# pps-lab/rofl-project-code

Hardware: AMD Instinct MI355X
Metric: range-proof elements/sec (create+verify), d=25k 32-bit (higher is better)
Workload: dtype u32x8 (255-bit integer field)

## Files before the change

### include/rofl_zk_debug.h

```cpp
#ifndef ROFL_ZK_DEBUG_H
#define ROFL_ZK_DEBUG_H
#include "rofl_zk.h"
#ifdef __cplusplus
extern "C" {
#endif

typedef struct {
    double total_ms;
    double msm_accumulate_ms;
    uint64_t msm_accumulate_launches;
    uint64_t msm_terms;
    double fold_ms;
    uint64_t fold_launches;
    uint64_t fold_point_reads;
    double host_ms;
    uint64_t msm_additions;
} rofl_timing_t;
int rofl_last_timing(rofl_timing_t *out);
enum { ROFL_TK_MSM_ACCUMULATE_FB = 0, ROFL_TK_MSM_ACCUMULATE_GEN = 1, ROFL_TK_MSM_SCATTER = 2, ROFL_TK_MSM_REDUCE = 3,
       ROFL_TK_MSM_SMALL = 4, ROFL_TK_FOLD_TAB = 5, ROFL_TK_FOLD = 6, ROFL_TK_OTHER = 7,
       ROFL_TK_SIGMA = 8,
       ROFL_TK_VERIFY_SCALARS = 9,
       ROFL_TK_CODEC = 10,
       ROFL_TK_COUNT = 11 };
typedef struct { double ms; uint64_t launches, fe_muls, bytes; } rofl_kernel_time_t;
int rofl_last_kernel_times(rofl_kernel_time_t out[ROFL_TK_COUNT]);
int rofl_set_timing(int enabled);
int rofl_dbg_map_device(int logical, int physical);
int rofl_dbg_bind_device(int device);

int rofl_dbg_msm(const uint8_t *scalars32, const uint8_t *points32, size_t n, uint8_t out32[32]);
int rofl_dbg_verify_labelled(const uint8_t *label, size_t label_len, size_t gens_capacity, const uint8_t *proof, size_t proof_len,
                             const uint8_t *commits32, size_t m, size_t n_bits, const uint8_t verifier_seed[32], int *ok_out);
int rofl_dbg_msm_retries(uint64_t out[4]);
int rofl_dbg_point_decodes(uint64_t *count_out);
int rofl_bench_femul(unsigned iters, double *fe_mul_per_sec_out);
int rofl_dbg_quad_ops(const uint8_t *pairs64, size_t pairs, unsigned doublings, uint8_t *out_serial32, uint8_t *out_quad32);
int rofl_dbg_fd_ops(unsigned op, size_t n, const uint32_t *in, uint32_t *out);
int rofl_dbg_sc_ops(unsigned op, size_t n, const uint32_t *in, uint32_t *out);
int rofl_dbg_quantize(unsigned site, size_t rows, size_t d, size_t dpad, size_t prove_range, unsigned fp_bits, unsigned fp_frac,
                      const float *values, const uint8_t *blindings32, void *out, float *terms_out, uint32_t *status_out);

int rofl_dbg_host_fd_ops_raw(unsigned op, size_t n, const uint32_t *in, uint32_t *out);
int rofl_dbg_host_sc_ops(unsigned op, size_t n, const uint32_t *in, uint32_t *out);
int rofl_dbg_host_pool_stress(unsigned threads, unsigned jobs);
int rofl_dbg_host_fe_mul(const uint8_t a[32], const uint8_t b[32], uint8_t out[32]);
int rofl_dbg_host_fe_ops(const uint8_t a[32], const uint8_t b[32], uint8_t out_add[32], uint8_t out_sub[32], uint8_t out_sq[32], uint8_t out_inv[32]);
int rofl_dbg_host_sc_invert(const uint8_t a[32], uint8_t out_ref[32], uint8_t out_fast[32], double *ns_ref, double *ns_fast);
int rofl_dbg_host_sc_mul(const uint8_t a[32], const uint8_t b[32], uint8_t out[32]);
int rofl_dbg_host_sc_wide(const uint8_t in[64], uint8_t out[32]);
int rofl_dbg_host_sc_wide_mont(const uint8_t in[64], uint8_t out[32]);
int rofl_dbg_host_sc_lazy(const uint8_t *a32, const uint8_t *b32, size_t count, uint8_t out_lazy[32], uint8_t out_ref[32]);
int rofl_dbg_host_from_uniform(const uint8_t in[64], uint8_t out[32]);
int rofl_dbg_host_scalarmult_base(const uint8_t k[32], int use_blinding_base, uint8_t out[32]);
int rofl_dbg_host_fd_codec(const uint8_t in[32], uint8_t out[32]);
int rofl_dbg_host_decode_encode(const uint8_t in[32], uint8_t out[32]);
int rofl_dbg_host_fd_ops(const uint8_t a[32], const uint8_t b[32], uint8_t out_mul[32], uint8_t out_sq[32], uint8_t out_add[32], uint8_t out_sub[32], uint8_t out_inv[32]);
int rofl_dbg_host_fd_scalarmult(const uint8_t k[32], const uint8_t p[32], uint8_t out[32]);
int rofl_dbg_host_merlin(const uint8_t *label, size_t label_len, const uint8_t *msg, size_t msg_len, uint8_t out[64]);
int rofl_dbg_host_nonce(const uint8_t seed[32], uint64_t idx, uint8_t out[32]);
int rofl_dbg_host_blind(const uint8_t seed[32], uint64_t idx, uint8_t out[32]);
int rofl_dbg_host_dh(const uint8_t sk32[32], const uint8_t *own_pk32, const uint8_t peer_pk32[32], uint8_t out32[32], uint8_t *status);
int rofl_dbg_host_shamir_share(size_t n_secrets, const uint8_t *secrets32, const uint8_t *coef_seeds32, size_t threshold, size_t n_shares,
                               const uint32_t *xs, uint8_t *shares_out32);
int rofl_dbg_host_shamir_reconstruct(size_t n_secrets, size_t n_shares, const uint32_t *xs, const uint8_t *shares32, uint8_t *secrets_out32);
int rofl_dbg_host_feldman_commit(size_t n_secrets, const uint8_t *secrets32, const uint8_t *coef_seeds32, size_t threshold,
                                 uint8_t *commitments_out32);
int rofl_dbg_host_feldman_verify(size_t n_secrets, size_t threshold, const uint8_t *commitments32, size_t n_shares, const uint32_t *xs,
                                 const uint8_t *shares32, uint8_t *verdict_out);

int rofl_dbg_host_bench(int what, unsigned iters, double *ns_out);
int rofl_dbg_host_horner8_selftest(unsigned W, unsigned c, int lanes, double *us_simd, double *us_scalar);
int rofl_dbg_host_encode8_selftest(unsigned batches, double *us_simd, double *us_scalar);
int rofl_dbg_host_merlin8_selftest(int lanes, unsigned count, unsigned skew, double *us_simd, double *us_scalar);
int rofl_dbg_host_merlin8_lbl3_selftest(int lanes, unsigned count, unsigned skew, double *us_simd, double *us_scalar);
int rofl_dbg_host_merlin8_lbl3_strided_selftest(int lanes, unsigned count, unsigned skew, unsigned stride, double *us_simd, double *us_scalar);
int rofl_dbg_host_merlin_run_selftest(unsigned count, unsigned skew);
int rofl_dbg_host_keccak_zmm_selftest(unsigned states, unsigned chain, double *ns_zmm, double *ns_scalar);
int rofl_dbg_last_hops(double out[10]);

#ifdef __cplusplus
}
#endif
#endif
```

### rofl_project_code_amd/csrc/fd_dbg.hpp

```cpp
#pragma once
#include "fe26.hpp"

namespace rofl {

#define FD_DBG_IN 80
#define FD_DBG_OUT 80
enum { FD_DBG_UNPACK = 0, FD_DBG_CARRY = 1, FD_DBG_PACK = 2, FD_DBG_ADD = 3, FD_DBG_SUB = 4, FD_DBG_NEG = 5, FD_DBG_MUL = 6, FD_DBG_SQ = 7,
       FD_DBG_MUL_LOOSE = 8, FD_DBG_SQ_LOOSE = 9, FD_DBG_INVERT = 10, FD_DBG_POW22523 = 11, FD_DBG_SQRT_RATIO = 12, FD_DBG_ABS = 13,
       FD_DBG_PRED = 14, FD_DBG_MADD = 15, FD_DBG_MSUB = 16, FD_DBG_GD_ADD = 17, FD_DBG_GD_DOUBLE = 18, FD_DBG_GD_DOUBLE_NOT = 19,
       FD_DBG_TO_NIELS = 20, FD_DBG_TO_NIELS_ZINV = 21, FD_DBG_THREAD_OPS = 22,
       FD_DBG_GQ_DOUBLE = 22, FD_DBG_GQ_ADD = 23, FD_DBG_OPS = 24 };

HD fd fd_dbg_load(const u32 *in, int k) {
    fd r;
#pragma unroll
    for (int i = 0; i < 10; i++) r.v[i] = in[10 * k + i];
    return r;
}
HD void fd_dbg_store(u32 *out, int k, const fd &a) {
#pragma unroll
    for (int i = 0; i < 10; i++) out[10 * k + i] = a.v[i];
}
HD gd gd_dbg_load(const u32 *in, int k) { gd r; r.X = fd_dbg_load(in, k); r.Y = fd_dbg_load(in, k + 1); r.Z = fd_dbg_load(in, k + 2); r.T = fd_dbg_load(in, k + 3); return r; }
HD void gd_dbg_store(u32 *out, int k, const gd &p) { fd_dbg_store(out, k, p.X); fd_dbg_store(out, k + 1, p.Y); fd_dbg_store(out, k + 2, p.Z); fd_dbg_store(out, k + 3, p.T); }
HD void fe_dbg_store(u32 *out, int w, const fe &a) {
#pragma unroll
    for (int i = 0; i < 8; i++) out[w + i] = a.v[i];
}
HD void niels_dbg_store(u32 *out, const niels &q) { fe_dbg_store(out, 0, q.ypx); fe_dbg_store(out, 8, q.ymx); fe_dbg_store(out, 16, q.t2d); }

HDN inline void fd_dbg_apply(u32 op, const u32 *in, u32 *out) {
    switch (op) {
    case FD_DBG_UNPACK: { fe w; for (int i = 0; i < 8; i++) w.v[i] = in[i]; fd_dbg_store(out, 0, fd_unpack(w)); break; }
    case FD_DBG_CARRY: fd_dbg_store(out, 0, fd_carry(fd_dbg_load(in, 0))); break;
    case FD_DBG_PACK: {
        fe w = fd_pack(fd_dbg_load(in, 0));
        uint8_t b[32]; fe_tobytes(b, w);
        fe_dbg_store(out, 0, w);
        for (int i = 0; i < 8; i++) out[8 + i] = (u32)b[4 * i] | ((u32)b[4 * i + 1] << 8) | ((u32)b[4 * i + 2] << 16) | ((u32)b[4 * i + 3] << 24);
        break;
    }
    case FD_DBG_ADD: fd_dbg_store(out, 0, fd_add(fd_dbg_load(in, 0), fd_dbg_load(in, 1))); break;
    case FD_DBG_SUB: fd_dbg_store(out, 0, fd_sub(fd_dbg_load(in, 0), fd_dbg_load(in, 1))); break;
    case FD_DBG_NEG: fd_dbg_store(out, 0, fd_neg(fd_dbg_load(in, 0))); break;
    case FD_DBG_MUL: fd_dbg_store(out, 0, fd_mul(fd_dbg_load(in, 0), fd_dbg_load(in, 1))); break;
    case FD_DBG_SQ: fd_dbg_store(out, 0, fd_sq(fd_dbg_load(in, 0))); break;
    case FD_DBG_MUL_LOOSE: fd_dbg_store(out, 0, fd_mul(fd_sub(fd_dbg_load(in, 0), fd_dbg_load(in, 1)), fd_add(fd_dbg_load(in, 2), fd_dbg_load(in, 3)))); break;
    case FD_DBG_SQ_LOOSE: fd_dbg_store(out, 0, fd_sq(fd_add(fd_dbg_load(in, 0), fd_dbg_load(in, 1)))); break;
    case FD_DBG_INVERT: fd_dbg_store(out, 0, fd_invert(fd_dbg_load(in, 0))); break;
    case FD_DBG_POW22523: fd_dbg_store(out, 0, fd_pow22523(fd_dbg_load(in, 0))); break;
    case FD_DBG_SQRT_RATIO: { fd r; bool sq = fd_sqrt_ratio_i(r, fd_dbg_load(in, 0), fd_dbg_load(in, 1)); fd_dbg_store(out, 0, r); out[10] = sq ? 1u : 0u; break; }
    case FD_DBG_ABS: fd_dbg_store(out, 0, fd_abs(fd_dbg_load(in, 0))); break;
    case FD_DBG_PRED: {
        fd a = fd_dbg_load(in, 0), b = fd_dbg_load(in, 1);
        out[0] = fd_isneg(a) ? 1u : 0u; out[1] = fd_iszero(a) ? 1u : 0u; out[2] = fd_eq(a, b) ? 1u : 0u;
        break;
    }
    case FD_DBG_MADD: case FD_DBG_MSUB: {
        nd q; q.ypx = fd_dbg_load(in, 4); q.ymx = fd_dbg_load(in, 5); q.t2d = fd_dbg_load(in, 6);
        gd_dbg_store(out, 0, gd_madd(gd_dbg_load(in, 0), q, op == FD_DBG_MSUB));
        break;
    }
    case FD_DBG_GD_ADD: gd_dbg_store(out, 0, gd_add(gd_dbg_load(in, 0), gd_dbg_load(in, 4))); break;
    case FD_DBG_GD_DOUBLE: gd_dbg_store(out, 0, gd_double(gd_dbg_load(in, 0))); break;
    case FD_DBG_GD_DOUBLE_NOT: gd_dbg_store(out, 0, gd_double_not(gd_dbg_load(in, 0))); break;
    case FD_DBG_TO_NIELS: niels_dbg_store(out, gd_to_niels(gd_dbg_load(in, 0))); break;
    case FD_DBG_TO_NIELS_ZINV: niels_dbg_store(out, gd_to_niels_zinv(gd_dbg_load(in, 0), fd_dbg_load(in, 4))); break;
    default: break;
    }
}

#define SC_DBG_IN 264
#define SC_DBG_OUT 8
enum { SC_DBG_MONTMUL = 0, SC_DBG_TO_MONT = 1, SC_DBG_FROM_MONT = 2, SC_DBG_MUL_PLAIN = 3, SC_DBG_ADD = 4, SC_DBG_NEG = 5, SC_DBG_SUB = 6,
       SC_DBG_LOAD_REDUCED = 7,
       SC_DBG_FROM_WIDE = 8, SC_DBG_FROM_WIDE_MONT = 9, SC_DBG_MAC = 10, SC_DBG_INVERT_MONT = 11, SC_DBG_OPS = 12 };

HD sc sc_dbg_load(const u32 *in, int k) {
    sc r;
#pragma unroll
    for (int i = 0; i < 8; i++) r.v[i] = in[8 * k + i];
    return r;
}
HDN inline sc sc_dbg_apply(u32 op, const u32 *in) {
    const sc a = sc_dbg_load(in, 0), b = sc_dbg_load(in, 1);
    switch (op) {
    case SC_DBG_MONTMUL: return sc_montmul(a, b);
    case SC_DBG_TO_MONT: return sc_to_mont(a);
    case SC_DBG_FROM_MONT: return sc_from_mont(a);
    case SC_DBG_MUL_PLAIN: return sc_mul_plain(a, b);
    case SC_DBG_ADD: return sc_add(a, b);
    case SC_DBG_NEG: return sc_neg(a);
    case SC_DBG_SUB: return sc_sub(a, b);
    case SC_DBG_LOAD_REDUCED: return sc_geq_l(a.v) ? sc_from_mont(sc_to_mont(a)) : a;
    case SC_DBG_FROM_WIDE: return sc_from_wide(a, b);
    case SC_DBG_FROM_WIDE_MONT: return sc_from_wide_mont(a, b);
    case SC_DBG_MAC: {
        u32 acc[17]; for (int i = 0; i < 17; i++) acc[i] = 0;
        u32 count = in[256] > 16 ? 16 : in[256];
        for (u32 k = 0; k < count; k++) sc_mac_wide(acc, sc_dbg_load(in, 2 * (int)k), sc_dbg_load(in, 2 * (int)k + 1));
        return sc_redc_wide(acc);
    }
    case SC_DBG_INVERT_MONT: return sc_invert_mont(a);
    default: return sc_zero();
    }
}

}
```

### rofl_project_code_amd/csrc/fe26.hpp

```cpp
#pragma once
#include "fe32.hpp"
#if defined(ROFL_FD_CHECK_HOST) && !defined(__HIP_DEVICE_COMPILE__)
#include <assert.h>
#define ROFL_FD_CHECK 1
#endif

namespace rofl {

struct fd { u32 v[10]; };
struct gd { fd X, Y, Z, T; };
struct nd { fd ypx, ymx, t2d; };

#define FD_M26 0x3ffffffu
#define FD_M25 0x1ffffffu

HD fd fd_zero() { fd r = {{0, 0, 0, 0, 0, 0, 0, 0, 0, 0}}; return r; }
HD fd fd_one() { fd r = {{1, 0, 0, 0, 0, 0, 0, 0, 0, 0}}; return r; }

HD fd fd_unpack(const fe &a) {
    const u32 *w = a.v;
    fd r;
    r.v[0] = w[0] & FD_M26;
    r.v[1] = ((w[0] >> 26) | (w[1] << 6)) & FD_M25;
    r.v[2] = ((w[1] >> 19) | (w[2] << 13)) & FD_M26;
// ... 68 lines not shown

HD fd fd_reduce_cols(u64 h0, u64 h1, u64 h2, u64 h3, u64 h4, u64 h5, u64 h6, u64 h7, u64 h8, u64 h9) {
    u64 c;
    c = h0 >> 26; h1 += c; h0 &= FD_M26;
    c = h4 >> 26; h5 += c; h4 &= FD_M26;
    c = h1 >> 25; h2 += c; h1 &= FD_M25;
    c = h5 >> 25; h6 += c; h5 &= FD_M25;
    c = h2 >> 26; h3 += c; h2 &= FD_M26;
    c = h6 >> 26; h7 += c; h6 &= FD_M26;
    c = h3 >> 25; h4 += c; h3 &= FD_M25;
    c = h7 >> 25; h8 += c; h7 &= FD_M25;
    c = h4 >> 26; h5 += c; h4 &= FD_M26;
    c = h8 >> 26; h9 += c; h8 &= FD_M26;
    c = h9 >> 25; h0 += c * 19; h9 &= FD_M25;
    c = h0 >> 26; h1 += c; h0 &= FD_M26;
    fd r = {{(u32)h0, (u32)h1, (u32)h2, (u32)h3, (u32)h4, (u32)h5, (u32)h6, (u32)h7, (u32)h8, (u32)h9}};
    return r;
}

HD fd fd_mul(const fd &f, const fd &g) {
#if defined(ROFL_FD_CHECK)
    for (int i = 0; i < 10; i++) { assert((u64)f.v[i] < (1ULL << 28) + (1ULL << 20)); assert((u64)g.v[i] * 19 < (1ULL << 32)); }
#endif
    u32 f0 = f.v[0], f1 = f.v[1], f2 = f.v[2], f3 = f.v[3], f4 = f.v[4], f5 = f.v[5], f6 = f.v[6], f7 = f.v[7], f8 = f.v[8], f9 = f.v[9];
    u32 g0 = g.v[0], g1 = g.v[1], g2 = g.v[2], g3 = g.v[3], g4 = g.v[4], g5 = g.v[5], g6 = g.v[6], g7 = g.v[7], g8 = g.v[8], g9 = g.v[9];
    u32 g1_19 = 19 * g1, g2_19 = 19 * g2, g3_19 = 19 * g3, g4_19 = 19 * g4, g5_19 = 19 * g5, g6_19 = 19 * g6, g7_19 = 19 * g7, g8_19 = 19 * g8, g9_19 = 19 * g9;
    u32 f1_2 = 2 * f1, f3_2 = 2 * f3, f5_2 = 2 * f5, f7_2 = 2 * f7, f9_2 = 2 * f9;
#define M(a, b) ((u64)(a) * (b))
    u64 h0 = M(f0, g0) + M(f1_2, g9_19) + M(f2, g8_19) + M(f3_2, g7_19) + M(f4, g6_19) + M(f5_2, g5_19) + M(f6, g4_19) + M(f7_2, g3_19) + M(f8, g2_19) + M(f9_2, g1_19);
    u64 h1 = M(f0, g1) + M(f1, g0) + M(f2, g9_19) + M(f3, g8_19) + M(f4, g7_19) + M(f5, g6_19) + M(f6, g5_19) + M(f7, g4_19) + M(f8, g3_19) + M(f9, g2_19);
    u64 h2 = M(f0, g2) + M(f1_2, g1) + M(f2, g0) + M(f3_2, g9_19) + M(f4, g8_19) + M(f5_2, g7_19) + M(f6, g6_19) + M(f7_2, g5_19) + M(f8, g4_19) + M(f9_2, g3_19);
    u64 h3 = M(f0, g3) + M(f1, g2) + M(f2, g1) + M(f3, g0) + M(f4, g9_19) + M(f5, g8_19) + M(f6, g7_19) + M(f7, g6_19) + M(f8, g5_19) + M(f9, g4_19);
    u64 h4 = M(f0, g4) + M(f1_2, g3) + M(f2, g2) + M(f3_2, g1) + M(f4, g0) + M(f5_2, g9_19) + M(f6, g8_19) + M(f7_2, g7_19) + M(f8, g6_19) + M(f9_2, g5_19);
    u64 h5 = M(f0, g5) + M(f1, g4) + M(f2, g3) + M(f3, g2) + M(f4, g1) + M(f5, g0) + M(f6, g9_19) + M(f7, g8_19) + M(f8, g7_19) + M(f9, g6_19);
    u64 h6 = M(f0, g6) + M(f1_2, g5) + M(f2, g4) + M(f3_2, g3) + M(f4, g2) + M(f5_2, g1) + M(f6, g0) + M(f7_2, g9_19) + M(f8, g8_19) + M(f9_2, g7_19);
    u64 h7 = M(f0, g7) + M(f1, g6) + M(f2, g5) + M(f3, g4) + M(f4, g3) + M(f5, g2) + M(f6, g1) + M(f7, g0) + M(f8, g9_19) + M(f9, g8_19);
    u64 h8 = M(f0, g8) + M(f1_2, g7) + M(f2, g6) + M(f3_2, g5) + M(f4, g4) + M(f5_2, g3) + M(f6, g2) + M(f7_2, g1) + M(f8, g0) + M(f9_2, g9_19);
    u64 h9 = M(f0, g9) + M(f1, g8) + M(f2, g7) + M(f3, g6) + M(f4, g5) + M(f5, g4) + M(f6, g3) + M(f7, g2) + M(f8, g1) + M(f9, g0);
    return fd_reduce_cols(h0, h1, h2, h3, h4, h5, h6, h7, h8, h9);
}

HD fd fd_sq(const fd &f) {
#if defined(ROFL_FD_CHECK)
    for (int i = 0; i < 10; i++) assert((u64)f.v[i] * ((i & 1) ? 38 : 19) < (1ULL << 32));
#endif
    u32 f0 = f.v[0], f1 = f.v[1], f2 = f.v[2], f3 = f.v[3], f4 = f.v[4], f5 = f.v[5], f6 = f.v[6], f7 = f.v[7], f8 = f.v[8], f9 = f.v[9];
    u32 f0_2 = 2 * f0, f1_2 = 2 * f1, f2_2 = 2 * f2, f3_2 = 2 * f3, f4_2 = 2 * f4, f5_2 = 2 * f5, f6_2 = 2 * f6, f7_2 = 2 * f7;
    u32 f5_38 = 38 * f5, f6_19 = 19 * f6, f7_38 = 38 * f7, f8_19 = 19 * f8, f9_38 = 38 * f9;
    u64 h0 = M(f0, f0) + M(f1_2, f9_38) + M(f2_2, f8_19) + M(f3_2, f7_38) + M(f4_2, f6_19) + M(f5, f5_38);
    u64 h1 = M(f0_2, f1) + M(f2, f9_38) + M(f3_2, f8_19) + M(f4, f7_38) + M(f5_2, f6_19);
    u64 h2 = M(f0_2, f2) + M(f1_2, f1) + M(f3_2, f9_38) + M(f4_2, f8_19) + M(f5_2, f7_38) + M(f6, f6_19);
    u64 h3 = M(f0_2, f3) + M(f1_2, f2) + M(f4, f9_38) + M(f5_2, f8_19) + M(f6, f7_38);
    u64 h4 = M(f0_2, f4) + M(f1_2, f3_2) + M(f2, f2) + M(f5_2, f9_38) + M(f6_2, f8_19) + M(f7, f7_38);
    u64 h5 = M(f0_2, f5) + M(f1_2, f4) + M(f2_2, f3) + M(f6, f9_38) + M(f7_2, f8_19);
    u64 h6 = M(f0_2, f6) + M(f1_2, f5_2) + M(f2_2, f4) + M(f3_2, f3) + M(f7_2, f9_38) + M(f8, f8_19);
    u64 h7 = M(f0_2, f7) + M(f1_2, f6) + M(f2_2, f5) + M(f3_2, f4) + M(f8, f9_38);
    u64 h8 = M(f0_2, f8) + M(f1_2, f7_2) + M(f2_2, f6) + M(f3_2, f5_2) + M(f4, f4) + M(f9, f9_38);
    u64 h9 = M(f0_2, f9) + M(f1_2, f8) + M(f2_2, f7) + M(f3_2, f6) + M(f4_2, f5);
    return fd_reduce_cols(h0, h1, h2, h3, h4, h5, h6, h7, h8, h9);
}
#undef M

HDN inline fd fd_sqn(fd a, int n) { for (int i = 0; i < n; i++) a = fd_sq(a); return a; }
HDN inline fd fd_invert(const fd &z) {
    fd z2 = fd_sq(z);
    fd z9 = fd_mul(fd_sqn(z2, 2), z);
    fd z11 = fd_mul(z9, z2);
    fd z_5_0 = fd_mul(fd_sq(z11), z9);
    fd z_10_0 = fd_mul(fd_sqn(z_5_0, 5), z_5_0);
    fd z_20_0 = fd_mul(fd_sqn(z_10_0, 10), z_10_0);
    fd z_40_0 = fd_mul(fd_sqn(z_20_0, 20), z_20_0);
    fd z_50_0 = fd_mul(fd_sqn(z_40_0, 10), z_10_0);
    fd z_100_0 = fd_mul(fd_sqn(z_50_0, 50), z_50_0);
    fd z_200_0 = fd_mul(fd_sqn(z_100_0, 100), z_100_0);
    fd z_250_0 = fd_mul(fd_sqn(z_200_0, 50), z_50_0);
    return fd_mul(fd_sqn(z_250_0, 5), z11);
}

HD fd fd_d2() {
    fd r = {{0x2b2f159u, 0x1a6e509u, 0x22add7au, 0x0d4141du, 0x0038052u, 0x0f3d130u, 0x3407977u, 0x19ce331u, 0x1c56dffu, 0x0901b67u}};
    return r;
}

HD gd gd_identity() { gd r; r.X = fd_zero(); r.Y = fd_one(); r.Z = fd_one(); r.T = fd_zero(); return r; }
HD gd gd_unpack(const ge &p) { gd r; r.X = fd_unpack(p.X); r.Y = fd_unpack(p.Y); r.Z = fd_unpack(p.Z); r.T = fd_unpack(p.T); return r; }
HD ge gd_pack(const gd &p) { ge r; r.X = fd_pack(p.X); r.Y = fd_pack(p.Y); r.Z = fd_pack(p.Z); r.T = fd_pack(p.T); return r; }
HD nd nd_unpack(const niels &q) { nd r; r.ypx = fd_unpack(q.ypx); r.ymx = fd_unpack(q.ymx); r.t2d = fd_unpack(q.t2d); return r; }

HD gd gd_madd(const gd &p, const nd &q, bool neg) {
    fd a_f = fd_select(q.ymx, q.ypx, neg), b_f = fd_select(q.ypx, q.ymx, neg);
    fd A = fd_mul(fd_sub(p.Y, p.X), a_f);
    fd B = fd_mul(fd_add(p.Y, p.X), b_f);
    fd C = fd_mul(p.T, q.t2d);
    fd D = fd_add(p.Z, p.Z);
    fd E = fd_sub(B, A), H = fd_add(B, A);
    fd DmC = fd_sub(D, C), DpC = fd_add(D, C);
    gd r;
    fd Fbig = DmC, Gsm = DpC;
    fd XF = fd_select(Fbig, Gsm, neg);
    fd XG = fd_select(Gsm, Fbig, neg);
    r.X = fd_mul(XF, E);
    r.Y = fd_mul(XG, H);
    r.T = fd_mul(E, H);
    r.Z = fd_mul(Fbig, Gsm);
    return r;
}
HD gd gd_add(const gd &p, const gd &q) {
    fd A = fd_mul(fd_sub(p.Y, p.X), fd_sub(q.Y, q.X));
    fd B = fd_mul(fd_add(p.Y, p.X), fd_add(q.Y, q.X));
    fd C = fd_mul(fd_mul(p.T, q.T), fd_d2());
    fd D = fd_mul(p.Z, q.Z); D = fd_add(D, D);
    fd E = fd_sub(B, A), H = fd_add(B, A);
    fd F = fd_sub(D, C), G = fd_add(D, C);
    gd r; r.X = fd_mul(F, E); r.Y = fd_mul(G, H); r.T = fd_mul(E, H); r.Z = fd_mul(F, G);
    return r;
}
HD gd gd_double(const gd &p) {
    fd XX = fd_sq(p.X), YY = fd_sq(p.Y), ZZ = fd_sq(p.Z);
    fd ZZ2 = fd_add(ZZ, ZZ);
    fd S = fd_sq(fd_add(p.X, p.Y));
    fd cY = fd_carry(fd_add(YY, XX));
    fd cZ = fd_carry(fd_sub(YY, XX));
    fd cX = fd_sub(S, cY);
    fd cT = fd_sub(ZZ2, cZ);
    gd r; r.X = fd_mul(cT, cX); r.Y = fd_mul(cY, cZ); r.Z = fd_mul(cT, cZ); r.T = fd_mul(cX, cY);
    return r;
}
HD gd gd_double_not(const gd &p) {
    fd XX = fd_sq(p.X), YY = fd_sq(p.Y), ZZ = fd_sq(p.Z);
    fd ZZ2 = fd_add(ZZ, ZZ);
    fd S = fd_sq(fd_add(p.X, p.Y));
    fd cY = fd_carry(fd_add(YY, XX));
    fd cZ = fd_carry(fd_sub(YY, XX));
    fd cX = fd_sub(S, cY);
    fd cT = fd_sub(ZZ2, cZ);
    gd r; r.X = fd_mul(cT, cX); r.Y = fd_mul(cY, cZ); r.Z = fd_mul(cT, cZ); r.T = p.T;
    return r;
}
HDN inline niels gd_to_niels_zinv(const gd &p, const fd &zi) {
    fd x = fd_mul(p.X, zi), y = fd_mul(p.Y, zi);
    niels r;
    r.ypx = fd_pack(fd_add(y, x)); r.ymx = fd_pack(fd_sub(y, x)); r.t2d = fd_pack(fd_mul(fd_mul(x, y), fd_d2()));
    return r;
}
HDN inline niels gd_to_niels(const gd &p) {
    fd zi = fd_invert(p.Z);
    fd x = fd_mul(p.X, zi), y = fd_mul(p.Y, zi);
    niels r;
    r.ypx = fd_pack(fd_add(y, x)); r.ymx = fd_pack(fd_sub(y, x)); r.t2d = fd_pack(fd_mul(fd_mul(x, y), fd_d2()));
    return r;
}

HD bool fd_iszero(const fd &a) { return fe_iszero(fd_pack(a)); }
HD bool fd_isneg(const fd &a) { return fe_isneg(fd_pack(a)); }
HD bool fd_eq(const fd &a, const fd &b) { return fe_iszero(fe_sub(fd_pack(a), fd_pack(b))); }
HD fd fd_abs(const fd &a) { fd t = fd_carry(a); return fd_select(t, fd_carry(fd_neg(t)), fd_isneg(t)); }
HDN inline fd fd_pow22523(const fd &z) {
    fd z2 = fd_sq(z);
    fd z9 = fd_mul(fd_sqn(z2, 2), z);
    fd z11 = fd_mul(z9, z2);
    fd z_5_0 = fd_mul(fd_sq(z11), z9);
    fd z_10_0 = fd_mul(fd_sqn(z_5_0, 5), z_5_0);
    fd z_20_0 = fd_mul(fd_sqn(z_10_0, 10), z_10_0);
    fd z_40_0 = fd_mul(fd_sqn(z_20_0, 20), z_20_0);
    fd z_50_0 = fd_mul(fd_sqn(z_40_0, 10), z_10_0);
    fd z_100_0 = fd_mul(fd_sqn(z_50_0, 50), z_50_0);
    fd z_200_0 = fd_mul(fd_sqn(z_100_0, 100), z_100_0);
    fd z_250_0 = fd_mul(fd_sqn(z_200_0, 50), z_50_0);
    return fd_mul(fd_sqn(z_250_0, 2), z);
}
HDN inline bool fd_sqrt_ratio_i(fd &out, const fd &u, const fd &v) {
    fd sqrtm1 = fd_unpack(fe_sqrtm1());
    fd v3 = fd_mul(fd_sq(v), v);
    fd v7 = fd_mul(fd_sq(v3), v);
    fd r = fd_mul(fd_mul(u, v3), fd_pow22523(fd_mul(u, v7)));
    fd check = fd_mul(v, fd_sq(r));
    fd neg_u = fd_carry(fd_neg(u));
    bool correct = fd_eq(check, u);
    bool flipped = fd_eq(check, neg_u);
    bool flipped_i = fd_eq(check, fd_mul(neg_u, sqrtm1));
    fd r_prime = fd_mul(r, sqrtm1);
    r = fd_select(r, r_prime, flipped || flipped_i);
    out = fd_abs(r);
    return correct || flipped;
}
HDN inline void gd_ristretto_encode(uint8_t *s, const gd &p) {
    fd sqrtm1 = fd_unpack(fe_sqrtm1());
    fd X = fd_carry(p.X), Y = fd_carry(p.Y), Z = fd_carry(p.Z), T = fd_carry(p.T);
    fd u1 = fd_mul(fd_add(Z, Y), fd_sub(Z, Y));
    fd u2 = fd_mul(X, Y);
    fd invsqrt; fd_sqrt_ratio_i(invsqrt, fd_one(), fd_mul(u1, fd_sq(u2)));
    fd den1 = fd_mul(invsqrt, u1), den2 = fd_mul(invsqrt, u2);
    fd z_inv = fd_mul(fd_mul(den1, den2), T);
    fd ix0 = fd_mul(X, sqrtm1), iy0 = fd_mul(Y, sqrtm1);
    fd ench = fd_mul(den1, fd_unpack(fe_invsqrt_a_minus_d()));
    bool rotate = fd_isneg(fd_mul(T, z_inv));
    fd x = fd_select(X, iy0, rotate), y = fd_select(Y, ix0, rotate);
    fd den_inv = fd_select(den2, ench, rotate);
    if (fd_isneg(fd_mul(x, z_inv))) y = fd_carry(fd_neg(y));
    fd sres = fd_abs(fd_mul(den_inv, fd_sub(Z, y)));
    fe_tobytes(s, fd_pack(sres));
}
HDN inline bool gd_ristretto_decode(gd &p, const uint8_t *sb) {
    fe s8 = fe_frombytes(sb);
    uint8_t chk[32]; fe_tobytes(chk, s8);
    bool canon = true;
    for (int i = 0; i < 32; i++) canon &= (chk[i] == sb[i]);
    if (!canon || (sb[0] & 1)) return false;
    fd s = fd_unpack(s8);
    fd ss = fd_sq(s);
    fd u1 = fd_carry(fd_sub(fd_one(), ss)), u2 = fd_carry(fd_add(fd_one(), ss));
    fd u2s = fd_sq(u2);
    fd v = fd_carry(fd_sub(fd_carry(fd_neg(fd_mul(fd_unpack(fe_d()), fd_sq(u1)))), u2s));
    fd invsqrt; bool ok = fd_sqrt_ratio_i(invsqrt, fd_one(), fd_mul(v, u2s));
    fd dx = fd_mul(invsqrt, u2);
    fd dy = fd_mul(fd_mul(invsqrt, dx), v);
    fd x = fd_abs(fd_mul(fd_add(s, s), dx));
    fd y = fd_mul(u1, dy);
    fd t = fd_mul(x, y);
    if (!ok || fd_isneg(t) || fd_iszero(y)) return false;
    p.X = x; p.Y = y; p.Z = fd_one(); p.T = t;
// ... 5 lines not shown
```

### rofl_project_code_amd/csrc/host_msm.hpp

```cpp
#pragma once

MsmPlan msm_plan(size_t n, size_t np = 1) {
    MsmPlan p;
    static const size_t t13 = knob("ROFL_MSM_T13") ? (size_t)atol(knob("ROFL_MSM_T13")) : ((size_t)1 << 13);
    static const size_t t10_knob = knob("ROFL_MSM_T10") ? (size_t)atol(knob("ROFL_MSM_T10")) : 0;
    const size_t t10 = t10_knob ? t10_knob : (np >= 32 ? (size_t)1 << 11 : (size_t)1 << 9);
    if (n >= (1u << 17)) p.c = 16; else if (n >= t13) p.c = 13; else if (n >= t10) p.c = 10; else if (n >= 64) p.c = 7; else p.c = 4;
    if (const char *e = knob("ROFL_MSM_C")) { int v = atoi(e); if (v == 4 || v == 7 || v == 10 || v == 13 || v == 16) p.c = (u32)v; }
    p.W = (254 + p.c - 1) / p.c;
    p.W = (253 - p.c + p.c - 1) / p.c + 1;
    p.wide = (253 - p.c) - (p.c - 1) * (p.W - 1);
    p.B = 1u << (p.c - 1);
    p.levels = (p.c - 1) / 3;
    return p;
}
struct MsmOpt { u32 lr_nh = 0, lr_ng = 0; const niels *fb_wtab = nullptr; size_t fb_stride = 0; u32 fb_c = 16; std::function<void()> overlap; std::function<void(size_t)> post; u32 tag = 0;
                std::function<void(size_t, int)> post8;
                const sc *ip_dev = nullptr; u32 ip_nblk = 0; const niels *qpts = nullptr; bool *ip_included = nullptr;
                hipEvent_t pts_ready = nullptr; };

struct MsmAllow { bool fb = true, small = true, two = true, slots = true; };
enum class MsmKind { FixedBase, Small, Slots, CountSort };
struct MsmJob {
    MsmWs *ws = nullptr; size_t np = 0, nq = 0, n = 0, PW = 0; MsmPlan P{}; MsmKind kind = MsmKind::CountSort; bool lr = false, two = false, dev_horner = false;
    bool host8 = false;
    u32 sets = 0, cap = 0;
    u32 cap_bin = 0, tile = 0, fused_t = 0, acc_bal = 0;
    u32 small_group = 1;
    bool fb() const { return kind == MsmKind::FixedBase; }
};
static const u32 MSM_OVF_MAX = 4096;

static inline u32 msm_bin_cap(size_t avg) {
    static const int sigmas = knob("ROFL_MSM_BIN_SIGMA") ? atoi(knob("ROFL_MSM_BIN_SIGMA")) : 8;
    size_t hot = 2 * avg, dev = 1;
    if (sigmas <= 0) return (u32)((hot + 256 + 63) / 64 * 64);
    while (dev * dev < hot) dev++;
    return (u32)((hot + (size_t)sigmas * dev + 64 + 63) / 64 * 64);
}

bool msm_plan_job(Ctx &C, MsmJob &J, const MsmOpt &opt, const MsmAllow &al, MsmMap &mm, u32 &small_cap, Msm2L &tl) {
    const size_t np = J.np, n = J.n; const bool lr = J.lr; const size_t nq = J.nq;
    const size_t per_side = lr ? n / 2 : n;
    mm = MsmMap{opt.lr_nh, opt.lr_ng, 0, 0, 0};
    J.two = false; J.sets = 0;
    bool want_fb = al.fb && opt.fb_wtab != nullptr && C.msm_slots;
    if (want_fb) {
        J.kind = MsmKind::FixedBase;
        J.P = msm_plan_c(opt.fb_c);
        bool crowded = C.crowded();
        size_t want = crowded ? C.msm_fb_threads / 2 : C.msm_fb_threads;
        u32 sets = J.P.W;
        for (u32 sdiv = 1; sdiv <= J.P.W; sdiv++)
            if (J.P.W % sdiv == 0 && (size_t)nq * (lr ? 2 : 1) * sdiv * J.P.B >= want) { sets = sdiv; break; }
        if (al.two && C.msm_two_level && (J.P.B == 32768 || J.P.B == 16384) && per_side >= 8192)
            while (sets < J.P.W && (size_t)msm_bin_cap(per_side * (J.P.W / sets) / 512) * 4 + 1024 > 96 * 1024) {
                u32 nx = sets + 1; while (nx < J.P.W && J.P.W % nx) nx++;
                sets = nx;
            }
        J.sets = sets;
        mm.fb_sets = sets; mm.fb_wps = J.P.W / sets; mm.fb_stride = (u32)opt.fb_stride;
        J.PW = nq * (lr ? 2 : 1) * sets;
        u32 cap = 16; while (cap < 2048 && (size_t)cap * J.P.B < 3 * per_side * (mm.fb_wps + 1)) cap *= 2;
        if (mm.fb_wps == 1) cap *= 2;
        J.cap = cap;
        bool two = al.two && C.msm_two_level && J.P.W * opt.fb_stride <= ((size_t)1 << 24) && (J.P.B == 32768 || J.P.B == 16384);
        const u32 fb0 = J.P.B == 32768 ? 7u : 6u;
        tl = Msm2L{256, fb0, 24, 0, 144};
        if (two) {
            auto size_bins = [&]() { tl.cap_bin = msm_bin_cap(per_side * mm.fb_wps / tl.nbins); return (size_t)tl.cap_bin * 4 + 1024 <= 96 * 1024; };
            bool fits = size_bins();
            if (!fits) { tl = Msm2L{512, fb0 - 1, 24, 0, 72}; fits = size_bins(); }
            if (!fits || per_side < 8192) two = false;
        }
        J.two = two; J.cap_bin = two ? tl.cap_bin : 0u;
        if (!two && (size_t)J.PW * J.P.B * J.cap * 4 > ((size_t)8 << 30)) return false;
        return true;
    }
    bool slots_mode = al.slots && C.msm_slots;
    J.P = msm_plan(n, J.np);
    if (C.msm_small_max && al.small && slots_mode && per_side <= C.msm_small_max && J.P.c > 10 && np * 26 <= 512) J.P = msm_plan_c(10);
    J.PW = np * J.P.W;
    { u32 cap = 16; while (cap < 256 && (size_t)cap * J.P.B < 4 * n) cap *= 2; J.cap = cap; }
    small_cap = per_side <= 8 * J.P.B ? (u32)MSM_SMALL_CAP : 72u;
    size_t small_lds = std::max((size_t)J.P.B * 4 * (1 + small_cap), std::max(((size_t)(J.P.B / 8) * 4 + (size_t)(J.P.B / 16) * 5 + 1) * sizeof(ge), ((size_t)J.P.B + (size_t)J.P.B * 3 / 4 + 1) * sizeof(ge)));
    bool small = slots_mode && al.small && C.msm_small_max && per_side <= C.msm_small_max && J.P.c <= 10 && per_side <= 16 * J.P.B && (J.PW <= 512 || small_lds <= 24 * 1024);
    J.kind = small ? MsmKind::Small : slots_mode ? MsmKind::Slots : MsmKind::CountSort;
    J.small_group = 1;
    if (small && J.P.B == 64 && J.PW > 512) {
        static const u32 grp = knob("ROFL_MSM_SMALL_GROUP") ? (u32)std::max(1, std::min(4, atoi(knob("ROFL_MSM_SMALL_GROUP")))) : 4u;
        J.small_group = grp == 3 ? 2 : grp;
    }
    if (J.kind == MsmKind::Slots && (size_t)J.PW * J.P.B * J.cap * 4 > ((size_t)8 << 30)) return false;
    return true;
}

MsmJob msm_enqueue(Ctx &C, MsmWs &W, const std::vector<MsmProb> &probs, size_t n, const MsmOpt &opt, MsmAllow &al, hipStream_t st = nullptr) {
    if (!st) st = C.stream;
    static const u32 acc_balance = knob("ROFL_ACC_BALANCE") ? (atoi(knob("ROFL_ACC_BALANCE")) ? 1u : 0u) : 1u;
    MsmJob J; J.ws = &W; J.np = probs.size(); J.n = n; J.lr = opt.lr_nh != 0; J.nq = J.lr ? J.np / 2 : J.np;
    const size_t np = J.np, nq = J.nq; const bool lr = J.lr;
    J.acc_bal = acc_balance;
    MsmMap mm{}; u32 small_cap = 0; Msm2L tl{};
    while (!msm_plan_job(C, J, opt, al, mm, small_cap, tl)) {
        if (al.fb && opt.fb_wtab && C.msm_slots) al.fb = false; else al.slots = false;
    }
    const MsmPlan &P = J.P; const size_t PW = J.PW; const bool fb = J.fb();
    MsmProb *d_probs = W.probs.as<MsmProb>(np);
    MsmProb *h_probs = W.h_probs.as<MsmProb>(np);
    for (size_t i = 0; i < np; i++) h_probs[i] = fb ? MsmProb{opt.fb_wtab, probs[i].scal} : probs[i];
    if (W.probs_on_dev.size() != np || memcmp(W.probs_on_dev.data(), h_probs, sizeof(MsmProb) * np) != 0) {
        HIPCHK(hipMemcpyAsync(d_probs, h_probs, sizeof(MsmProb) * np, hipMemcpyHostToDevice, st));
        W.probs_on_dev.assign(h_probs, h_probs + np);
    }
    u32 *cnt = W.cnt.as<u32>(PW * P.B + 4), *off = W.off.as<u32>(PW * P.B), *cur = W.cur.as<u32>(PW * P.B);
    u32 *perm = W.perm.as<u32>(PW * P.B);
    ge *buckets = W.buckets.as<ge>(PW * P.B);
    MsmWin mw{P.c, P.W, P.wide};
    static const bool host8_on = h8::available() && !(knob("ROFL_MSM_HOST8") && atoi(knob("ROFL_MSM_HOST8")) == 0);
    static const size_t host8_min = knob("ROFL_MSM_HOST8_MIN") ? (size_t)std::max(1L, atol(knob("ROFL_MSM_HOST8_MIN"))) : 8;
    J.dev_horner = !fb && P.W <= 64 && (np >= C.msm_dev_horner_min || (host8_on && np >= host8_min));
    J.host8 = J.dev_horner && host8_on;
    ge *hres_dev = W.h_res.dev<ge>(PW * (size_t)P.c + np);
    u32 *h_flag = W.h_ovf.as<u32>(4), *d_flag = W.h_ovf.dev<u32>(4);
    const u32 Wb = (u32)(PW / nq);
    const u32 n_side = (u32)(lr ? n / 2 : n);
    const u32 nb_final = P.c - 1;
    hipEvent_t e0 = nullptr, e1 = nullptr;
    *h_flag = 0;
    if (opt.ip_included) *opt.ip_included = J.kind == MsmKind::Small && opt.ip_dev && opt.qpts && lr;
    if (J.kind == MsmKind::Small) {
        ge *S_fin_s = J.dev_horner ? W.S[0].as<ge>(PW) : hres_dev;
        ge *C_fin_s = J.dev_horner ? W.Cacc[0].as<ge>(PW * (size_t)nb_final) : hres_dev + PW;
        const u32 G = J.small_group;
        size_t lds_lists = G > 1 ? (size_t)G * P.B * (4 + 2 * (size_t)small_cap)
                                 : (size_t)P.B * 4 * (1 + small_cap);
        size_t lds_red = G > 1 ? ((size_t)G * P.B * 3 / 4 + 1) * sizeof(ge)
                               : std::max(((size_t)(P.B / 8) * 4 + (size_t)(P.B / 16) * 5 + 1) * sizeof(ge), ((size_t)P.B + (size_t)P.B * 3 / 4 + 1) * sizeof(ge));
        uint64_t items = (uint64_t)np * n_side * P.W;
        KSpan ks(C.tm, st, ROFL_TK_MSM_SMALL, items * 7 + (uint64_t)PW * P.B * 10, (uint64_t)np * n_side * (32 + 96));
        static const bool small_tl = knob("ROFL_DBG_SMALL_TIMELINE") != nullptr;
        unsigned long long *tl_dev = nullptr;
        if (small_tl) { HIPCHK(hipMalloc(&tl_dev, PW * 32)); HIPCHK(hipMemsetAsync(tl_dev, 0, PW * 32, st)); }
        if (opt.pts_ready) HIPCHK(hipStreamWaitEvent(st, opt.pts_ready, 0));
        const u32 Wg = (P.W + G - 1) / G;
        if (G > 1)
            ROFL_LAUNCH(k_msm_small_g, dim3((unsigned)(np * Wg)), dim3(G * P.B), std::max(lds_lists, lds_red), st, n_side, mw, mm, d_probs, buckets,
                               S_fin_s, C_fin_s, nb_final, d_flag, small_cap, G, tl_dev, J.host8 ? hres_dev : (ge *)nullptr,
                               lr ? opt.ip_dev : (const sc *)nullptr, opt.ip_nblk, lr ? opt.qpts : (const niels *)nullptr);
        else
            ROFL_LAUNCH(k_msm_small, dim3((unsigned)PW), dim3(P.B < 64 ? 64 : P.B), std::max(lds_lists, lds_red), st, n_side, mw, mm, d_probs, buckets,
                               S_fin_s, C_fin_s, nb_final, d_flag, small_cap, G, tl_dev, J.host8 ? hres_dev : (ge *)nullptr,
                               lr ? opt.ip_dev : (const sc *)nullptr, opt.ip_nblk, lr ? opt.qpts : (const niels *)nullptr);
        if (small_tl) {
            std::vector<unsigned long long> hts(PW * 4);
            HIPCHK(hipMemcpyAsync(hts.data(), tl_dev, PW * 32, hipMemcpyDeviceToHost, st)); HIPCHK(hipStreamSynchronize(st)); HIPCHK(hipFree(tl_dev));
            double ph[3] = {0, 0, 0}; unsigned long long t_lo = ~0ull, t_hi = 0;
            const size_t nblocks = G > 1 ? np * Wg : PW;
            for (size_t b = 0; b < nblocks; b++) { for (int k = 0; k < 3; k++) ph[k] += (double)(hts[b * 4 + k + 1] - hts[b * 4 + k]); t_lo = std::min(t_lo, hts[b * 4]); t_hi = std::max(t_hi, hts[b * 4 + 3]); }
            fprintf(stderr, "[rofl] k_msm_small PW=%zu blocks=%zu n_side=%u c=%u: rank %.1f us, bucket sums %.1f us, reduce %.1f us (block means); first start -> last end %.1f us\n",
                    PW, nblocks, n_side, P.c, ph[0] / nblocks * 0.01, ph[1] / nblocks * 0.01, ph[2] / nblocks * 0.01, (double)(t_hi - t_lo) * 0.01);
        }
        if (J.host8) {}
        else if (J.dev_horner) ROFL_LAUNCH(k_msm_horner, dim3((unsigned)np), dim3(256), 0, st, mw, (const ge *)S_fin_s, (const ge *)C_fin_s, nb_final, hres_dev);
        return J;
    }
    const uint64_t terms = (uint64_t)(lr ? nq : np) * n;
    if (J.two) {
        u32 *bins = W.sorted.as<u32>(PW * tl.nbins * tl.cap_bin);
        u32 *bcur = W.cur.as<u32>(PW * tl.nbins * 2);
        u32 *btail = W.tail.as<u32>(PW * tl.nbins * (size_t)MSM_BIN_TAIL);
        HIPCHK(hipMemsetAsync(bcur, 0, sizeof(u32) * PW * tl.nbins * 2, st));
        const u64 wdiv = (u64)mm.fb_stride * mm.fb_sets;
        const bool worder = mm.fb_wps > 1 && mm.fb_wps <= 16 && wdiv && (wdiv & (wdiv - 1)) == 0 && wdiv < ((u64)1 << tl.ebits);
        const u32 worder_wps = worder ? mm.fb_wps : 1u, worder_shift = worder ? (u32)lg2u((size_t)wdiv) : 0u;
        u32 iter_pts = (tl.stage >= 144 ? 16384u : 12288u) / mm.fb_wps; if (iter_pts < 1024) iter_pts = 1024;
        u32 tile = iter_pts;
        while (((size_t)((n_side + tile - 1) / tile) * PW > 512 || (n_side + tile - 1) / tile > 48) && tile < n_side) tile *= 2;
        {
            const size_t kCU = 256;
            auto cost = [&](u32 t) { const size_t tiles = (n_side + t - 1) / t; return (double)((tiles * PW + kCU - 1) / kCU) * ((double)std::min<u32>(t, n_side) + 0.25 * iter_pts); };
            u32 best = tile; double best_cost = cost(tile);
            for (u32 t = iter_pts; t < n_side + iter_pts; t += iter_pts) {
                const size_t tiles = (n_side + t - 1) / t;
                if (tiles > 48 || tiles * PW > 4096) continue;
                const double c = cost(t);
                if (c < best_cost * 0.999) { best = t; best_cost = c; }
            }
            if (knob("ROFL_TRACE")) fprintf(stderr, "[rofl] bin_l1 tiling: n_side=%u PW=%zu iter=%u: tile %u (%zu blocks, cost %.0f) -> best %u (%zu blocks, cost %.0f)\n", n_side, PW, iter_pts, tile,
                                            (size_t)((n_side + tile - 1) / tile) * PW, cost(tile), best, (size_t)((n_side + best - 1) / best) * PW, best_cost);
            if (best_cost < 0.85 * cost(tile)) tile = best;
        }
        dim3 grid((n_side + tile - 1) / tile, (u32)PW);
        { KSpan ks(C.tm, st, ROFL_TK_MSM_SCATTER, 0, terms * 32 + terms * P.W * 4);
          ROFL_LAUNCH(k_msm_bin_l1, grid, dim3(1024), (size_t)(tl.nbins + tl.nbins * tl.stage) * 4, st, n_side, tile, iter_pts, mw, mm, d_probs, bcur, bins, btail, tl, d_flag);
          ROFL_LAUNCH(k_msm_bin_l2, dim3(tl.nbins, (u32)PW), dim3(512), (size_t)(2 * 128 * worder_wps + tl.cap_bin) * 4, st, tl, P.B, bcur, bins, (const u32 *)btail, cnt, off, d_flag,
                      worder_wps, worder_shift); }
        ROFL_LAUNCH(k_msm_scan, dim3((unsigned)PW), dim3(P.B >= 1024 ? 1024 : 256), 0, st, P.B, cnt, off, (u32 *)nullptr, perm);
        if (C.tm.enabled) { e0 = C.tm.get(); e1 = C.tm.get(); HIPCHK(hipEventRecord(e0, st)); }
        {
            KSpan ks_acc(C.tm, st, ROFL_TK_MSM_ACCUMULATE_FB, terms * P.W * 7, terms * 32);
            static const char *timeline = knob("ROFL_DBG_ACC_TIMELINE");
            if (timeline) {
                dim3 g = grid1((size_t)Wb * P.B, (u32)nq);
                size_t waves = (size_t)g.x * g.y * (TPB / 64);
                unsigned long long *rec; HIPCHK(hipMalloc(&rec, waves * 32)); HIPCHK(hipMemsetAsync(rec, 0, waves * 32, st));
                ROFL_LAUNCH(k_msm_accumulate_fb_dbg, g, dim3(TPB), 0, st, (u32)n, P.c, Wb, (u32)(np / nq), d_probs, cnt, off, bins, perm, buckets, MSM_LIST_ABS, acc_balance, rec);
                std::vector<unsigned long long> h(waves * 4);
                HIPCHK(hipMemcpyAsync(h.data(), rec, waves * 32, hipMemcpyDeviceToHost, st)); HIPCHK(hipStreamSynchronize(st));
                if (FILE *f = fopen(timeline, "ab")) { unsigned long long hdr[4] = {0x54494d45ull, waves, g.x, g.y}; fwrite(hdr, 8, 4, f); fwrite(h.data(), 8, h.size(), f); fclose(f); }
                HIPCHK(hipFree(rec));
            } else
            ROFL_LAUNCH(k_msm_accumulate_fb, grid1((size_t)Wb * P.B, (u32)nq), dim3(TPB), 0, st, (u32)n, P.c, Wb, (u32)(np / nq), d_probs, cnt, off, bins, perm, buckets, MSM_LIST_ABS,
                        acc_balance | ((worder && nq > 1 && Wb > 1) ? 2u : 0u));
        }
        if (C.tm.enabled) HIPCHK(hipEventRecord(e1, st));
    } else if (J.kind != MsmKind::CountSort) {
        HIPCHK(hipMemsetAsync(cnt, 0, sizeof(u32) * (PW * P.B + 4), st));
        const u32 cap = J.cap;
        u32 *slots = W.sorted.as<u32>(PW * P.B * cap);
        MsmOvf *ovf = W.ovf.as<MsmOvf>(MSM_OVF_MAX);
        u32 *ovf_count = cnt + PW * P.B;
        if (C.msm_lds && n >= C.msm_lds_min && (size_t)P.B * 4 <= 128 * 1024) {
            u32 per_q = fb ? J.sets : P.W;
            u32 tile = n_side;
            u32 wps = fb ? mm.fb_wps : 1;
            while (tile > 1024 && ((size_t)tile * wps > (size_t)C.msm_lds_tile || (size_t)((n_side + tile - 1) / tile) * nq * (lr ? 2 : 1) * per_q < 256)) tile /= 2;
            dim3 grid((n_side + tile - 1) / tile, (u32)(nq * (lr ? 2 : 1) * per_q));
            J.tile = tile;
            uint64_t items = terms * P.W;
            KSpan ks(C.tm, st, ROFL_TK_MSM_SCATTER, 0, terms * 32 + items * 4);
            ROFL_LAUNCH(k_msm_scatter_lds, grid, dim3(1024), (size_t)P.B * 4, st, n_side, tile, mw, mm, d_probs, cnt, slots, cap, ovf_count, ovf, MSM_OVF_MAX);
        } else
            ROFL_LAUNCH(k_msm_scatter_slots, grid1(n, (u32)(nq * P.W)), dim3(TPB), 0, st, (u32)n, mw, mm, d_probs, cnt, slots, cap, ovf_count, ovf, MSM_OVF_MAX);
        ROFL_LAUNCH(k_msm_scan, dim3((unsigned)PW), dim3(P.B >= 1024 ? 1024 : 256), 0, st, P.B, cnt, off, (u32 *)nullptr, perm);
        if (opt.pts_ready) HIPCHK(hipStreamWaitEvent(st, opt.pts_ready, 0));
        if (C.tm.enabled) { e0 = C.tm.get(); e1 = C.tm.get(); HIPCHK(hipEventRecord(e0, st)); }
        {
            uint64_t acc_adds = terms * P.W;
            KSpan ks_acc(C.tm, st, fb ? ROFL_TK_MSM_ACCUMULATE_FB : ROFL_TK_MSM_ACCUMULATE_GEN, acc_adds * 7, terms * 32);
            if (fb) ROFL_LAUNCH(k_msm_accumulate_fb, grid1((size_t)Wb * P.B, (u32)nq), dim3(TPB), 0, st, (u32)n, P.c, Wb, (u32)(np / nq), d_probs, cnt, off, slots, perm, buckets, cap, acc_balance);
            else ROFL_LAUNCH(k_msm_accumulate_gen, grid1((size_t)Wb * P.B, (u32)nq), dim3(TPB), 0, st, (u32)n, P.c, Wb, (u32)(np / nq), d_probs, cnt, off, slots, perm, buckets, cap, acc_balance);
        }
        if (C.tm.enabled) HIPCHK(hipEventRecord(e1, st));
        ROFL_LAUNCH(k_msm_overflow, dim3(1), dim3(64), 0, st, Wb, P.B, (u32)(np / nq), d_probs, ovf_count, ovf, MSM_OVF_MAX, buckets, fb ? 1 : 0);
        HIPCHK(hipMemcpyAsync(h_flag, ovf_count, 4, hipMemcpyDeviceToHost, st));
    } else {
        HIPCHK(hipMemsetAsync(cnt, 0, sizeof(u32) * (PW * P.B + 4), st));
        u32 *sorted = W.sorted.as<u32>(PW * n * 2);
        ROFL_LAUNCH(k_msm_count, grid1(n, (u32)(nq * P.W)), dim3(TPB), 0, st, (u32)n, mw, mm, d_probs, cnt);
        ROFL_LAUNCH(k_msm_scan, dim3((unsigned)PW), dim3(P.B >= 1024 ? 1024 : 256), 0, st, P.B, cnt, off, cur, perm);
        ROFL_LAUNCH(k_msm_scatter, grid1(n, (u32)(nq * P.W)), dim3(TPB), 0, st, (u32)n, mw, mm, d_probs, cur, sorted);
        if (opt.pts_ready) HIPCHK(hipStreamWaitEvent(st, opt.pts_ready, 0));
        if (C.tm.enabled) { e0 = C.tm.get(); e1 = C.tm.get(); HIPCHK(hipEventRecord(e0, st)); }
        ROFL_LAUNCH(k_msm_accumulate_gen, grid1((size_t)Wb * P.B, (u32)nq), dim3(TPB), 0, st, (u32)n, P.c, Wb, (u32)(np / nq), d_probs, cnt, off, sorted, perm, buckets, 0u, acc_balance);
        if (C.tm.enabled) HIPCHK(hipEventRecord(e1, st));
    }
    if (C.tm.enabled) {
        C.tm.acc_ev.push_back({e0, e1}); C.tm.t.msm_accumulate_launches++; C.tm.t.msm_additions += terms * P.W;
        char tg[96]; snprintf(tg, sizeof tg, "msm np=%zu n=%zu c=%u cap=%u fb=%u lr=%d", np, n, P.c, J.kind != MsmKind::CountSort ? J.cap : 0u, fb ? J.sets : 0u, (int)lr); C.tm.acc_tag.push_back(tg);
    }
    const ge *S_in = buckets; const ge *C_in = nullptr;
    u32 E = P.B, nb = 0, lv = 0;
    uint64_t red_adds = 0;
    { u32 e = P.B, b = 0; while (e > 512) { red_adds += (uint64_t)(e / 8) * (11 + 7 * b); e /= 8; b += 3; }
      red_adds += (uint64_t)(e / 8) * (16 + 7 * b); e /= 8; b += 3; while (e > 1) { red_adds += (uint64_t)(e / 2) * (1 + b); e /= 2; b++; } }
    ge *S_fin = J.dev_horner ? W.S[1].as<ge>(PW) : hres_dev;
    ge *C_fin = J.dev_horner ? W.Cacc[1].as<ge>(PW * (size_t)nb_final) : hres_dev + PW;
    {
        KSpan ks_red(C.tm, st, ROFL_TK_MSM_REDUCE, red_adds * PW * 9, (uint64_t)PW * P.B * 128);
        while (E > 512) {
            u32 E8 = E / 8;
            ge *S_out = W.S[lv & 1].as<ge>(PW * E8);
            ge *C_out = W.Cacc[lv & 1].as<ge>(PW * (size_t)(nb + 3) * E8);
            ROFL_LAUNCH(k_msm_reduce_level, grid1((size_t)E8 * (1 + nb), (u32)PW), dim3(TPB), 0, st, E, nb, S_in, C_in, S_out, C_out);
            S_in = S_out; C_in = C_out; E = E8; nb += 3; lv++;
        }
        if (J.dev_horner) { S_fin = W.S[lv & 1].as<ge>(PW); C_fin = W.Cacc[lv & 1].as<ge>(PW * (size_t)nb_final); }
        static const u32 red_fused_max = knob("ROFL_RED_FUSED_T") ? (u32)std::max(64, atoi(knob("ROFL_RED_FUSED_T"))) : 768u;
        u32 fused_items = (E / 8) * (4 + nb), fused_threads = fused_items > 512 ? (fused_items > 640 ? 768 : 640) : fused_items > 256 ? 512 : fused_items > 128 ? 256 : fused_items > 64 ? 128 : 64;
        if (fused_threads > red_fused_max) fused_threads = red_fused_max;
        J.fused_t = fused_threads;
        size_t lds = ((size_t)(E / 8) * (1 + nb + 3) + (size_t)(E / 16) * (1 + nb + 4) + 1) * sizeof(ge);
        ROFL_LAUNCH(k_msm_reduce_fused, dim3((unsigned)PW), dim3(fused_threads), lds, st, E, nb, S_in, C_in, S_fin, C_fin, nb_final);
    }
    if (J.host8)
        ROFL_LAUNCH(k_msm_wsum, grid1(PW * 4), dim3(TPB), 0, st, (u32)PW, (const ge *)S_fin, (const ge *)C_fin, nb_final, hres_dev);
    else if (J.dev_horner)
        ROFL_LAUNCH(k_msm_horner, dim3((unsigned)np), dim3(256), 0, st, mw, (const ge *)S_fin, (const ge *)C_fin, nb_final, hres_dev);
    return J;
}

std::atomic<uint64_t> g_msm_stat[4];
bool msm_retry_inner(const MsmJob &J, MsmAllow &al);
bool msm_retry(const MsmJob &J, MsmAllow &al) {
    const bool small = J.kind == MsmKind::Small, two = J.two;
    const bool again = msm_retry_inner(J, al);
    g_msm_stat[again ? (small ? 1 : two ? 2 : 3) : 0].fetch_add(1, std::memory_order_relaxed);
    return again;
}
bool msm_retry_inner(const MsmJob &J, MsmAllow &al) {
    u32 flag = *J.ws->h_ovf.as<u32>(4);
    if (knob("ROFL_TRACE") && J.kind != MsmKind::CountSort)
        fprintf(stderr, "[rofl] msm np=%zu n=%zu c=%u cap=%u fb=%u lr=%d overflow=%u kind=%s two=%d bin=%u tile=%u group=%u fused_t=%u bal=%u horner=%s\n", J.np, J.n, J.P.c, J.cap, J.fb() ? J.sets : 0u, (int)J.lr, flag,
                J.fb() ? "fb" : J.kind == MsmKind::Small ? "small" : "slots", (int)J.two, J.cap_bin, J.tile, J.kind == MsmKind::Small ? J.small_group : 0u, J.fused_t, J.acc_bal, J.host8 ? "host8" : J.dev_horner ? "dev" : "host");
    if (J.kind == MsmKind::Small) { if (flag) { al.small = false; return true; } return false; }
    if (J.two) { if (flag) { al.two = false; return true; } return false; }
    if (J.kind == MsmKind::CountSort) return false;
    if (flag > MSM_OVF_MAX) { if (J.fb()) al.fb = false; else al.slots = false; return true; }
    return false;
}

void msm_finish(Ctx &C, const MsmJob &J, std::vector<ge5> &results, const MsmOpt &opt) {
    const size_t np = J.np, PW = J.PW; const MsmPlan &P = J.P; const u32 sets = J.sets;
    u32 nb = P.c - 1;
    ge *h = J.ws->h_res.as<ge>(PW * (size_t)P.c + np);
    double t0 = now_ms();
    results.resize(np);
    std::vector<double> cpu_each(np, 0.0);
    const char *fin = "host";
    if (J.host8) {
        fin = "host8";
        u32 pos[64];
// ... 138 lines not shown
```

### rofl_project_code_amd/csrc/host_prover.hpp

```cpp
#pragma once

void tr_append_point(Merlin &t, const char *label, const ge5 &p, uint8_t *enc_out) {
    uint8_t e[32]; h51::encode(e, p); t.append(label, e, 32); if (enc_out) memcpy(enc_out, e, 32);
}
void fill_pow2(sc *tab, sc base_mont, int count) { tab[0] = base_mont; for (int i = 1; i < count; i++) tab[i] = sc_montmul(tab[i - 1], tab[i - 1]); }

sc sum_partials(const sc *p, size_t count, size_t stride, size_t which) {
    sc acc = sc_zero();
    for (size_t i = 0; i < count; i++) acc = sc_add(acc, p[i * stride + which]);
    return acc;
}

struct ChunkNonce { int mode; NonceSeed seed; const uint8_t *d_stream; u64 stream_scalars, base; };
void prove_chunks(Ctx &C, const char *label, size_t P, size_t n, size_t m, const u64 *d_vshift, const sc *d_blind,
                  const std::vector<ChunkNonce> &nonces, const uint8_t *h_V , uint8_t *const *proofs_out,
                  hipEvent_t v_ready = nullptr ) {
    size_t N = n * m; unsigned lgN = lg2u(N);
    static const bool ptrace = knob("ROFL_TRACE") && atoi(knob("ROFL_TRACE")) >= 2;
    double pt0 = now_ms(), ptl = pt0;
    auto mark = [&](const char *what, long a = -1) {
        if (!ptrace) return;
        double t = now_ms(); fprintf(stderr, "[rofl-trace lane=%p] %-14s %6ld  +%.3f ms  (t=%.3f)\n", (void *)&C, what, a, t - ptl, t - pt0); ptl = t;
    };
    size_t plen = 32 * (9 + 2 * (size_t)lgN);
// ... 217 lines not shown
                sc inv = h51::sc_invert_mont_fast(pre[nch - 1]);
                for (int k = nch - 1; k >= 1; k--) { uim[k] = sc_montmul(inv, pre[k - 1]); inv = sc_montmul(inv, um[k]); }
                uim[0] = inv;
            } else
                for (int k = 0; k < nch; k++) uim[k] = h51::sc_invert_mont_fast(um[k]);
            for (int k = 0; k < nch; k++) {
                size_t c = (p0 >> 1) + (size_t)k;
                h_round[2 * c] = um[k]; h_round[2 * c + 1] = uim[k];
                h_cp[c].pend_u[pu[c].size()] = um[k]; h_cp[c].pend_ui[pu[c].size()] = uim[k];
                pu[c].push_back(um[k]); pui[c].push_back(uim[k]);
            }
        };
        msm_run(C, pr, 2 * n_g, res, mo);
        mark("round msm", (long)(2 * n_g));
        bool last = (round + 1 == lgN);
        r++;
        unsigned t_now = first_level ? (unsigned)C.fold_t1 : (unsigned)C.fold_t;
        size_t n_after = n_g >> r;
        bool fold_pays = n_after >= C.fold_min || (n_after >= 64 && 2 * P * n_after >= 8 * C.fold_min);
        if (!last && r >= t_now && fold_pays) {
            size_t n_new = n_g >> r; u32 nsrc = 1u << r;
            bool use_tab = first_level && C.fold_tab;
            FoldTabCfg fc = gens.fc();
            size_t dstride = use_tab ? (size_t)fc.np * FOLD_TAB_DIGITS : 256;
            th = now_ms();
            const size_t dbytes = use_tab ? 2 : 1;
            int8_t *h_dig = C.h_fdig.as<int8_t>(2 * P * nsrc * dstride * dbytes);
            int16_t *h_dig16 = reinterpret_cast<int16_t *>(h_dig);
            memset(h_dig, 0, 2 * P * nsrc * dstride * dbytes);
            FoldProb *h_fp = C.h_fprob.as<FoldProb>(2 * P);
            niels *gnew = C.gbuf[gsel].as<niels>(P * 2 * n_new);
            std::vector<int> topc(P, 0);
            C.pool->run(P, [&](size_t c) {
                int top = 0;
                sc yn = sc_one_mont();
                sc ystep = sc_one_mont();
                { size_t e = n_new; int bidx = 0; while (e) { if (e & 1) ystep = sc_montmul(ystep, h_cp[c].yinvpow2[bidx]); e >>= 1; bidx++; } }
                sc g0, h0; stab(c, 0, g0, h0);
                sc gall, hall; stab(c, nsrc - 1, gall, hall);
                for (u32 h = 1; h < nsrc; h++) {
                    sc g, hh; stab(c, h, g, hh);
                    yn = sc_montmul(yn, ystep);
                    hh = sc_montmul(hh, yn);
                    g = sc_montmul(g, gall); hh = sc_montmul(hh, hall);
                    sc gc = h_canon(g), hc = h_canon(hh);
                    if (use_tab) {
                        for (u32 pc = 0; pc < fc.np; pc++) {
                            auto piece = [&](const sc &s) {
                                u32 bit0 = pc * fc.pb; u64 lo = (u64)s.v[bit0 / 32] | ((bit0 / 32 + 1 < 8) ? (u64)s.v[bit0 / 32 + 1] << 32 : 0);
                                lo >>= (bit0 % 32);
                                return fc.pb == 64 ? lo : (lo & (((u64)1 << fc.pb) - 1));
                            };
                            int t1 = wnaf_u64(h_dig16 + (((2 * c) * nsrc + h) * fc.np + pc) * FOLD_TAB_DIGITS, piece(gc), fc.w);
                            int t2 = wnaf_u64(h_dig16 + (((2 * c + 1) * nsrc + h) * fc.np + pc) * FOLD_TAB_DIGITS, piece(hc), fc.w);
                            top = std::max(top, std::max(t1, t2));
                        }
                    } else {
                        int t1 = sc_naf(h_dig + ((2 * c) * nsrc + h) * 256, gc);
                        int t2 = sc_naf(h_dig + ((2 * c + 1) * nsrc + h) * 256, hc);
                        top = std::max(top, std::max(t1, t2));
                    }
                }
                gscale[c] = sc_montmul(gscale[c], g0); hscale[c] = sc_montmul(hscale[c], h0); h_cp[c].gscale = gscale[c]; h_cp[c].hscale = hscale[c];
                h_fp[2 * c] = FoldProb{cur[c], gnew + c * 2 * n_new};
                h_fp[2 * c + 1] = FoldProb{cur[c] + n_g, gnew + c * 2 * n_new + n_new};
                topc[c] = top;
            });
            int top = 0; for (int t : topc) top = std::max(top, t);
            C.tm.t.host_ms += now_ms() - th;
            int8_t *d_dig = nullptr; FoldProb *d_fp = nullptr;
            if (!use_tab) {
                d_dig = C.naf.as<int8_t>(2 * P * nsrc * dstride);
                HIPCHK(hipMemcpyAsync(d_dig, h_dig, 2 * P * nsrc * dstride, hipMemcpyHostToDevice, C.stream));
                d_fp = C.foldprobs.as<FoldProb>(2 * P);
                HIPCHK(hipMemcpyAsync(d_fp, h_fp, sizeof(FoldProb) * 2 * P, hipMemcpyHostToDevice, C.stream));
            }
            hipEvent_t e0 = nullptr, e1 = nullptr;
            if (C.tm.enabled) { e0 = C.tm.get(); e1 = C.tm.get(); HIPCHK(hipEventRecord(e0, C.stream)); }
            {
                u32 K = 1;
                size_t thr = (size_t)2 * P * n_new;
                while (K < FOLD_MAXSEG && thr * K < (size_t)C.fold_threads / (C.crowded() ? 2 : 1)) K *= 2;
                if (C.fold_k > 0) K = (u32)C.fold_k;
                FoldSeg seg{};
                double eff = (double)(nsrc - 1);
                double cst = 1.0 + (use_tab ? eff * fc.np / (fc.w + 1.0) : eff / 3.0), lo_t = 0, hi_t = (top + 1) * cst + top + 1;
                int bounds[FOLD_MAXSEG + 1];
                for (int it = 0; it < 60; it++) {
                    double T = 0.5 * (lo_t + hi_t), pos = 0;
                    for (u32 k = 0; k < K; k++) { double len = (T - pos) / cst; if (len < 0) len = 0; pos += len; }
                    if (pos >= top + 1) hi_t = T; else lo_t = T;
                }
                { double pos = 0; bounds[0] = 0; for (u32 k = 0; k < K; k++) { double len = (hi_t - pos) / cst; if (len < 0) len = 0; pos += len; bounds[k + 1] = (int)(pos + 0.5); } }
                bounds[K] = top + 1;
                for (u32 k = 1; k <= K; k++) if (bounds[k] < bounds[k - 1]) bounds[k] = bounds[k - 1];
                for (u32 k = 0; k <= FOLD_MAXSEG; k++) seg.lo[k] = bounds[k <= K ? k : K];
                dim3 grid((unsigned)((n_new + 63) / 64), (u32)(2 * P)), block(64, K);
                if (knob("ROFL_TRACE")) fprintf(stderr, "[rofl] fold chunks=%zu n_g=%zu n_new=%zu nsrc=%u tab=%d pb=%u w=%u K=%u top=%d\n", P, n_g, n_new, nsrc, (int)use_tab, fc.pb, fc.w, K, top);
                uint64_t nz = 0;
                if (C.tm.enabled) { size_t tot_d = 2 * P * nsrc * dstride; for (size_t q = 0; q < tot_d; q++) nz += use_tab ? h_dig16[q] != 0 : h_dig[q] != 0; }
                uint64_t fold_muls = (nz * 7 / (2 * P) + (uint64_t)(top + 1) * 8 + 7) * (uint64_t)(2 * P * n_new);
                KSpan ks_fold(C.tm, C.stream, use_tab ? ROFL_TK_FOLD_TAB : ROFL_TK_FOLD, fold_muls, (uint64_t)2 * P * n_g * 32 + (uint64_t)2 * P * n_new * 32);
                if (use_tab) {
                    const bool defer = 2 * P * n_new >= ((size_t)1 << 17);
                    ge *ext = defer ? C.foldext.as<ge>(2 * P * n_new) : nullptr;
                    std::vector<std::vector<u32>> tev(2 * P);
                    C.pool->run(2 * P, [&](size_t q) {
                        std::vector<u32> &e = tev[q];
                        for (u32 h = 1; h < nsrc; h++)
                            for (u32 pc = 0; pc < fc.np; pc++) {
                                const int16_t *dd = h_dig16 + ((q * nsrc + h) * fc.np + pc) * FOLD_TAB_DIGITS;
                                for (int b = 0; b < FOLD_TAB_DIGITS; b++) if (int d = dd[b]) e.push_back(FOLD_EV(b, h, pc * fc.e + ((u32)((d < 0 ? -d : d) - 1) >> 1), d < 0));
                            }
                        std::stable_sort(e.begin(), e.end(), [](u32 x, u32 y) { return (x & 511u) > (y & 511u); });
                    });
                    size_t tot_ev = 0; for (auto &e : tev) tot_ev += e.size();
                    u32 *h_ev = C.h_fev.as<u32>(tot_ev + 4 + (2 * P * sizeof(FoldWProb) + 3) / 4);
                    const size_t wp_off = (tot_ev + 2) & ~(size_t)1;
                    FoldWProb *h_wp = reinterpret_cast<FoldWProb *>(h_ev + wp_off);
                    size_t off = 0;
                    for (size_t q = 0; q < 2 * P; q++) {
                        std::vector<u32> &e = tev[q];
                        FoldWProb &w = h_wp[q];
                        w.src = h_fp[q].src; w.dst = h_fp[q].dst; w.tab_off = (u32)(h_fp[q].src - tbl); w.ev_off = (u32)off; w.n_ev = (u32)e.size();
                        for (u32 k = 0; k < FOLD_MAXSEG; k++) {
                            const int hi = seg.lo[std::min<u32>(k + 1, FOLD_MAXSEG)] - 1;
                            u32 j = 0; while (j < e.size() && (int)(e[j] & 511u) > hi) j++;
                            w.seg_start[k] = j;
                        }
                        memcpy(h_ev + off, e.data(), e.size() * sizeof(u32)); off += e.size();
                    }
                    u32 *d_ev = C.fold_ev.as<u32>(tot_ev + 4 + (2 * P * sizeof(FoldWProb) + 3) / 4);
                    HIPCHK(hipMemcpyAsync(d_ev, h_ev, wp_off * sizeof(u32) + 2 * P * sizeof(FoldWProb), hipMemcpyHostToDevice, C.stream));
                    ROFL_LAUNCH(k_fold_gens_w, grid, block, (K - 1) * 64 * sizeof(ge), C.stream, (u32)n_new, seg, reinterpret_cast<const FoldWProb *>(d_ev + wp_off),
                                       (const u32 *)d_ev, (const niels *)(tbl + (size_t)(2 * N)), (size_t)(2 * N), ext);
                    if (defer) {
                        if (!C.ev_norm) { HIPCHK(hipEventCreateWithFlags(&C.ev_norm, hipEventDisableTiming)); HIPCHK(hipEventCreateWithFlags(&C.ev_norm0, hipEventDisableTiming)); }
                        HIPCHK(hipEventRecord(C.ev_norm0, C.stream));
                        HIPCHK(hipStreamWaitEvent(C.stream2, C.ev_norm0, 0));
                        const size_t tot = 2 * P * n_new;
                        ROFL_LAUNCH(k_niels_batch, grid1((tot + NB_BATCH - 1) / NB_BATCH), dim3(TPB), 0, C.stream2, (u32)tot, (const ge *)ext, gnew);
                        HIPCHK(hipEventRecord(C.ev_norm, C.stream2));
                        pts_pending = true;
                    }
                }
                else if (nsrc == 4)
                    ROFL_LAUNCH(k_fold_gens4, grid, block, (K - 1) * 64 * sizeof(ge), C.stream, (u32)n_new, seg, (const FoldProb *)d_fp, d_dig);
                else
                    ROFL_LAUNCH(k_fold_gens, grid, block, (K - 1) * 64 * sizeof(ge), C.stream, (u32)n_new, nsrc, seg, (const FoldProb *)d_fp, d_dig, 1);
            }
            if (C.tm.enabled) { HIPCHK(hipEventRecord(e1, C.stream)); C.tm.fold_ev.push_back({e0, e1}); C.tm.t.fold_launches++; { char tg[96]; snprintf(tg, sizeof tg, "fold n_g=%zu nsrc=%u tab=%d", n_g, nsrc, (int)use_tab); C.tm.fold_tag.push_back(tg); } C.tm.t.fold_point_reads += (uint64_t)2 * P * n_g; }
            HIPCHK(hipMemcpyAsync(d_cp, h_cp, sizeof(ChunkParams) * P, hipMemcpyHostToDevice, C.stream));
            if (ptrace) C.sync();
            mark("fold", (long)n_new);
            for (size_t c = 0; c < P; c++) { cur[c] = gnew + c * 2 * n_new; pu[c].clear(); pui[c].clear(); }
            n_g = n_new; r = 0; gsel ^= 1; first_level = false; just_materialised = true;
        }
    }
    const sc *q = C.h_abfin.as<sc>(4 * P);
    for (size_t c = 0; c < P; c++) {
        uint8_t *o = proofs_out[c] + 7 * 32 + 64 * lgN;
        const sc &um = h_round[2 * c], &uim = h_round[2 * c + 1];
        sc_tobytes(o, h_canon(sc_add(sc_montmul(q[4 * c], um), sc_montmul(q[4 * c + 1], uim))));
        sc_tobytes(o + 32, h_canon(sc_add(sc_montmul(q[4 * c + 2], uim), sc_montmul(q[4 * c + 3], um))));
    }
    if (ptrace) {
        fprintf(stderr, "[rofl-hops] %d msm calls: enqueue %.3f ms, sync wait %.3f, horner wall %.3f (max task cpu %.3f), round-host wall %.3f (max task cpu %.3f)\n",
                C.hs.n, C.hs.enqueue, C.hs.sync, C.hs.horner_wall, C.hs.horner_cpu, C.hs.host_wall, C.hs.host_cpu);
        C.hs = Ctx::HopStats();
    }
}
```

### rofl_project_code_amd/csrc/host_rt.hpp

```cpp
#pragma once

struct Knob { const char *name, *dflt, *what; };
static const Knob KNOBS[] = {
    {"ROFL_LANES", "3", "calls that can be in flight on a device (HIP stream + workspace each); 1..16, larger values are clamped (with a note on stderr)"},
    {"ROFL_DEVICES", "0", "option devices: bit mask of the logical devices the batch entry points shard their clients over (0 = the calling thread's device only)"},
    {"ROFL_DEVICE_MAP", "", "logical -> physical HIP device, comma separated (0,0 = two logical devices on GPU 0: how the multi-device paths are tested on a one-GPU box); default: identity"},
    {"ROFL_RCCL_LIB", "librccl.so.1", "the RCCL library rofl_comm_* loads with dlopen (a host that has torch in the process names /opt/rocm/lib/librccl.so.1: the bare soname would resolve to torch's bundled copy)"},
    {"ROFL_HOST_THREADS", "usable cores, in [2, 16]", "threads of the primary lane's host pool (window combination, encodings, transcripts of a round); other lanes: usable cores, in [6, 12]"},
    {"ROFL_POOL_SPIN_US", "400", "how long an idle pool worker polls for the next job before it sleeps (0 = sleep at once)"},
    {"ROFL_BLOCKING_SYNC", "-1", "option blocking_sync: -1 spin while <= 3 calls are in flight, 0 always spin, 1 sleep between polls"},
    {"ROFL_VERIFY_ZIP_TRUNCATE", "0", "option verify_zip_truncate: 1 = the reference's zip-truncating verify_rangeproof"},
    {"ROFL_VERIFY_BATCH", "1", "option verify_batch: 0 = one check per proof, 1 = one per client, 2 = one per batch of clients (bisecting down to per-client checks on failure)"},
    {"ROFL_SIGMA_BATCH", "1", "option sigma_batch: 0 = one check per element in the Sigma-proof verifiers"},
    {"ROFL_STAGE_KEEP_MB", "256", "pinned staging memory a lane keeps between calls (a call that needed more frees it when it ends)"},
    {"ROFL_GENS_LAZY", "1", "0 = the first call of a shape waits for its full fold table (otherwise it is served from the compact table while a background thread builds the full one)"},
    {"ROFL_GENS_LAZY_IDLE_MS", "20", "the background build of a full fold table starts when no call has been in flight for this long (its allocation stalls every HIP call of the process)"},
    {"ROFL_GENS_LAZY_MAX_WAIT_MS", "3000", "... or after this long, whichever comes first (a host that never pauses still gets its full table)"},
    {"ROFL_GENS_RESERVE_MB", "40960", "HBM a table allocation of 4 GB or more leaves free on the device (other contexts / processes / workspaces; the runtime aborts when HBM runs out): the table is narrowed instead"},
    {"ROFL_GENS_BUDGET_MB", "131072", "HBM budget of the generator-table cache (LRU eviction of unpinned entries beyond it)"},
    {"ROFL_FOLD_T1", "3", "IPP rounds before the first generator fold (1..6)"},
    {"ROFL_FOLD_T", "2", "IPP rounds between later folds (1..6)"},
    {"ROFL_FOLD_MIN", "1024", "no fold once fewer generators per chunk would remain (launches with many chunks fold down to 64)"},
    {"ROFL_MSM_BIN_SIGMA", "8", "room of a coarse bin of the two-level sort above twice its mean load, in standard deviations of that load (0 = the fixed 256 entries of rounds 2-3)"},
    {"ROFL_FOLD_TAB", "1", "0 = first fold without the precomputed odd-multiple slices"},
// ... 4 lines not shown
    {"ROFL_FOLD_THREADS", "131072", "fold launches with fewer threads split their chains into segments"},
    {"ROFL_MSM_FB", "1", "0 = no window tables (every MSM generic)"},
    {"ROFL_MSM_FB_MIN", "4096", "generator sets smaller than this get no window table"},
    {"ROFL_MSM_FB_C", "0", "one window width (13, 15, 16) for every window table; 0 = 16-bit tables, plus a 15-bit one for generator sets below 2^17 that launches with many problems and the verifier use"},
    {"ROFL_MSM_FB_THREADS", "524288", "accumulate threads a fixed-base launch aims for (decides the number of bucket sets)"},
    {"ROFL_MSM_TWO_LEVEL", "1", "0 = slot sort instead of the two-level bucket sort in fixed-base launches"},
    {"ROFL_MSM_SLOTS", "1", "0 = count / scan / scatter sort only (no fixed-capacity structures)"},
    {"ROFL_MSM_LDS", "1", "0 = per-item global atomics instead of LDS ranking in the slot sort"},
    {"ROFL_MSM_LDS_MIN", "8192", "MSMs with fewer terms use the per-item slot sort"},
    {"ROFL_MSM_LDS_TILE", "131072", "items one block of the LDS slot sort ranks"},
    {"ROFL_MSM_SMALL_MAX", "8192", "terms per side up to which a generic MSM runs as one fused launch (0 = off)"},
    {"ROFL_MSM_SMALL_GROUP", "4", "windows of a problem per block of the fused launch at c = 7 with more than 512 bucket arrays (1 = one window per one-wave block, 2, 4)"},
    {"ROFL_MERLIN_X8", "1", "0 = the verifier hashes every chunk's transcript prefix on its own even when the host has AVX-512 (eight chunks per instruction stream otherwise, from 32 chunks on)"},
    {"ROFL_MSM_HOST8", "1", "0 = launches with many problems combine their windows on the device (k_msm_horner) even when the host has AVX-512 IFMA"},
    {"ROFL_MSM_HOST8_MIN", "8", "launches with at least this many problems run their window chains eight per AVX-512 IFMA stream on the host (when the CPU has it)"},
    {"ROFL_MSM_FB_HOST8_MIN", "8", "fixed-base launches with at least this many problems finish eight problems per AVX-512 IFMA task (32 = as in rounds 3-4: one scalar chain per pool task below 32 problems)"},
    {"ROFL_KECCAK_ZMM", "", "host transcripts: 1 = Keccak-f[1600] with one state across five AVX-512 registers, 0 = the scalar rounds; unset = whichever a 50 us measurement at first use finds faster (Intel: the registers, 1.27x; Zen 5: scalar)"},
    {"ROFL_MSM_DEV_HORNER_MIN", "32", "launches with at least this many problems combine their windows on the device"},
    {"ROFL_MSM_T13", "8192", "generic MSMs from this many terms on use 13-bit windows"},
    {"ROFL_MSM_T10", "512 / 2048", "generic MSMs from this many terms on use 10-bit windows (7-bit below, 4-bit below 64); default 2048 for launches with >= 32 problems"},
    {"ROFL_MSM_C", "0", "window width of every generic MSM (4, 7, 10, 13, 16; 0 = by size)"},
    {"ROFL_RED_FUSED_T", "768", "largest block of k_msm_reduce_fused (64 at least: smaller values are raised to one wave)"},
    {"ROFL_ACC_BALANCE", "1", "0 = accumulate blocks in plain descending-load order instead of equal-work blocks"},
    {"ROFL_TRACE", "0", "1 = one line per MSM, window combination, generator fold, table eviction and verifier hashing pass on stderr (which variant ran), 2 = per-phase host timeline of every proof / verification"},
    {"ROFL_DBG_SMALL_TIMELINE", "", "set: per-phase block timings of every fused small-MSM launch on stderr (synchronises; debugging)"},
    {"ROFL_DBG_ACC_TIMELINE", "", "file to append per-wave start / end / placement records of every fixed-base accumulate launch to"},
    {"ROFL_FEMUL_LDS", "0", "rofl_bench_femul: dynamic LDS per block (pins the micro-benchmark's occupancy)"},
    {"ROFL_FEMUL_MODE", "0", "rofl_bench_femul: 0 multiplication chain, 1-3 mixed addition from registers / a 32 KB table / a gathered table"},
    {"ROFL_FEMUL_TABLE", "2097152", "rofl_bench_femul mode 3: table entries (128 B each)"},
};
const char *knob(const char *name) {
#ifndef NDEBUG
    bool known = false; for (const Knob &k : KNOBS) known |= !strcmp(k.name, name);
    if (!known) { fprintf(stderr, "librofl_zk: unregistered knob %s\n", name); abort(); }
#endif
    return getenv(name);
}
static const bool g_keccak_knob_applied = [] { if (const char *e = knob("ROFL_KECCAK_ZMM")) if (*e) keccak_zmm_flag() = atoi(e) != 0 && __builtin_cpu_supports("avx512f"); return true; }();

thread_local std::string g_err;
int fail(int code, const std::string &msg) { g_err = msg; return code; }
std::atomic<uint64_t> g_point_decodes{0};
inline void count_decodes(size_t n) { g_point_decodes.fetch_add((uint64_t)n, std::memory_order_relaxed); }
struct HipErr { hipError_t e; const char *what; };
#define HIPCHK(x) do { hipError_t e__ = (x); if (e__ != hipSuccess) throw HipErr{e__, #x}; } while (0)
#define ROFL_LAUNCH(...) do { (void)hipGetLastError(); hipLaunchKernelGGL(__VA_ARGS__); hipError_t e__ = hipGetLastError(); \
                              if (e__ != hipSuccess && e__ != hipErrorNotReady) throw HipErr{e__, "kernel launch"}; } while (0)

double now_ms() { return std::chrono::duration<double, std::milli>(std::chrono::steady_clock::now().time_since_epoch()).count(); }

sc h_mont(const sc &canon) { return sc_to_mont(canon); }
sc h_canon(const sc &mont) { return sc_from_mont(mont); }
sc h_mul(const sc &a, const sc &b) { return sc_mul_plain(a, b); }
sc h_inv(const sc &canon) { return h_canon(h51::sc_invert_mont_fast(h_mont(canon))); }
bool sc_is_canonical_bytes(const uint8_t *b) { sc s = sc_frombytes(b); return !sc_geq_l(s.v); }

int sc_naf(int8_t out[256], const sc &k) {
    u32 x[9]; for (int i = 0; i < 8; i++) x[i] = k.v[i]; x[8] = 0;
    int top = -1;
    for (int pos = 0; pos < 256; pos++) {
        int d = 0;
        if (x[0] & 1) {
            d = 2 - (int)(x[0] & 3);
            if (d > 0) { x[0] -= 1; }
            else { u64 c = 1; for (int i = 0; i < 9 && c; i++) { c += x[i]; x[i] = (u32)c; c >>= 32; } }
            top = pos;
        }
        out[pos] = (int8_t)d;
        for (int i = 0; i < 8; i++) x[i] = (x[i] >> 1) | (x[i + 1] << 31);
        x[8] >>= 1;
    }
    return top;
}

int wnaf_u64(int16_t out[FOLD_TAB_DIGITS], u64 piece, unsigned w) {
    unsigned __int128 k = piece; int top = -1;
    const int full = 1 << w, half = 1 << (w - 1);
    for (int pos = 0; pos < FOLD_TAB_DIGITS; pos++) {
        int d = 0;
        if (k & 1) { d = (int)(k & (unsigned)(full - 1)); if (d >= half) d -= full; if (d >= 0) k -= (unsigned)d; else k += (unsigned)(-d); top = pos; }
        out[pos] = (int16_t)d; k >>= 1;
    }
    return top;
}

using h51::ge5; using h51::niels5;
struct HostTables { std::vector<niels> B, Bb; std::vector<niels5> B5, Bb5; ge base, bblind; };

void build_fixed_table(std::vector<niels> &tab, ge P) {
    tab.resize(64 * 8);
    for (int w = 0; w < 64; w++) {
        ge acc = P;
        for (int e = 0; e < 8; e++) {
            tab[w * 8 + e] = ge_to_niels(acc);
            acc = ge_add(acc, P);
        }
        for (int k = 0; k < 4; k++) P = ge_double(P);
    }
}
ge5 h_fixed_mul(const std::vector<niels5> &tab, const sc &k_canon) {
    ge5 acc = h51::identity();
    int carry = 0;
    for (int i = 0; i < 64; i++) {
        int v = (int)((k_canon.v[i >> 3] >> ((i & 7) * 4)) & 15) + carry;
        carry = (v + 8) >> 4;
        int d = v - (carry << 4);
        if (d > 0) acc = h51::gmadd(acc, tab[i * 8 + d - 1], false);
        else if (d < 0) acc = h51::gmadd(acc, tab[i * 8 - d - 1], true);
    }
    return acc;
}
void to_tab5(std::vector<niels5> &o, const std::vector<niels> &t) { o.resize(t.size()); for (size_t i = 0; i < t.size(); i++) o[i] = h51::from_niels(t[i]); }
ge h_fixed_mul32(const std::vector<niels> &tab, const sc &k_canon) {
    ge acc = ge_identity();
    int carry = 0;
    for (int i = 0; i < 64; i++) {
        int v = (int)((k_canon.v[i >> 3] >> ((i & 7) * 4)) & 15) + carry;
        carry = (v + 8) >> 4;
        int d = v - (carry << 4);
        if (d > 0) acc = ge_madd(acc, tab[i * 8 + d - 1], false);
        else if (d < 0) acc = ge_madd(acc, tab[i * 8 - d - 1], true);
    }
    return acc;
}

int usable_cores() {
    int n = (int)std::thread::hardware_concurrency(); if (n < 1) n = 1;
    cpu_set_t set; CPU_ZERO(&set);
    if (sched_getaffinity(0, sizeof set, &set) == 0) { int c = CPU_COUNT(&set); if (c > 0 && c < n) n = c; }
    if (FILE *f = fopen("/sys/fs/cgroup/cpu.max", "r")) {
        char q[64]; long per = 0;
        if (fscanf(f, "%63s %ld", q, &per) == 2 && strcmp(q, "max") != 0 && per > 0) { long c = atol(q) / per; if (c >= 1 && c < n) n = (int)c; }
        fclose(f);
    }
    return n;
}
class HostPool {
    std::vector<std::thread> workers; std::mutex mu;
    std::function<void(size_t)> fn; std::atomic<size_t> count{0}, next{0}, done{0}; std::atomic<int> active{0}; std::atomic<uint64_t> gen{0}; std::atomic<bool> stop{false};
    std::unique_ptr<std::atomic<uint32_t>[]> asleep;
    void wake(int w) { if (asleep[w].exchange(0, std::memory_order_seq_cst) == 1) syscall(SYS_futex, reinterpret_cast<uint32_t *>(&asleep[w]), FUTEX_WAKE_PRIVATE, 1, nullptr, nullptr, 0); }
    double spin_us = 400.0;
    std::atomic<uint64_t> hint_seq{0}; std::atomic<double> gap_us{0.0};
    const std::atomic<int> *calls_in_flight = nullptr;
    std::atomic<int> hot{0}; int recent_max = 0, recent_runs = 0;
    std::exception_ptr first_error; std::mutex err_mu;
    void work() {
        struct Active { std::atomic<int> &a; explicit Active(std::atomic<int> &x) : a(x) { a.fetch_add(1); } ~Active() { a.fetch_sub(1); } } guard(active);
        for (;;) {
            size_t i = next.load();
            if (i >= count.load()) break;
            if (!next.compare_exchange_weak(i, i + 1)) continue;
            try { fn(i); } catch (...) { std::lock_guard<std::mutex> lk(err_mu); if (!first_error) first_error = std::current_exception(); }
            done.fetch_add(1);
        }
    }
    void loop(int my_index) {
        uint64_t seen = 0, my_hint = 0;
        for (;;) {
            if (spin_us > 0 && my_index < hot.load(std::memory_order_relaxed) && (!calls_in_flight || calls_in_flight->load(std::memory_order_relaxed) <= 1)) {
                auto t0 = std::chrono::steady_clock::now();
                uint64_t g;
                while ((g = gen.load(std::memory_order_acquire)) == seen) {
                    __builtin_ia32_pause();
                    uint64_t hs = hint_seq.load(std::memory_order_acquire);
                    if (hs != my_hint) {
// ... 697 lines not shown
```

### rofl_project_code_amd/csrc/kernels.hpp

```cpp
#pragma once
#include <type_traits>
#include "fe32.hpp"
#include "fe26.hpp"
#include "quad26.hpp"
#include "fd_dbg.hpp"
#include "keccak.hpp"

namespace rofl {

#define TPB 256

#ifndef ROFL_KGROUP
#define ROFL_KGROUP 0
#endif
#define ROFL_KG(g) (ROFL_KGROUP == 0 || ROFL_KGROUP == (g))

typedef unsigned int v4u __attribute__((ext_vector_type(4)));
typedef __attribute__((address_space(1))) v4u g_uint4;
__device__ __forceinline__ niels gload_niels(const niels *p) {
    niels r;
    const g_uint4 *s = (const g_uint4 *)p;
    v4u *d = reinterpret_cast<v4u *>(&r);
#pragma unroll
    for (int i = 0; i < 6; i++) d[i] = s[i];
// ... 587 lines not shown
        store_sc(&ip_out[((size_t)c * gridDim.x + blockIdx.x) * 2 + 1], v[1]);
    }
}
#endif


#if ROFL_KG(4)
__global__ void __launch_bounds__(TPB) k_ipp_round(u32 n_g, u32 n_k, u32 r_prev, int use_new, ChunkParams *cp, const sc *round_ch, const sc *a_in, const sc *b_in,
                                                   sc *a_out, sc *b_out, size_t ab_stride, const sc *yinvpow, size_t y_stride, sc *SL, sc *ip_out,
                                                   const sc *ptab_in, sc *ptab_out, size_t ptab_stride, sc *ab_host, sc *ip_dev) {
    __shared__ sc lds[TPB * 2];
    __shared__ sc s_u[2];
    u32 c = blockIdx.y;
    if (threadIdx.x == 0) { s_u[0] = load_sc(&round_ch[2 * c]); s_u[1] = load_sc(&round_ch[2 * c + 1]); }
    __syncthreads();
    const sc u = s_u[0], ui = s_u[1];
    if (use_new && blockIdx.x == 0 && threadIdx.x == 0) { store_sc(&cp[c].pend_u[r_prev], u); store_sc(&cp[c].pend_ui[r_prev], ui); }
    const sc *ai = a_in + c * ab_stride, *bi = b_in + c * ab_stride;
    sc *ao = a_out + c * ab_stride, *bo = b_out + c * ab_stride;
    const u32 nh = n_k / 2;
    const sc gs = sc_from_mont(load_sc(&cp[c].gscale)), hs = sc_from_mont(load_sc(&cp[c].hscale));
    sc *sl = SL + (size_t)c * 2 * n_g;
    sc v[2] = {sc_zero(), sc_zero()};
    auto fold2 = [](const sc &x, const sc &cu, const sc &y, const sc &cv) {
        u32 w[17];
#pragma unroll
        for (int q = 0; q < 17; q++) w[q] = 0;
        sc_mac_wide(w, x, cu); sc_mac_wide(w, y, cv);
        return sc_redc_wide(w);
    };
    for (u32 j = blockIdx.x * blockDim.x + threadIdx.x; j < n_g; j += gridDim.x * blockDim.x) {
        u32 h = j / n_k, i = j % n_k;
        bool lo = i < nh; u32 ii = lo ? nh + i : i - nh;
        sc af = fold2(load_sc(&ai[ii]), u, load_sc(&ai[n_k + ii]), ui);
        sc bf = fold2(load_sc(&bi[ii]), ui, load_sc(&bi[n_k + ii]), u);
        u32 hp = use_new ? h >> 1 : h;
        sc tG = r_prev ? load_sc(&ptab_in[(size_t)c * 2 * ptab_stride + hp]) : gs;
        sc tH = r_prev ? load_sc(&ptab_in[(size_t)c * 2 * ptab_stride + ptab_stride + hp]) : hs;
        if (use_new) { bool bit = h & 1; tG = sc_montmul(tG, bit ? u : ui); tH = sc_montmul(tH, bit ? ui : u); }
        if (i == 0) { store_sc(&ptab_out[(size_t)c * 2 * ptab_stride + h], tG); store_sc(&ptab_out[(size_t)c * 2 * ptab_stride + ptab_stride + h], tH); }
        const sc sG = tG, sH = sc_montmul(tH, load_sc(&yinvpow[c * y_stride + j]));
        store_sc(&sl[j], sc_montmul(af, sG));
        store_sc(&sl[n_g + j], sc_montmul(bf, sH));
        if (h == 0) {
            store_sc(&ao[ii], af); store_sc(&bo[ii], bf);
            if (ab_host && n_k == 2) { store_sc(&ab_host[c * 4 + ii], af); store_sc(&ab_host[c * 4 + 2 + ii], bf); }
            if (lo) {
                sc al = fold2(load_sc(&ai[i]), u, load_sc(&ai[n_k + i]), ui);
                sc bl = fold2(load_sc(&bi[i]), ui, load_sc(&bi[n_k + i]), u);
                v[0] = sc_add(v[0], sc_montmul(al, bf));
                v[1] = sc_add(v[1], sc_montmul(af, bl));
            }
        }
    }
    block_sum_sc<2>(v, lds);
    if (threadIdx.x == 0) {
        store_sc(&ip_out[((size_t)c * gridDim.x + blockIdx.x) * 2 + 0], v[0]);
        store_sc(&ip_out[((size_t)c * gridDim.x + blockIdx.x) * 2 + 1], v[1]);
        if (ip_dev) {
            store_sc(&ip_dev[((size_t)c * gridDim.x + blockIdx.x) * 2 + 0], v[0]);
            store_sc(&ip_dev[((size_t)c * gridDim.x + blockIdx.x) * 2 + 1], v[1]);
        }
    }
}
#endif

struct FoldProb { const niels *src; niels *dst; };
#define FOLD_MAXSRC 64
#define FOLD_MAXSEG 4
struct FoldSeg { int lo[FOLD_MAXSEG + 1]; };
#if ROFL_KG(2)
__global__ void __launch_bounds__(256, 4) k_fold_gens(u32 n_new, u32 nsrc, FoldSeg seg, const FoldProb *probs, const int8_t *naf , int unit_first) {
    extern __shared__ __align__(16) unsigned char smem[];
    ge *lds = reinterpret_cast<ge *>(smem);
    u32 q = blockIdx.y;
    u32 i = blockIdx.x * 64 + threadIdx.x;
    u32 k = threadIdx.y, K = blockDim.y;
    bool active = i < n_new;
    const niels *src = probs[q].src;
    const int8_t *dg = naf + (size_t)q * nsrc * 256;
    gd acc = gd_identity();
    if (active) {
        int lo = seg.lo[k], hi = seg.lo[k + 1] - 1;
        for (int bit = hi; bit >= lo; bit--) {
            acc = gd_double(acc);
            for (u32 h = unit_first ? 1 : 0; h < nsrc; h++) {
                int d = dg[h * 256 + bit];
                if (d != 0) acc = gd_madd(acc, gload_nd(&src[(size_t)h * n_new + i]), d < 0);
            }
        }
        for (int t = 0; t < lo; t++) acc = gd_double(acc);
    }
    if (K > 1) {
        if (k > 0) lds[(k - 1) * 64 + threadIdx.x] = gd_pack(acc);
        __syncthreads();
        if (k == 0)
            for (u32 s2 = 1; s2 < K; s2++) acc = gd_add(acc, gd_unpack(lds[(s2 - 1) * 64 + threadIdx.x]));
    }
    if (active && k == 0) {
        if (unit_first) acc = gd_madd(acc, gload_nd(&src[i]), false);
        gstore_niels(&probs[q].dst[i], gd_to_niels(acc));
    }
}
#endif

#if ROFL_KG(2)
__global__ void __launch_bounds__(256, 2) k_fold_gens4(u32 n_new, FoldSeg seg, const FoldProb *probs, const int8_t *naf ) {
    extern __shared__ __align__(16) unsigned char smem[];
    ge *lds = reinterpret_cast<ge *>(smem);
    u32 q = blockIdx.y;
    u32 i = blockIdx.x * 64 + threadIdx.x;
    u32 k = threadIdx.y, K = blockDim.y;
    bool active = i < n_new;
    const niels *src = probs[q].src;
    const int8_t *dg = naf + (size_t)q * 4 * 256;
    gd acc = gd_identity();
    if (active) {
        const nd s1 = gload_nd(&src[(size_t)1 * n_new + i]), s2 = gload_nd(&src[(size_t)2 * n_new + i]), s3 = gload_nd(&src[(size_t)3 * n_new + i]);
        int lo = seg.lo[k], hi = seg.lo[k + 1] - 1;
        for (int bit = hi; bit >= lo; bit--) {
            acc = gd_double(acc);
            int d1 = dg[256 + bit], d2 = dg[512 + bit], d3 = dg[768 + bit];
            if (d1 != 0) acc = gd_madd(acc, s1, d1 < 0);
            if (d2 != 0) acc = gd_madd(acc, s2, d2 < 0);
            if (d3 != 0) acc = gd_madd(acc, s3, d3 < 0);
        }
        for (int t = 0; t < lo; t++) acc = gd_double(acc);
    }
    if (K > 1) {
        if (k > 0) lds[(k - 1) * 64 + threadIdx.x] = gd_pack(acc);
        __syncthreads();
        if (k == 0)
            for (u32 s2i = 1; s2i < K; s2i++) acc = gd_add(acc, gd_unpack(lds[(s2i - 1) * 64 + threadIdx.x]));
    }
    if (active && k == 0) {
        acc = gd_madd(acc, gload_nd(&src[i]), false);
        gstore_niels(&probs[q].dst[i], gd_to_niels(acc));
    }
}
#endif

#define FOLD_TAB_DIGITS 72
struct FoldWProb { const niels *src; niels *dst; u32 tab_off, ev_off, n_ev, seg_start[FOLD_MAXSEG]; };
#define FOLD_EV(bit, h, e, neg) ((u32)(bit) | ((u32)(h) << 9) | ((u32)(e) << 15) | ((u32)(neg) << 27))
#if ROFL_KG(2)
__device__ __forceinline__ void fold_w_body(u32 n_new, const FoldSeg &seg, const FoldWProb *probs, const u32 *events, const niels *tab, size_t tstride, ge *ext_out) {
    extern __shared__ __align__(16) unsigned char smem[];
    ge *lds = reinterpret_cast<ge *>(smem);
    const u32 q = blockIdx.y;
    const u32 i = blockIdx.x * 64 + threadIdx.x;
    const u32 k = threadIdx.y, K = blockDim.y;
    const bool active = i < n_new;
    const niels *src = probs[q].src;
    const u32 *ev = events + probs[q].ev_off;
    gd acc = gd_identity();
    if (active) {
        const niels *tb = tab + probs[q].tab_off;
        auto operand = [&](u32 w) { const u32 h = (w >> 9) & 63u, e = (w >> 15) & 4095u;
                                    const niels *p = e ? tb + (size_t)(e - 1) * tstride : src;
                                    return gload_nd(&p[(size_t)h * n_new + i]); };
        const int lo = seg.lo[k];
        int pos = seg.lo[k + 1];
        u32 j = probs[q].seg_start[k];
        const u32 jend = k == 0 ? probs[q].n_ev : probs[q].seg_start[k - 1];
        if (j < jend) {
            u32 w = ev[j];
            nd nxt = operand(w);
            while (j < jend) {
                const nd cur = nxt; const u32 wc = w;
                j++;
                if (j < jend) { w = ev[j]; nxt = operand(w); }
                const int b = (int)(wc & 511u);
                for (; pos > b; pos--) acc = gd_double(acc);
                acc = gd_madd(acc, cur, (wc >> 27) & 1u);
            }
        }
        for (; pos > lo; pos--) acc = gd_double(acc);
        for (int t = 0; t < lo; t++) acc = gd_double(acc);
    }
    if (K > 1) {
        if (k > 0) lds[(k - 1) * 64 + threadIdx.x] = gd_pack(acc);
        __syncthreads();
        if (k == 0)
            for (u32 s2 = 1; s2 < K; s2++) acc = gd_add(acc, gd_unpack(lds[(s2 - 1) * 64 + threadIdx.x]));
    }
    if (active && k == 0) {
        acc = gd_madd(acc, gload_nd(&src[i]), false);
        if (ext_out) store_gd(&ext_out[(size_t)q * n_new + i], acc);
        else gstore_niels(&probs[q].dst[i], gd_to_niels(acc));
    }
}
__global__ void __launch_bounds__(256, 2) k_fold_gens_w(u32 n_new, FoldSeg seg, const FoldWProb *probs, const u32 *events, const niels *tab, size_t tstride, ge *ext_out) {
    fold_w_body(n_new, seg, probs, events, tab, tstride, ext_out);
}
#endif

#define NB_BATCH 8
#if ROFL_KG(2)
__global__ void __launch_bounds__(TPB) k_niels_batch(u32 count, const ge *ext, niels *out) {
    const u32 t = blockIdx.x * blockDim.x + threadIdx.x;
    const size_t i0 = (size_t)t * NB_BATCH;
    if (i0 >= count) return;
    const u32 nb = (u32)min((size_t)NB_BATCH, (size_t)count - i0);
    fe pre[NB_BATCH];
    fd run = fd_unpack(reinterpret_cast<const fe *>(&ext[i0])[2]);
    pre[0] = fd_pack(run);
#pragma unroll
    for (u32 k = 1; k < NB_BATCH; k++) {
        if (k < nb) { run = fd_mul(run, fd_unpack(reinterpret_cast<const fe *>(&ext[i0 + k])[2])); pre[k] = fd_pack(run); }
    }
    fd inv = fd_invert(run);
#pragma unroll
    for (int k = NB_BATCH - 1; k >= 0; k--) {
        if ((u32)k >= nb) continue;
        const gd p = load_gd(&ext[i0 + k]);
        const fd zi = k ? fd_mul(inv, fd_unpack(pre[k - 1])) : inv;
        if (k) inv = fd_mul(inv, p.Z);
        gstore_niels(&out[i0 + k], gd_to_niels_zinv(p, zi));
    }
}
#endif

struct MsmWin { u32 c, W, wide; };
__device__ __forceinline__ void msm_window(const MsmWin &mw, u32 w, u32 &pos, u32 &width) {
    if (w + 1 == mw.W) { pos = 253 - mw.c; width = mw.c + 1; }
    else if (w < mw.wide) { pos = w * mw.c; width = mw.c; }
    else { pos = mw.wide * mw.c + (w - mw.wide) * (mw.c - 1); width = mw.c - 1; }
}
#if ROFL_KG(2)
__global__ void __launch_bounds__(TPB) k_gens_wtab(u32 total, MsmWin mw, const niels *gens, ndm *wtab, size_t stride) {
    u32 g = blockIdx.x * blockDim.x + threadIdx.x;
    if (g >= total) return;
    niels p0 = load_niels(&gens[g]);
    store_ndm(&wtab[g], p0);
    gd cur = gd_unpack(ge_from_niels(p0));
    u32 at = 0;
    for (u32 w = 1; w < mw.W; w++) {
        u32 pos, wid; msm_window(mw, w, pos, wid);
        for (; at + 1 < pos; at++) cur = gd_double_not(cur);
        for (; at < pos; at++) cur = gd_double(cur);
        store_ndm(&wtab[(size_t)w * stride + g], gd_to_niels(cur));
    }
}
#endif

__device__ __forceinline__ int msm_digit(const sc &k, u32 wpos, u32 c) {
    int pos = (int)wpos - 1;
    u32 need = c + 1;
    u64 bits;
    if (pos < 0) {
        bits = ((u64)k.v[0] | ((u64)k.v[1] << 32)) << 1;
    } else {
        u32 limb = (u32)pos >> 5, off = (u32)pos & 31;
        u64 lo = limb < 8 ? k.v[limb] : 0, mid = limb + 1 < 8 ? k.v[limb + 1] : 0;
        bits = (lo >> off) | (mid << (32 - off));
    }
    u32 x = (u32)(bits & ((1ULL << need) - 1));
    u32 V = x >> 1, bm1 = x & 1, top = (V >> (c - 1)) & 1;
    return (int)(V & ((1u << (c - 1)) - 1)) + (int)bm1 - (int)(top << (c - 1));
}
__device__ __forceinline__ int msm_digit_mem(const u32 *kw, u32 wpos, u32 c) {
// ... 270 lines not shown
    u32 n = bin_cursor[((size_t)pw * L.nbins + bin) * 2], n2 = bin_cursor[((size_t)pw * L.nbins + bin) * 2 + 1];
    size_t rbase = ((size_t)pw * L.nbins + bin) * L.cap_bin;
    if (n > L.cap_bin || n2 > MSM_BIN_TAIL || n + n2 > L.cap_bin) {
        if (threadIdx.x == 0) *(volatile u32 *)overflow = 1u;
        for (u32 f = threadIdx.x; f < (1u << L.fbits); f += blockDim.x) {
            size_t bi = (size_t)pw * B + (size_t)bin * (1u << L.fbits) + f;
            cnt[bi] = 0; off[bi] = (u32)rbase;
        }
        return;
    }
    u32 *reg = bins + rbase;
    const u32 *tl = tails + ((size_t)pw * L.nbins + bin) * MSM_BIN_TAIL;
    const u32 fmask = FBK - 1, keep = ~(fmask << L.ebits), emask = (1u << L.ebits) - 1;
    auto key = [&](u32 v) { u32 f = (v >> L.ebits) & fmask; if (wps <= 1) return f; u32 ws = (v & emask) >> wshift; return f * wps + (ws < wps ? ws : wps - 1); };
    for (u32 f = threadIdx.x; f < FB; f += blockDim.x) hist[f] = 0;
    __syncthreads();
    for (u32 j = threadIdx.x; j < n + n2; j += blockDim.x) atomicAdd(&hist[key(j < n ? reg[j] : tl[j - n])], 1u);
    __syncthreads();
    if (threadIdx.x < 64) {
        u32 per = (FB + 63) / 64, lo = threadIdx.x * per, sum = 0;
        for (u32 f = lo; f < lo + per && f < FB; f++) sum += hist[f];
        u32 incl = sum;
        for (u32 dlt = 1; dlt < 64; dlt <<= 1) { u32 v = __shfl_up(incl, dlt); if (threadIdx.x >= dlt) incl += v; }
        u32 run = incl - sum;
        for (u32 f = lo; f < lo + per && f < FB; f++) { ofs[f] = run; run += hist[f]; }
    }
    __syncthreads();
    for (u32 f = threadIdx.x; f < FBK; f += blockDim.x) {
        size_t bi = (size_t)pw * B + (size_t)bin * FBK + f;
        u32 tot = 0; for (u32 q = 0; q < wps; q++) tot += hist[f * wps + q];
        cnt[bi] = tot;
        off[bi] = (u32)(rbase + ofs[f * wps]);
    }
    __syncthreads();
    for (u32 j = threadIdx.x; j < n + n2; j += blockDim.x) {
        u32 v = j < n ? reg[j] : tl[j - n];
        u32 pos = atomicAdd(&ofs[key(v)], 1u);
        out[pos] = v & keep;
    }
    __syncthreads();
    for (u32 j = threadIdx.x; j < n + n2; j += blockDim.x) reg[j] = out[j];
}
#endif
#if ROFL_KG(1)
__global__ void k_msm_overflow(u32 W, u32 B, u32 pstep, const MsmProb *probs, const u32 *ovf_count, const MsmOvf *ovf, u32 ovf_max, ge *buckets, int fb) {
    if (blockIdx.x) return;
    u32 cnt = *ovf_count; if (cnt > ovf_max) cnt = ovf_max;
    for (u32 o = 0; o < cnt; o++) {
        u32 bi = ovf[o].bucket, v = ovf[o].entry, p = bi / (W * B) * pstep;
        if ((bi & 63u) != threadIdx.x) continue;
        gd acc = load_gd(&buckets[bi]);
        u32 idx = v & 0x7fffffffu;
        acc = gd_madd(acc, fb ? gload_ndm(reinterpret_cast<const ndm *>(probs[p].pts) + idx) : gload_nd(&probs[p].pts[idx]), (v >> 31) != 0);
        store_gd(&buckets[bi], acc);
    }
}
#endif
template <bool FB> __device__ __forceinline__ void msm_accumulate_body(u32 n, u32 c, u32 W, u32 pstep, const MsmProb *probs, const u32 *cnt, const u32 *off,
                                 const u32 *sorted, const u32 *perm, ge *buckets, u32 cap, u32 balance) {
    u32 p = blockIdx.y, B = 1u << (c - 1);
    u32 t = blockIdx.x * blockDim.x + threadIdx.x;
    if ((balance & 2u) && B >= TPB) {
        const u32 nbs = B / TPB, lin = blockIdx.y * gridDim.x + blockIdx.x, per_set = nbs * gridDim.y;
        const u32 ws = lin / per_set, rem = lin - ws * per_set;
        p = rem / nbs;
        t = ws * B + (rem - p * nbs) * TPB + threadIdx.x;
    }
    if (t >= W * B) return;
    u32 w = t / B;
    if ((balance & 1u) && B >= 1024) {
        u32 tb = t & (B - 1), nw = B / 64, j = tb / TPB, k = (tb / 64) & 3;
        u32 sw = k == 0 ? j : k == 1 ? nw - 1 - j : k == 2 ? nw / 2 - 1 - j : nw / 2 + j;
        t = w * B + sw * 64 + (tb & 63);
    }
    size_t bi = ((size_t)p * W + w) * B + perm[(size_t)p * W * B + t];
    u32 num = cnt[bi];
    const u32 *lst;
    if (cap == MSM_LIST_ABS) lst = sorted + off[bi];
    else if (cap) { lst = sorted + bi * cap; if (num > cap) num = cap; }
    else lst = sorted + ((size_t)p * W + w) * n * 2 + off[bi];
    const niels *pts = probs[p * pstep].pts;
    gd acc = gd_identity();
    u32 vnext = num ? lst[0] : 0u;
    for (u32 e = 0; e < num; e++) {
        u32 v = vnext;
        if (e + 1 < num) vnext = lst[e + 1];
        u32 idx = v & 0x7fffffffu;
        acc = gd_madd(acc, FB ? gload_ndm(reinterpret_cast<const ndm *>(pts) + idx) : gload_nd(&pts[idx]), (v >> 31) != 0);
    }
    store_gd(&buckets[bi], acc);
}
#if ROFL_KG(1)
__global__ void __launch_bounds__(TPB) k_msm_accumulate_fb(u32 n, u32 c, u32 W, u32 pstep, const MsmProb *probs, const u32 *cnt, const u32 *off,
                                 const u32 *sorted, const u32 *perm, ge *buckets, u32 cap, u32 balance) {
    msm_accumulate_body<true>(n, c, W, pstep, probs, cnt, off, sorted, perm, buckets, cap, balance);
}
#endif
#if ROFL_KG(1)
__global__ void __launch_bounds__(TPB) k_msm_accumulate_fb_dbg(u32 n, u32 c, u32 W, u32 pstep, const MsmProb *probs, const u32 *cnt, const u32 *off,
                                 const u32 *sorted, const u32 *perm, ge *buckets, u32 cap, u32 balance, unsigned long long *rec) {
    unsigned long long t0 = wall_clock64();
    msm_accumulate_body<true>(n, c, W, pstep, probs, cnt, off, sorted, perm, buckets, cap, balance);
    unsigned long long t1 = wall_clock64();
    if ((threadIdx.x & 63) == 0) {
        u32 hw, xcc;
        asm volatile("s_getreg_b32 %0, hwreg(HW_REG_HW_ID)" : "=s"(hw));
        asm volatile("s_getreg_b32 %0, hwreg(HW_REG_XCC_ID)" : "=s"(xcc));
        size_t wv = ((size_t)blockIdx.y * gridDim.x + blockIdx.x) * (TPB / 64) + threadIdx.x / 64;
        rec[wv * 4 + 0] = t0; rec[wv * 4 + 1] = t1; rec[wv * 4 + 2] = hw; rec[wv * 4 + 3] = xcc;
    }
}
#endif
#if ROFL_KG(1)
__global__ void __launch_bounds__(TPB) k_msm_accumulate_gen(u32 n, u32 c, u32 W, u32 pstep, const MsmProb *probs, const u32 *cnt, const u32 *off,
                                 const u32 *sorted, const u32 *perm, ge *buckets, u32 cap, u32 balance) {
    msm_accumulate_body<false>(n, c, W, pstep, probs, cnt, off, sorted, perm, buckets, cap, balance);
}
#endif
__device__ __forceinline__ void msm_reduce_item(u32 E, u32 nb, const ge *S_in, const ge *C_in, ge *S_out, ge *C_out, u32 item) {
    u32 E8 = E / 8, role = item / E8, g = item % E8;
    if (role == 0) {
        const ge *s = S_in + (size_t)g * 8;
        gd p0 = load_gd(&s[0]), p1 = load_gd(&s[1]);
        gd q0 = gd_add(p0, p1); gd D0 = p1;
        p0 = load_gd(&s[2]); p1 = load_gd(&s[3]);
        gd q1 = gd_add(p0, p1); D0 = gd_add(D0, p1);
        p0 = load_gd(&s[4]); p1 = load_gd(&s[5]);
        gd q2 = gd_add(p0, p1); D0 = gd_add(D0, p1);
        p0 = load_gd(&s[6]); p1 = load_gd(&s[7]);
        gd q3 = gd_add(p0, p1); D0 = gd_add(D0, p1);
        store_gd(&C_out[(size_t)(nb + 0) * E8 + g], D0);
        gd D1 = gd_add(q1, q3);
        store_gd(&C_out[(size_t)(nb + 1) * E8 + g], D1);
        gd r1 = gd_add(q2, q3);
        store_gd(&C_out[(size_t)(nb + 2) * E8 + g], r1);
        gd S = gd_add(gd_add(q0, q1), r1);
        store_gd(&S_out[g], S);
    } else {
        const ge *s = C_in + (size_t)(role - 1) * E + (size_t)g * 8;
        gd acc = gd_add(load_gd(&s[0]), load_gd(&s[1]));
#pragma unroll 1
        for (int k = 2; k < 8; k++) acc = gd_add(acc, load_gd(&s[k]));
        store_gd(&C_out[(size_t)(role - 1) * E8 + g], acc);
    }
}
__device__ __forceinline__ void msm_reduce_item_split(u32 E, u32 nb, const ge *S_in, const ge *C_in, ge *S_out, ge *C_out, u32 item) {
    u32 E8 = E / 8, role = item / E8, g = item % E8;
    if (role >= 4) {
        const ge *cs = C_in + (size_t)(role - 4) * E + (size_t)g * 8;
        gd acc = gd_add(load_gd(&cs[0]), load_gd(&cs[1]));
#pragma unroll 1
        for (int t = 2; t < 8; t++) acc = gd_add(acc, load_gd(&cs[t]));
        store_gd(&C_out[(size_t)(role - 4) * E8 + g], acc);
        return;
    }
    const ge *s = S_in + (size_t)g * 8;
    if (role == 0) {
        gd acc = gd_add(load_gd(&s[0]), load_gd(&s[1]));
#pragma unroll 1
        for (int t = 2; t < 8; t++) acc = gd_add(acc, load_gd(&s[t]));
        store_gd(&S_out[g], acc);
    } else {
        u32 b = role - 1, st = 1u << b;
        u32 i0 = st, i1 = b == 2 ? 5 : 3, i2 = b == 0 ? 5 : 6, i3 = 7;
        gd acc = gd_add(load_gd(&s[i0]), load_gd(&s[i1]));
        acc = gd_add(acc, load_gd(&s[i2]));
        acc = gd_add(acc, load_gd(&s[i3]));
        store_gd(&C_out[(size_t)(nb + b) * E8 + g], acc);
    }
}
#if ROFL_KG(1)
// ... 154 lines not shown
    while (Ecur > G) { msm_binary_level_inplace(Ecur, nb, buf); Ecur /= 2; nb += 1; }
    for (u32 item = threadIdx.x; item < gv * (1 + nb); item += blockDim.x) {
        const u32 g = item / (1 + nb), l = item % (1 + nb);
        if (l == 0) store_ge(&fin_s[g], buf[g]);
        else if (l - 1 < nb_final) store_ge(&fin_c[(size_t)g * nb_final + (l - 1)], buf[(size_t)G + (size_t)(l - 1) * G + g]);
    }
}
#define MSM_SMALL_CAP 64
#define MSM_SMALL_CAP_MAX 80
#if ROFL_KG(1)
template <bool L16>
__device__ __forceinline__ void msm_small_body(unsigned char *smem, u32 n_side, MsmWin mw, MsmMap mm, const MsmProb *probs, ge *buckets, ge *S_fin, ge *C_fin,
                                               u32 nb_final, u32 *overflow, u32 cap, u32 G, unsigned long long *dbg, ge *wsum_out,
                                               const sc *ip_dev, u32 ip_nblk, const niels *qpts) {
    auto stamp = [&](int k) { if (dbg && threadIdx.x == 0) dbg[(size_t)blockIdx.x * 4 + k] = wall_clock64(); };
    stamp(0);
    const u32 B = 1u << (mw.c - 1);
    const u32 Wg = (mw.W + G - 1) / G;
    const u32 p = G > 1 ? blockIdx.x / Wg : blockIdx.x / mw.W, w0 = G > 1 ? (blockIdx.x % Wg) * G : blockIdx.x % mw.W;
    const u32 gv = min(G, mw.W - w0);
    const u32 pw = p * mw.W + w0;
    const u32 VB = G * B;
    u32 side = mm.lr_nh ? (p & 1u) : 0u;
    typedef typename std::conditional<L16, unsigned short, u32>::type lst_t;
    const u32 SIGN = L16 ? 0x8000u : 0x80000000u, IDXM = SIGN - 1;
    u32 *lcnt = reinterpret_cast<u32 *>(smem);
    lst_t *lst = reinterpret_cast<lst_t *>(lcnt + VB);
    for (u32 b = threadIdx.x; b < VB; b += blockDim.x) lcnt[b] = 0;
    __syncthreads();
    const sc *scal = probs[p].scal;
    auto put = [&](const u32 *kw, u32 g, u32 entry_idx) {
        u32 wpos, wwid; msm_window(mw, w0 + g, wpos, wwid);
        int d = msm_digit_mem(kw, wpos, wwid);
        u32 ad = (u32)(d < 0 ? -d : d), entry = entry_idx | (d < 0 ? SIGN : 0u);
        for (int rep = 0; rep < 2; rep++) {
            u32 a1 = rep == 0 ? (ad > B ? B : 0u) : (ad > B ? ad - B : ad);
            if (!a1) continue;
            u32 vb = g * B + a1 - 1;
            u32 pos = atomicAdd(&lcnt[vb], 1u);
            if (pos < cap) lst[vb * cap + pos] = (lst_t)entry;
            else *(volatile u32 *)overflow = 1u;
        }
    };
    for (u32 k = threadIdx.x; k < n_side; k += blockDim.x) {
        u32 i = mm.lr_nh ? msm_side_term(mm, side, k) : k;
        const u32 *kw = reinterpret_cast<const u32 *>(&scal[i]);
        for (u32 g = 0; g < gv; g++) put(kw, g, i);
    }
    const u32 QIDX = IDXM;
    if (ip_dev && threadIdx.x == 0) {
        sc acc = sc_zero();
        for (u32 b = 0; b < ip_nblk; b++) acc = sc_add(acc, load_sc(&ip_dev[((size_t)(p >> 1) * ip_nblk + b) * 2 + (p & 1u)]));
        sc cs = sc_from_mont(acc);
        for (u32 g = 0; g < gv; g++) put(reinterpret_cast<const u32 *>(&cs), g, QIDX);
    }
    __syncthreads();
    stamp(1);
    const niels *pts = probs[p].pts;
    const niels *qpt = qpts ? qpts + (p >> 1) : pts;
    auto fetch = [&](u32 v) { const u32 i = v & IDXM; return gload_nd(i == QIDX ? qpt : &pts[i]); };
    u32 my_b = threadIdx.x;
    const bool sorted = (blockDim.x == 512 && B == 512) || G > 1;
    if (sorted) {
        __shared__ u32 chist[MSM_SMALL_CAP_MAX + 2], cbase[MSM_SMALL_CAP_MAX + 2];
        __shared__ unsigned short order[512];
        if (threadIdx.x < MSM_SMALL_CAP_MAX + 2) chist[threadIdx.x] = 0;
        __syncthreads();
        u32 mycnt = lcnt[threadIdx.x]; if (mycnt > cap) mycnt = cap;
        u32 rank_in = atomicAdd(&chist[mycnt], 1u);
        __syncthreads();
        if (threadIdx.x == 0) { u32 run = 0; for (int cval = (int)cap; cval >= 0; cval--) { cbase[cval] = run; run += chist[cval]; } }
        __syncthreads();
        order[cbase[mycnt] + rank_in] = (unsigned short)threadIdx.x;
        __syncthreads();
        u32 wv = threadIdx.x >> 6, ln = threadIdx.x & 63;
        u32 grp = G > 1 ? (wv + blockIdx.x) % G : (wv < 4 ? wv : 11 - wv);
        my_b = order[grp * 64 + ln];
    }
    for (u32 vb = my_b; vb < VB; vb += blockDim.x) {
        u32 num = lcnt[vb]; if (num > cap) num = cap;
        gd acc = gd_identity();
        u32 v = num ? lst[vb * cap] : 0u;
        nd nxt = fetch(v);
        for (u32 e = 0; e < num; e++) {
            nd q = nxt; bool ng = (v & SIGN) != 0;
            if (e + 1 < num) { v = lst[vb * cap + e + 1]; nxt = fetch(v); }
            acc = gd_madd(acc, q, ng);
        }
        if (vb < gv * B) store_gd(&buckets[(size_t)pw * B + vb], acc);
    }
    __threadfence_block();
    __syncthreads();
    stamp(2);
    if (G > 1) msm_reduce_binary_multi(B, G, gv, buckets + (size_t)pw * B, S_fin + pw, C_fin + (size_t)pw * nb_final, nb_final, smem);
    else if (B >= 16) msm_reduce_binary_body(B, buckets + (size_t)pw * B, S_fin + pw, C_fin + (size_t)pw * nb_final, smem);
    else msm_reduce_fused_body(B, 0, buckets + (size_t)pw * B, nullptr, S_fin + pw, C_fin + (size_t)pw * nb_final, smem);
    stamp(3);
    if (wsum_out) {
        __threadfence_block();
        __syncthreads();
        if (threadIdx.x < 4 * gv) {
            const u32 q = threadIdx.x & 3, g = threadIdx.x >> 2;
            auto coord = [&](const ge *pt) { gq r; r.v = fd_unpack(reinterpret_cast<const fe *>(pt)[q]); return r; };
            const ge *cf = C_fin + (size_t)(pw + g) * nb_final;
            gq acc = coord(&cf[nb_final - 1]);
#pragma unroll 1
            for (int l = (int)nb_final - 2; l >= 0; l--) acc = gq_add(gq_double(acc, q), coord(&cf[l]), q);
            acc = gq_add(acc, coord(&S_fin[pw + g]), q);
            reinterpret_cast<fe *>(&wsum_out[pw + g])[q] = fd_pack(acc.v);
        }
    }
}
__global__ void __launch_bounds__(512) k_msm_small(u32 n_side, MsmWin mw, MsmMap mm, const MsmProb *probs, ge *buckets, ge *S_fin, ge *C_fin,
                                                   u32 nb_final, u32 *overflow, u32 cap, u32 G, unsigned long long *dbg, ge *wsum_out,
                                                   const sc *ip_dev, u32 ip_nblk, const niels *qpts) {
    extern __shared__ __align__(16) unsigned char smem[];
    msm_small_body<false>(smem, n_side, mw, mm, probs, buckets, S_fin, C_fin, nb_final, overflow, cap, G, dbg, wsum_out, ip_dev, ip_nblk, qpts);
}
__global__ void __launch_bounds__(256, 4) k_msm_small_g(u32 n_side, MsmWin mw, MsmMap mm, const MsmProb *probs, ge *buckets, ge *S_fin, ge *C_fin,
                                                        u32 nb_final, u32 *overflow, u32 cap, u32 G, unsigned long long *dbg, ge *wsum_out,
                                                        const sc *ip_dev, u32 ip_nblk, const niels *qpts) {
    extern __shared__ __align__(16) unsigned char smem[];
    msm_small_body<true>(smem, n_side, mw, mm, probs, buckets, S_fin, C_fin, nb_final, overflow, cap, G, dbg, wsum_out, ip_dev, ip_nblk, qpts);
}
#endif

#if ROFL_KG(1)
__global__ void __launch_bounds__(256) k_msm_horner(MsmWin mw, const ge *S_fin, const ge *C_fin, u32 nb, ge *out) {
    __shared__ ge sh[64];
    const u32 p = blockIdx.x, w = threadIdx.x >> 2, q = threadIdx.x & 3;
    auto coord = [&](const ge *pt) { gq r; r.v = fd_unpack(reinterpret_cast<const fe *>(pt)[q]); return r; };
    gq acc;
    if (w < mw.W) {
        size_t pw = (size_t)p * mw.W + w;
        acc = coord(&C_fin[pw * nb + nb - 1]);
#pragma unroll 1
        for (int l = (int)nb - 2; l >= 0; l--) acc = gq_add(gq_double(acc, q), coord(&C_fin[pw * nb + l]), q);
        acc = gq_add(acc, coord(&S_fin[pw]), q);
        u32 pos, wid; msm_window(mw, w, pos, wid);
#pragma unroll 1
        for (u32 i = 0; i < pos; i++) acc = gq_double(acc, q);
        reinterpret_cast<fe *>(&sh[w])[q] = fd_pack(acc.v);
    }
    __syncthreads();
#pragma unroll 1
    for (u32 s = 32; s >= 1; s >>= 1) {
        if (w < s && w + s < mw.W) {
            acc = gq_add(acc, coord(&sh[w + s]), q);
            reinterpret_cast<fe *>(&sh[w])[q] = fd_pack(acc.v);
        }
        __syncthreads();
    }
    if (w == 0) reinterpret_cast<fe *>(&out[p])[q] = fd_pack(acc.v);
}
#endif

#if ROFL_KG(1)
__global__ void __launch_bounds__(256) k_msm_wsum(u32 PW, const ge *S_fin, const ge *C_fin, u32 nb, ge *out) {
    const u32 pw = (blockIdx.x * blockDim.x + threadIdx.x) >> 2, q = threadIdx.x & 3;
    if (pw >= PW) return;
    auto coord = [&](const ge *pt) { gq r; r.v = fd_unpack(reinterpret_cast<const fe *>(pt)[q]); return r; };
    gq acc = coord(&C_fin[(size_t)pw * nb + nb - 1]);
#pragma unroll 1
    for (int l = (int)nb - 2; l >= 0; l--) acc = gq_add(gq_double(acc, q), coord(&C_fin[(size_t)pw * nb + l]), q);
    acc = gq_add(acc, coord(&S_fin[pw]), q);
    reinterpret_cast<fe *>(&out[pw])[q] = fd_pack(acc.v);
}
#endif

#if ROFL_KG(4)
__global__ void __launch_bounds__(TPB) k_dbg_quad(u32 pairs, u32 doublings, const uint8_t *in , uint8_t *out_serial, uint8_t *out_quad, u32 *status) {
    u32 t = blockIdx.x * blockDim.x + threadIdx.x;
    u32 i = t >> 2, q = t & 3;
    if (i >= pairs) return;
    __align__(16) uint8_t b[64];
    for (int k = 0; k < 64; k++) b[k] = in[(size_t)i * 64 + k];
    gd P, Q;
    if (!gd_ristretto_decode(P, b) || !gd_ristretto_decode(Q, b + 32)) { atomicOr(status, 4u); return; }
    gq a = gq_from_gd(P, q), c = gq_from_gd(Q, q);
    for (u32 k = 0; k < doublings; k++) a = gq_double(a, q);
    a = gq_add(a, c, q);
    gd R = gq_to_gd(a);
    if (q == 0) {
        gd_ristretto_encode(out_quad + (size_t)i * 32, R);
        gd S = P;
        for (u32 k = 0; k < doublings; k++) S = gd_double(S);
        S = gd_add(S, Q);
        gd_ristretto_encode(out_serial + (size_t)i * 32, S);
    }
}
__global__ void __launch_bounds__(TPB) k_dbg_fd(u32 op, u32 n, const u32 *in , u32 *out ) {
    const u32 t = blockIdx.x * blockDim.x + threadIdx.x;
    if (op < FD_DBG_THREAD_OPS) {
        if (t < n) fd_dbg_apply(op, in + (size_t)t * FD_DBG_IN, out + (size_t)t * FD_DBG_OUT);
        return;
    }
    const u32 i = t >> 2, q = t & 3;
    if (i >= n) return;
    const u32 *ci = in + (size_t)i * FD_DBG_IN; u32 *co = out + (size_t)i * FD_DBG_OUT;
    const gd P = gd_dbg_load(ci, 0), Q = gd_dbg_load(ci, 4);
    const gq a = gq_from_gd(P, q);
    const gq r = op == FD_DBG_GQ_DOUBLE ? gq_double(a, q) : gq_add(a, gq_from_gd(Q, q), q);
    const gd R = gq_to_gd(r);
    if (q == 0) {
        gd_dbg_store(co, 0, R);
        gd_dbg_store(co, 4, op == FD_DBG_GQ_DOUBLE ? gd_double(P) : gd_add(P, Q));
    }
}
__global__ void __launch_bounds__(TPB) k_dbg_sc(u32 op, u32 n, const u32 *in , u32 *out ) {
    const u32 t = blockIdx.x * blockDim.x + threadIdx.x;
    if (t >= n) return;
    const u32 *ci = in + (size_t)t * SC_DBG_IN;
    const sc r = op == SC_DBG_LOAD_REDUCED ? load_sc_reduced(reinterpret_cast<const sc *>(ci)) : sc_dbg_apply(op, ci);
    store_sc(reinterpret_cast<sc *>(out + (size_t)t * SC_DBG_OUT), r);
}
#endif

__device__ __forceinline__ bool gd_load_decode(gd &p, const uint8_t *src) {
    __align__(16) uint8_t b[32];
    reinterpret_cast<uint4 *>(b)[0] = reinterpret_cast<const uint4 *>(src)[0]; reinterpret_cast<uint4 *>(b)[1] = reinterpret_cast<const uint4 *>(src)[1];
    return gd_ristretto_decode(p, b);
}
#if ROFL_KG(4)
__global__ void __launch_bounds__(TPB) k_decode(u32 count, u32 valid_count, const uint8_t *in, const niels *shift, niels *out_niels,
                         uint8_t *out_enc, u32 *status) {
    u32 i = blockIdx.x * blockDim.x + threadIdx.x;
    if (i >= count) return;
    {
        const size_t y = blockIdx.y;
        in += y * count * 32; status += y;
        if (out_niels) out_niels += y * count;
        if (out_enc) out_enc += y * count * 32;
    }
    if (i >= valid_count) {
        if (out_niels) store_niels(&out_niels[i], niels_identity());
        if (out_enc) { uint4 z = make_uint4(0, 0, 0, 0); reinterpret_cast<uint4 *>(out_enc + (size_t)i * 32)[0] = z; reinterpret_cast<uint4 *>(out_enc + (size_t)i * 32)[1] = z; }
        return;
    }
    gd p;
    if (!gd_load_decode(p, in + (size_t)i * 32)) { atomicOr(status, 4u); p = gd_identity(); }
    if (out_niels) { niels r; r.ypx = fd_pack(fd_add(p.Y, p.X)); r.ymx = fd_pack(fd_sub(p.Y, p.X)); r.t2d = fd_pack(fd_mul(p.T, fd_d2())); store_niels(&out_niels[i], r); }
    if (shift) p = gd_madd(p, load_nd(shift), false);
    if (out_enc) gd_ristretto_encode(out_enc + (size_t)i * 32, p);
}
#endif
#if ROFL_KG(4)
__global__ void __launch_bounds__(TPB) k_add_points(u32 count, const uint8_t *a, const uint8_t *b, uint8_t *out, u32 *status) {
    u32 i = blockIdx.x * blockDim.x + threadIdx.x;
    if (i >= count) return;
    gd p, q;
    if (!gd_ristretto_decode(p, a + (size_t)i * 32)) { atomicOr(status, 4u); p = gd_identity(); }
    if (!gd_ristretto_decode(q, b + (size_t)i * 32)) { atomicOr(status, 4u); q = gd_identity(); }
    gd_ristretto_encode(out + (size_t)i * 32, gd_add(p, q));
}
#endif
#if ROFL_KG(4)
__global__ void __launch_bounds__(TPB) k_verify_scalars(u32 n, u32 m, u32 lgN, const uint2 *grp, const ChunkParams *cp, const PowTabs *pt, const sc *two_pow, sc *out) {
    u32 gidx = blockIdx.y;
    const u32 first = grp[gidx].x, group = grp[gidx].y;
    size_t N = (size_t)n * m;
    u32 k = blockIdx.x * blockDim.x + threadIdx.x;
    if (k >= N) return;
    u32 j = k / n, i = k % n;
    sc gacc = sc_zero(), hacc = sc_zero();
    for (u32 cc = 0; cc < group; cc++) {
        const ChunkParams &P = cp[first + cc];
        const PowTabs &T = pt[first + cc];
        u32 kc = ~k;
        sc s = sc_montmul(sc_montmul(load_sc(&T.s[0][k & (PT_E - 1)]), load_sc(&T.s[1][(k >> PT_W) & (PT_E - 1)])), load_sc(&T.s[2][(k >> (2 * PT_W)) & (PT_E - 1)]));
        sc sinv = sc_montmul(sc_montmul(load_sc(&T.s[0][kc & (PT_E - 1)]), load_sc(&T.s[1][(kc >> PT_W) & (PT_E - 1)])), load_sc(&T.s[2][(kc >> (2 * PT_W)) & (PT_E - 1)]));
        for (u32 q = 0; q + 3 * PT_W < lgN; q++) {
            bool bit = (k >> (lgN - 1 - q)) & 1;
            s = sc_montmul(s, bit ? P.u[q] : P.uinv[q]);
            sinv = sc_montmul(sinv, bit ? P.uinv[q] : P.u[q]);
        }
        sc g = sc_neg(sc_add(P.rz, sc_montmul(P.ra, s)));
        sc zj2 = sc_montmul(sc_montmul(P.rzz, pt_pow(T.z, P.zpow2, j)), two_pow[i]);
        sc h = sc_add(P.rz, sc_montmul(pt_pow(T.yinv, P.yinvpow2, k), sc_sub(zj2, sc_montmul(P.rb, sinv))));
        gacc = sc_add(gacc, g); hacc = sc_add(hacc, h);
    }
    sc *o = out + (size_t)gidx * 2 * N;
    store_sc(&o[k], sc_from_mont(gacc));
    store_sc(&o[N + k], sc_from_mont(hacc));
}
#endif
struct VTabs { sc s0[PT_E], s1[PT_E], s2[PT_E], q0[PT_E], q1[PT_E], q2[PT_E], w0[PT_E], w1[PT_E], w2[PT_E], zi[64]; };
#define VS_TP 8
#if ROFL_KG(4)
__global__ void __launch_bounds__(256) k_vtabs(const ChunkParams *cp, const PowTabs *pt, const sc *two_pow, VTabs *vt, u32 n, u32 lgn) {
    const u32 c = blockIdx.y, t = blockIdx.x * blockDim.x + threadIdx.x;
// ... 877 lines not shown
```

### rofl_project_code_amd/csrc/rofl_zk.hip

```cpp
#include <hip/hip_runtime.h>
#include <rccl/rccl.h>
#include <dlfcn.h>
#include <immintrin.h>
#include <chrono>
#include <time.h>
#include <sched.h>
#include <unistd.h>
#include <sys/syscall.h>
#include <linux/futex.h>
#include <cmath>
#include <cstdio>
#include <cstdlib>
#include <map>
#include <memory>
#include <atomic>
#include <condition_variable>
#include <deque>
#include <exception>
#include <functional>
#include <mutex>
#include <shared_mutex>
#include <thread>
#include <string>
#include <vector>
// ... 2488 lines not shown
int rofl_get_l2_clip_bounds(size_t range, unsigned fp_bits, unsigned fp_frac, float *out) {
    if (!valid_fp(fp_bits, fp_frac) || range == 0 || range > 127) return fail(ROFL_BAD_PARAM, "bad parameter");
    *out = l2_clip_bound(range, fp_bits, fp_frac); return ROFL_OK;
}

int rofl_dbg_msm(const uint8_t *scalars32, const uint8_t *points32, size_t n, uint8_t out32[32]) {
    return guarded([&]() -> int {
        LaneLock lane_lock = acquire_lane(); Ctx &C = *lane_lock.c;
        if (n == 0) return fail(ROFL_BAD_PARAM, "bad parameter");
        C.init();
        std::vector<sc> hs(n);
        for (size_t i = 0; i < n; i++) { hs[i] = sc_frombytes(scalars32 + 32 * i); if (sc_geq_l(hs[i].v)) hs[i] = sc_from_mont(sc_to_mont(hs[i])); }
        uint8_t *dp = C.tmp_in.as<uint8_t>(n * 32); niels *dn = C.aux_pts.as<niels>(n); sc *ds = C.aux_scal.as<sc>(n);
        u32 *status = C.status.as<u32>(4);
        HIPCHK(hipMemsetAsync(status, 0, 16, C.stream));
        C.up(dp, points32, n * 32, C.stream);
        C.up(ds, hs.data(), n * 32, C.stream);
        count_decodes(n);
        ROFL_LAUNCH(k_decode, grid1(n), dim3(TPB), 0, C.stream, (u32)n, (u32)n, dp, (const niels *)nullptr, dn, (uint8_t *)nullptr, status);
        u32 st = 0;
        HIPCHK(hipMemcpyAsync(&st, status, 4, hipMemcpyDeviceToHost, C.stream));
        C.sync();
        if (st & 4u) return fail(ROFL_FORMAT_ERROR, "invalid Ristretto encoding");
        std::vector<MsmProb> pr(1, MsmProb{dn, ds}); std::vector<ge5> res;
        msm_run(C, pr, n, res);
        h51::encode(out32, res[0]);
        return ROFL_OK;
    });
}
int rofl_dbg_verify_labelled(const uint8_t *label, size_t label_len, size_t gens_capacity, const uint8_t *proof, size_t proof_len,
                             const uint8_t *commits32, size_t m, size_t n_bits, const uint8_t verifier_seed[32], int *ok_out) {
    return guarded([&]() -> int {
        LaneLock lane_lock = acquire_lane(false, true); Ctx &C = *lane_lock.c;
        if (!label || !label_len || label_len > 255 || !proof || !commits32 || !m || !is_pow2(m) || !verifier_seed || !ok_out) return fail(ROFL_BAD_PARAM, "bad parameter");
        *ok_out = 0;
        std::string lbl((const char *)label, label_len);
        if (lbl.find('\0') != std::string::npos) return fail(ROFL_BAD_PARAM, "the label holds a NUL byte");
        C.init();
        timing_begin(C);
        uint8_t *d_in = C.Cbytes.as<uint8_t>(m * 32), *d_enc = C.Vbytes.as<uint8_t>(m * 32);
        niels *d_vn = C.gbuf[0].as<niels>(m);
        u32 *status = C.status.as<u32>(4);
        HIPCHK(hipMemsetAsync(status, 0, 16, C.stream));
        C.up(d_in, commits32, m * 32, C.stream);
        count_decodes(m);
        ROFL_LAUNCH(k_decode, grid1(m), dim3(TPB), 0, C.stream, (u32)m, (u32)m, d_in, (const niels *)nullptr, d_vn, d_enc, status);
        std::vector<uint8_t> hV(m * 32); u32 *h_st = C.h_misc.as<u32>(4);
        uint8_t *hp = C.h_V.as<uint8_t>(m * 32);
        HIPCHK(hipMemcpyAsync(hp, d_enc, m * 32, hipMemcpyDeviceToHost, C.stream));
        HIPCHK(hipMemcpyAsync(h_st, status, 4, hipMemcpyDeviceToHost, C.stream));
        C.sync();
        if (h_st[0] & 4u) { timing_end(C); return fail(ROFL_FORMAT_ERROR, "commitment is not a valid Ristretto encoding"); }
        u64 cidx = 0; int ok = 0;
        int rc = verify_chunks(C, lbl.c_str(), gens_capacity, 1, n_bits, m, proof, proof_len, hp, d_vn, verifier_seed, &cidx, &ok);
        timing_end(C);
        if (rc) return fail(rc, "proof rejected before verification (format / bitsize / generator capacity)");
        *ok_out = ok;
        return ROFL_OK;
    });
}
int rofl_dbg_msm_retries(uint64_t out[4]) { if (!out) return ROFL_BAD_PARAM; for (int i = 0; i < 4; i++) out[i] = g_msm_stat[i].load(); return ROFL_OK; }
int rofl_dbg_quad_ops(const uint8_t *pairs64, size_t pairs, unsigned doublings, uint8_t *out_serial32, uint8_t *out_quad32) {
    return guarded([&]() -> int {
        LaneLock lane_lock = acquire_lane(); Ctx &C = *lane_lock.c;
        if (pairs == 0) return fail(ROFL_BAD_PARAM, "bad parameter");
        C.init();
        uint8_t *din = C.tmp_in.as<uint8_t>(pairs * 64), *dout = C.tmp_out.as<uint8_t>(pairs * 64);
        u32 *status = C.status.as<u32>(4);
        HIPCHK(hipMemsetAsync(status, 0, 16, C.stream));
        HIPCHK(hipMemsetAsync(dout, 0, pairs * 64, C.stream));
        C.up(din, pairs64, pairs * 64, C.stream);
        ROFL_LAUNCH(k_dbg_quad, grid1(pairs * 4), dim3(TPB), 0, C.stream, (u32)pairs, doublings, (const uint8_t *)din, dout, dout + pairs * 32, status);
        u32 st = 0;
        HIPCHK(hipMemcpyAsync(&st, status, 4, hipMemcpyDeviceToHost, C.stream));
        C.down(out_serial32, dout, pairs * 32, C.stream);
        C.down(out_quad32, dout + pairs * 32, pairs * 32, C.stream);
        C.sync();
        if (st & 4u) return fail(ROFL_FORMAT_ERROR, "invalid Ristretto encoding");
        return ROFL_OK;
    });
}
static int dbg_ops_device(bool scalar_field, unsigned op, size_t n, const uint32_t *in, uint32_t *out) {
    const size_t in_words = scalar_field ? SC_DBG_IN : FD_DBG_IN, out_words = scalar_field ? SC_DBG_OUT : FD_DBG_OUT;
    if (op >= (unsigned)(scalar_field ? SC_DBG_OPS : FD_DBG_OPS)) return fail(ROFL_BAD_PARAM, "bad parameter");
    return guarded([&]() -> int {
        LaneLock lane_lock = acquire_lane(); Ctx &C = *lane_lock.c;
        if (n == 0 || n > (1u << 20) || !in || !out) return fail(ROFL_BAD_PARAM, "bad parameter");
        C.init();
        u32 *din = C.tmp_in.as<u32>(n * in_words), *dout = C.tmp_out.as<u32>(n * out_words);
        C.up(din, in, n * in_words * 4, C.stream);
        C.up(dout, out, n * out_words * 4, C.stream);
        if (scalar_field) ROFL_LAUNCH(k_dbg_sc, grid1(n), dim3(TPB), 0, C.stream, (u32)op, (u32)n, (const u32 *)din, dout);
        else ROFL_LAUNCH(k_dbg_fd, grid1(op < FD_DBG_THREAD_OPS ? n : n * 4), dim3(TPB), 0, C.stream, (u32)op, (u32)n, (const u32 *)din, dout);
        C.down(out, dout, n * out_words * 4, C.stream);
        C.sync();
        return ROFL_OK;
    });
}
int rofl_dbg_fd_ops(unsigned op, size_t n, const uint32_t *in, uint32_t *out) { return dbg_ops_device(false, op, n, in, out); }
int rofl_dbg_sc_ops(unsigned op, size_t n, const uint32_t *in, uint32_t *out) { return dbg_ops_device(true, op, n, in, out); }
int rofl_dbg_quantize(unsigned site, size_t rows, size_t d, size_t dpad, size_t prove_range, unsigned fp_bits, unsigned fp_frac,
                      const float *values, const uint8_t *blindings32, void *out, float *terms_out, uint32_t *status_out) {
    if (site > 2 || !valid_fp(fp_bits, fp_frac) || rows == 0 || d == 0 || !values || !out) return fail(ROFL_BAD_PARAM, "bad parameter");
    if (site != 0) dpad = d;
    if (dpad < d || rows > (1u << 20) || dpad > (1u << 20) || rows * dpad > (1u << 20)) return fail(ROFL_BAD_PARAM, "bad parameter");
    if (site == 0 && (prove_range == 0 || prove_range > fp_bits || !status_out)) return fail(ROFL_BAD_PARAM, "bad parameter");
    if (site == 1 && (prove_range == 0 || prove_range > 128 || !blindings32 || !terms_out || !status_out)) return fail(ROFL_BAD_PARAM, "bad parameter");
    return guarded([&]() -> int {
        LaneLock lane_lock = acquire_lane(); Ctx &C = *lane_lock.c;
        C.init();
        const size_t n = rows * d;
        float *dv = C.vals.as<float>(n + 1);
        u32 *status = C.status.as<u32>(rows + 4);
        HIPCHK(hipMemsetAsync(status, 0, 4 * (rows + 4), C.stream));
        C.up(dv, values, 4 * n, C.stream);
        float mn = 0, mx = 0; if (site != 2) clip_bounds(prove_range, fp_bits, fp_frac, &mn, &mx);
        if (site == 0) {
            u64 *vshift = C.vshift.as<u64>(rows * dpad);
            HIPCHK(hipMemsetAsync(vshift, 0xff, 8 * rows * dpad, C.stream));
            ROFL_LAUNCH(k_quantize_shift, grid1(dpad, (u32)rows), dim3(TPB), 0, C.stream, dv, (u32)d, (u32)dpad, (u32)prove_range, fp_bits, fp_frac, mn, mx, vshift, status);
            C.down(out, vshift, 8 * rows * dpad, C.stream);
        } else if (site == 1) {
            const u32 nblk = l2_sum_blocks(d);
            float *dterms = C.tmp_out.as<float>(n);
            sc *dbl = C.blind.as<sc>(n), *part_bl = C.tmp_in2.as<sc>(rows * nblk), *dsums = C.aux_scal.as<sc>(2 * rows);
            u64 *part_sq = C.tmp_in.as<u64>(rows * nblk * 3);
            C.up(dbl, blindings32, 32 * n, C.stream);
            ROFL_LAUNCH(k_l2_sumsq_batch, dim3(nblk, (unsigned)rows), dim3(TPB), 0, C.stream, (u32)d, fp_bits, fp_frac, mn, mx, (const float *)dv, (const sc *)dbl, dterms, part_sq, part_bl, status);
            ROFL_LAUNCH(k_l2_sumsq_combine, dim3((unsigned)((rows + 63) / 64)), dim3(64), 0, C.stream, (u32)rows, nblk, (const u64 *)part_sq, (const sc *)part_bl, dsums);
            C.down(terms_out, dterms, 4 * n, C.stream);
            C.down(out, dsums, sizeof(sc) * 2 * rows, C.stream);
        } else {
            sc *ds = C.aux_scal.as<sc>(n);
            ROFL_LAUNCH(k_dbg_quant, grid1(n), dim3(TPB), 0, C.stream, (u32)n, fp_bits, fp_frac, (const float *)dv, ds);
            C.down(out, ds, sizeof(sc) * n, C.stream);
        }
        if (site != 2) C.down(status_out, status, 4 * rows, C.stream);
        C.sync();
        return ROFL_OK;
    });
}
int rofl_discrete_log_vec(const uint8_t *points32, size_t d, size_t table_size, unsigned bsgs_bits, uint8_t *scalars_out32) {
    return guarded([&]() -> int {
        LaneLock lane_lock = acquire_lane(true); Ctx &C = *lane_lock.c;
        if (table_size == 0 || table_size >= (1u << 30) || !(bsgs_bits == 8 || bsgs_bits == 16 || bsgs_bits == 32)) return fail(ROFL_BAD_PARAM, "bad parameter");
        if (d == 0) return ROFL_OK;
        C.init();
        timing_begin(C);
        uint8_t *dp = C.tmp_in.as<uint8_t>(d * 32), *dout = C.Cbytes.as<uint8_t>(d * 32);
        u32 *status = C.status.as<u32>(4);
        HIPCHK(hipMemsetAsync(status, 0, 16, C.stream));
        C.up(dp, points32, 32 * d, C.stream);
        bsgs_solve_launch(C, d, dp, table_size, bsgs_bits, dout, status);
        u32 st = 0;
        C.down(scalars_out32, dout, 32 * d, C.stream);
        HIPCHK(hipMemcpyAsync(&st, status, 4, hipMemcpyDeviceToHost, C.stream));
        C.sync();
        timing_end(C);
        if (st & 4u) return fail(ROFL_FORMAT_ERROR, "invalid Ristretto encoding");
        if (st & 8u) return fail(ROFL_BAD_PARAM, "discrete log not found (the reference unwraps None)");
        return ROFL_OK;
    });
}
int rofl_acc_create(size_t d, int init, uint64_t *handle_out) {
    if (!handle_out || d == 0 || (init != 0 && init != 1)) return fail(ROFL_BAD_PARAM, "bad parameter");
    if (d >= ((size_t)1 << 31)) return fail(ROFL_BAD_PARAM, "accumulator too large");
    auto A = std::make_shared<Acc>();
    A->d = d; A->init = init; A->device = current_device();
    DeviceBinding bind(A->device);
    int rc = guarded([&]() -> int {
        LaneLock lane_lock = acquire_lane(); Ctx &C = *lane_lock.c;
        C.init();
        HIPCHK(hipMalloc(&A->sum, sizeof(ge) * 2 * d));
        acc_reset_launch(C, *A);
        C.sync();
        return ROFL_OK;
    });
    if (rc) { if (A->sum) (void)hipFree(A->sum); return rc; }
    *handle_out = g_accs.add(A);
    return ROFL_OK;
}
int rofl_acc_add(uint64_t h, size_t n_clients, const uint8_t *const *records, const size_t *d_each, size_t stride) {
// ... 629 lines not shown
    }
    if (us_simd) *us_simd = (t2 - t1) * 1e3;
    if (us_scalar) *us_scalar = (t1 - t0) * 1e3;
    return bad;
}
int rofl_dbg_last_hops(double out[10]) { if (!out) return fail(ROFL_BAD_PARAM, "bad parameter"); memcpy(out, g_last_hops, sizeof g_last_hops); return ROFL_OK; }
int rofl_dbg_host_fe_mul(const uint8_t a[32], const uint8_t b[32], uint8_t out[32]) { fe_tobytes(out, fe_mul(fe_frombytes(a), fe_frombytes(b))); return 0; }
int rofl_dbg_host_fe_ops(const uint8_t a[32], const uint8_t b[32], uint8_t oa[32], uint8_t os[32], uint8_t oq[32], uint8_t oi[32]) {
    fe x = fe_frombytes(a), y = fe_frombytes(b);
    fe_tobytes(oa, fe_add(x, y)); fe_tobytes(os, fe_sub(x, y)); fe_tobytes(oq, fe_sq(x)); fe_tobytes(oi, fe_invert(x)); return 0;
}
int rofl_dbg_host_sc_invert(const uint8_t a[32], uint8_t out_ref[32], uint8_t out_fast[32], double *ns_ref, double *ns_fast) {
    sc am = h_mont(sc_frombytes(a));
    sc r1 = sc_invert_mont(am), r2 = h51::sc_invert_mont_fast(am);
    sc_tobytes(out_ref, h_canon(r1)); sc_tobytes(out_fast, h_canon(r2));
    if (ns_ref && ns_fast) {
        const int reps = 200; volatile u32 sink = 0;
        double t0 = now_ms(); for (int i = 0; i < reps; i++) { am.v[0] ^= (u32)i; sink += sc_invert_mont(am).v[0]; } double t1 = now_ms();
        for (int i = 0; i < reps; i++) { am.v[0] ^= (u32)i; sink += h51::sc_invert_mont_fast(am).v[0]; } double t2 = now_ms();
        *ns_ref = (t1 - t0) * 1e6 / reps; *ns_fast = (t2 - t1) * 1e6 / reps; (void)sink;
    }
    return 0;
}
int rofl_dbg_host_sc_mul(const uint8_t a[32], const uint8_t b[32], uint8_t out[32]) { sc_tobytes(out, h_mul(sc_frombytes(a), sc_frombytes(b))); return 0; }
int rofl_dbg_host_sc_lazy(const uint8_t *a32, const uint8_t *b32, size_t count, uint8_t out_lazy[32], uint8_t out_ref[32]) {
    if (count > 16) return ROFL_BAD_PARAM;
    u32 acc[17]; for (int i = 0; i < 17; i++) acc[i] = 0;
    sc ref = sc_zero();
    for (size_t k = 0; k < count; k++) {
        const sc a = sc_frombytes(a32 + 32 * k), b = sc_frombytes(b32 + 32 * k);
        sc_mac_wide(acc, a, b);
        ref = sc_add(ref, sc_montmul(a, b));
    }
    sc_tobytes(out_lazy, sc_redc_wide(acc)); sc_tobytes(out_ref, ref);
    return 0;
}
int rofl_dbg_host_sc_wide_mont(const uint8_t in[64], uint8_t out[32]) { sc_tobytes(out, sc_from_mont(sc_from_wide_mont(sc_frombytes(in), sc_frombytes(in + 32)))); return 0; }
int rofl_dbg_host_sc_wide(const uint8_t in[64], uint8_t out[32]) { sc_tobytes(out, sc_from_wide(sc_frombytes(in), sc_frombytes(in + 32))); return 0; }
int rofl_dbg_host_from_uniform(const uint8_t in[64], uint8_t out[32]) { ristretto_encode(out, ristretto_from_uniform(in)); return 0; }
int rofl_dbg_host_scalarmult_base(const uint8_t k[32], int use_bb, uint8_t out[32]) {
    static HostTables ht; static bool init = false; static std::mutex mu;
    std::lock_guard<std::mutex> lk(mu);
    if (!init) {
        static const uint8_t Bc[32] = {0xe2, 0xf2, 0xae, 0x0a, 0x6a, 0xbc, 0x4e, 0x71, 0xa8, 0x84, 0xa9, 0x61, 0xc5, 0x00, 0x51, 0x5f,
                                       0x58, 0xe3, 0x0b, 0x6a, 0xa5, 0x82, 0xdd, 0x8d, 0xb6, 0xa6, 0x59, 0x45, 0xe0, 0x8d, 0x2d, 0x76};
        ristretto_decode(ht.base, Bc); uint8_t h[64]; sha3_512(h, Bc, 32); ht.bblind = ristretto_from_uniform(h);
        build_fixed_table(ht.B, ht.base); build_fixed_table(ht.Bb, ht.bblind); init = true;
    }
    if (use_bb & 2) { to_tab5(ht.B5, ht.B); to_tab5(ht.Bb5, ht.Bb); h51::encode(out, h_fixed_mul((use_bb & 1) ? ht.Bb5 : ht.B5, sc_frombytes(k))); return 0; }
    ristretto_encode(out, h_fixed_mul32((use_bb & 1) ? ht.Bb : ht.B, sc_frombytes(k))); return 0;
}
int rofl_dbg_host_fd_ops(const uint8_t a[32], const uint8_t b[32], uint8_t om[32], uint8_t oq[32], uint8_t oa[32], uint8_t os[32], uint8_t oi[32]) {
    fe fa = fe_frombytes(a), fb = fe_frombytes(b);
    fa.v[7] |= (u32)(a[31] & 0x80) << 24; fb.v[7] |= (u32)(b[31] & 0x80) << 24;
    fd x = fd_unpack(fa), y = fd_unpack(fb);
    fe_tobytes(om, fd_pack(fd_mul(fd_sub(fd_add(x, x), x), fd_add(y, fd_zero()))));
    fe_tobytes(oq, fd_pack(fd_sq(x))); fe_tobytes(oa, fd_pack(fd_add(x, y))); fe_tobytes(os, fd_pack(fd_sub(x, y)));
    fe_tobytes(oi, fd_pack(fd_invert(x)));
    return 0;
}
int rofl_dbg_host_fd_scalarmult(const uint8_t k[32], const uint8_t p[32], uint8_t out[32]) {
    ge P; if (!ristretto_decode(P, p)) return ROFL_FORMAT_ERROR;
    nd q = nd_unpack(ge_to_niels(P));
    sc s = sc_frombytes(k);
    if (sc_geq_l(s.v)) s = sc_from_mont(sc_to_mont(s));
    int8_t naf[256]; int top = sc_naf(naf, s);
    gd acc = gd_identity();
    for (int i = top; i >= 0; i--) { acc = gd_double(acc); if (naf[i]) acc = gd_madd(acc, q, naf[i] < 0); }
    gd twice = gd_add(acc, acc);
    gd back = gd_madd(twice, nd_unpack(gd_to_niels(acc)), true);
    ristretto_encode(out, gd_pack(back));
    return 0;
}
int rofl_dbg_host_fd_codec(const uint8_t in[32], uint8_t out[32]) {
    gd p; if (!gd_ristretto_decode(p, in)) return ROFL_FORMAT_ERROR;
    gd q = gd_add(gd_double(p), gd_madd(gd_identity(), nd_unpack(gd_to_niels(p)), true));
    gd_ristretto_encode(out, q); return 0;
}
int rofl_dbg_host_fd_ops_raw(unsigned op, size_t n, const uint32_t *in, uint32_t *out) {
    if (op >= FD_DBG_THREAD_OPS || !in || !out) return ROFL_BAD_PARAM;
    for (size_t i = 0; i < n; i++) fd_dbg_apply(op, in + i * FD_DBG_IN, out + i * FD_DBG_OUT);
    return 0;
}
int rofl_dbg_host_sc_ops(unsigned op, size_t n, const uint32_t *in, uint32_t *out) {
    if (op >= SC_DBG_OPS || !in || !out) return ROFL_BAD_PARAM;
    for (size_t i = 0; i < n; i++) { const sc r = sc_dbg_apply(op, in + i * SC_DBG_IN); for (int k = 0; k < 8; k++) out[i * SC_DBG_OUT + k] = r.v[k]; }
    return 0;
}
int rofl_dbg_host_decode_encode(const uint8_t in[32], uint8_t out[32]) { ge p; if (!ristretto_decode(p, in)) return ROFL_FORMAT_ERROR; ristretto_encode(out, ge_add(p, ge_identity())); return 0; }
int rofl_dbg_host_merlin(const uint8_t *label, size_t label_len, const uint8_t *msg, size_t msg_len, uint8_t out[64]) {
    Merlin t((const char *)label, label_len); t.append("msg", msg, msg_len); t.challenge_bytes("chal", out, 64); return 0;
}
int rofl_dbg_host_nonce(const uint8_t seed[32], uint64_t idx, uint8_t out[32]) {
    const u64 dom[2] = ROFL_NONCE_DOM;
    u64 sd[4]; memcpy(sd, seed, 32); u64 st[25]; shake256_seeded_block(st, dom, sd, idx >> 1);
    const int h = (int)(idx & 1);
    sc lo, hi; for (int i = 0; i < 4; i++) { lo.v[2 * i] = (u32)st[8 * h + i]; lo.v[2 * i + 1] = (u32)(st[8 * h + i] >> 32); hi.v[2 * i] = (u32)st[8 * h + 4 + i]; hi.v[2 * i + 1] = (u32)(st[8 * h + 4 + i] >> 32); }
    sc_tobytes(out, sc_from_wide(lo, hi)); return 0;
}
int rofl_dbg_host_blind(const uint8_t seed[32], uint64_t idx, uint8_t out[32]) {
    const u64 dom[2] = ROFL_BLIND_DOM;
    u64 sd[4]; memcpy(sd, seed, 32); u64 st[25]; shake256_seeded_block(st, dom, sd, idx >> 1);
    sc_tobytes(out, xof_block_scalar(st, (int)(idx & 1))); return 0;
}

}
```

Measured before the change: 1.173 million.

## Skip unused T coordinate in fold doublings/madds and seed buckets from first point

Extended-coordinate doublings and mixed additions gain an option to skip computing T whenever the next operation is another doubling, which never reads T. The fold kernels track, per bit, whether T is needed and pass that flag. MSM bucket accumulation starts from the first point converted directly to extended form instead of adding it to the identity. Fold segment balancing is updated for the reduced doubling cost. Debug entry points and op-count accounting are added alongside; the risk is correctness if a skipped T is later read.

```diff
diff --git a/include/rofl_zk_debug.h b/include/rofl_zk_debug.h
--- a/include/rofl_zk_debug.h
+++ b/include/rofl_zk_debug.h
@@ -37,11 +37,14 @@
 int rofl_bench_femul(unsigned iters, double *fe_mul_per_sec_out);
 int rofl_dbg_quad_ops(const uint8_t *pairs64, size_t pairs, unsigned doublings, uint8_t *out_serial32, uint8_t *out_quad32);
 int rofl_dbg_fd_ops(unsigned op, size_t n, const uint32_t *in, uint32_t *out);
+int rofl_dbg_fd_ops_ext(unsigned op, size_t n, const uint32_t *in, uint32_t *out);
+int rofl_dbg_fold(unsigned nsrc, unsigned K, const uint8_t *scalars32, const uint8_t *points32, size_t n_new, uint8_t *out32);
 int rofl_dbg_sc_ops(unsigned op, size_t n, const uint32_t *in, uint32_t *out);
 int rofl_dbg_quantize(unsigned site, size_t rows, size_t d, size_t dpad, size_t prove_range, unsigned fp_bits, unsigned fp_frac,
                       const float *values, const uint8_t *blindings32, void *out, float *terms_out, uint32_t *status_out);
 
 int rofl_dbg_host_fd_ops_raw(unsigned op, size_t n, const uint32_t *in, uint32_t *out);
+int rofl_dbg_host_fd_ops_ext(unsigned op, size_t n, const uint32_t *in, uint32_t *out);
 int rofl_dbg_host_sc_ops(unsigned op, size_t n, const uint32_t *in, uint32_t *out);
 int rofl_dbg_host_pool_stress(unsigned threads, unsigned jobs);
 int rofl_dbg_host_fe_mul(const uint8_t a[32], const uint8_t b[32], uint8_t out[32]);
diff --git a/rofl_project_code_amd/csrc/fd_dbg.hpp b/rofl_project_code_amd/csrc/fd_dbg.hpp
--- a/rofl_project_code_amd/csrc/fd_dbg.hpp
+++ b/rofl_project_code_amd/csrc/fd_dbg.hpp
@@ -9,7 +9,8 @@
        FD_DBG_MUL_LOOSE = 8, FD_DBG_SQ_LOOSE = 9, FD_DBG_INVERT = 10, FD_DBG_POW22523 = 11, FD_DBG_SQRT_RATIO = 12, FD_DBG_ABS = 13,
        FD_DBG_PRED = 14, FD_DBG_MADD = 15, FD_DBG_MSUB = 16, FD_DBG_GD_ADD = 17, FD_DBG_GD_DOUBLE = 18, FD_DBG_GD_DOUBLE_NOT = 19,
        FD_DBG_TO_NIELS = 20, FD_DBG_TO_NIELS_ZINV = 21, FD_DBG_THREAD_OPS = 22,
-       FD_DBG_GQ_DOUBLE = 22, FD_DBG_GQ_ADD = 23, FD_DBG_OPS = 24 };
+       FD_DBG_GQ_DOUBLE = 22, FD_DBG_GQ_ADD = 23, FD_DBG_OPS = 24,
+       FD_DBG_MADD_NOT = 24, FD_DBG_MSUB_NOT = 25, FD_DBG_GD_DOUBLE_FLAG_NOT = 26, FD_DBG_FROM_ND = 27, FD_DBG_FROM_ND_NEG = 28, FD_DBG_OPS_EXT = 29 };
 
 HD fd fd_dbg_load(const u32 *in, int k) {
     fd r;
@@ -70,6 +71,23 @@
     }
 }
 
+HDN inline void fd_dbg_apply_ext(u32 op, const u32 *in, u32 *out) {
+    switch (op) {
+    case FD_DBG_MADD_NOT: case FD_DBG_MSUB_NOT: {
+        nd q; q.ypx = fd_dbg_load(in, 4); q.ymx = fd_dbg_load(in, 5); q.t2d = fd_dbg_load(in, 6);
+        gd_dbg_store(out, 0, gd_madd(gd_dbg_load(in, 0), q, op == FD_DBG_MSUB_NOT, in[79] != 0));
+        break;
+    }
+    case FD_DBG_GD_DOUBLE_FLAG_NOT: gd_dbg_store(out, 0, gd_double(gd_dbg_load(in, 0), in[79] != 0)); break;
+    case FD_DBG_FROM_ND: case FD_DBG_FROM_ND_NEG: {
+        nd q; q.ypx = fd_dbg_load(in, 0); q.ymx = fd_dbg_load(in, 1); q.t2d = fd_dbg_load(in, 2);
+        gd_dbg_store(out, 0, gd_from_nd(q, op == FD_DBG_FROM_ND_NEG));
+        break;
+    }
+    default: break;
+    }
+}
+
 #define SC_DBG_IN 264
 #define SC_DBG_OUT 8
 enum { SC_DBG_MONTMUL = 0, SC_DBG_TO_MONT = 1, SC_DBG_FROM_MONT = 2, SC_DBG_MUL_PLAIN = 3, SC_DBG_ADD = 4, SC_DBG_NEG = 5, SC_DBG_SUB = 6,
diff --git a/rofl_project_code_amd/csrc/fe26.hpp b/rofl_project_code_amd/csrc/fe26.hpp
--- a/rofl_project_code_amd/csrc/fe26.hpp
+++ b/rofl_project_code_amd/csrc/fe26.hpp
@@ -174,12 +174,17 @@
     return r;
 }
 
+HD fd fd_dinv() {
+    fd r = {{0x1c9f843u, 0x03c9db3u, 0x285c4bcu, 0x0c213cau, 0x02d775au, 0x1b9cf66u, 0x3108a66u, 0x1c86562u, 0x1214d5cu, 0x10241fbu}};
+    return r;
+}
+
 HD gd gd_identity() { gd r; r.X = fd_zero(); r.Y = fd_one(); r.Z = fd_one(); r.T = fd_zero(); return r; }
 HD gd gd_unpack(const ge &p) { gd r; r.X = fd_unpack(p.X); r.Y = fd_unpack(p.Y); r.Z = fd_unpack(p.Z); r.T = fd_unpack(p.T); return r; }
 HD ge gd_pack(const gd &p) { ge r; r.X = fd_pack(p.X); r.Y = fd_pack(p.Y); r.Z = fd_pack(p.Z); r.T = fd_pack(p.T); return r; }
 HD nd nd_unpack(const niels &q) { nd r; r.ypx = fd_unpack(q.ypx); r.ymx = fd_unpack(q.ymx); r.t2d = fd_unpack(q.t2d); return r; }
 
-HD gd gd_madd(const gd &p, const nd &q, bool neg) {
+HD gd gd_madd(const gd &p, const nd &q, bool neg, bool with_t = true) {
     fd a_f = fd_select(q.ymx, q.ypx, neg), b_f = fd_select(q.ypx, q.ymx, neg);
     fd A = fd_mul(fd_sub(p.Y, p.X), a_f);
     fd B = fd_mul(fd_add(p.Y, p.X), b_f);
@@ -193,8 +198,17 @@
     fd XG = fd_select(Gsm, Fbig, neg);
     r.X = fd_mul(XF, E);
     r.Y = fd_mul(XG, H);
-    r.T = fd_mul(E, H);
     r.Z = fd_mul(Fbig, Gsm);
+    if (with_t) r.T = fd_mul(E, H); else r.T = p.T;
+    return r;
+}
+HD gd gd_from_nd(const nd &q, bool neg) {
+    gd r;
+    r.X = fd_carry(fd_sub(fd_select(q.ypx, q.ymx, neg), fd_select(q.ymx, q.ypx, neg)));
+    r.Y = fd_carry(fd_add(q.ypx, q.ymx));
+    r.Z = fd_zero(); r.Z.v[0] = 2;
+    fd T = fd_mul(q.t2d, fd_dinv());
+    r.T = fd_select(T, fd_carry(fd_neg(T)), neg);
     return r;
 }
 HD gd gd_add(const gd &p, const gd &q) {
@@ -207,7 +221,7 @@
     gd r; r.X = fd_mul(F, E); r.Y = fd_mul(G, H); r.T = fd_mul(E, H); r.Z = fd_mul(F, G);
     return r;
 }
-HD gd gd_double(const gd &p) {
+HD gd gd_double(const gd &p, bool with_t = true) {
     fd XX = fd_sq(p.X), YY = fd_sq(p.Y), ZZ = fd_sq(p.Z);
     fd ZZ2 = fd_add(ZZ, ZZ);
     fd S = fd_sq(fd_add(p.X, p.Y));
@@ -215,20 +229,11 @@
     fd cZ = fd_carry(fd_sub(YY, XX));
     fd cX = fd_sub(S, cY);
     fd cT = fd_sub(ZZ2, cZ);
-    gd r; r.X = fd_mul(cT, cX); r.Y = fd_mul(cY, cZ); r.Z = fd_mul(cT, cZ); r.T = fd_mul(cX, cY);
-    return r;
-}
-HD gd gd_double_not(const gd &p) {
-    fd XX = fd_sq(p.X), YY = fd_sq(p.Y), ZZ = fd_sq(p.Z);
-    fd ZZ2 = fd_add(ZZ, ZZ);
-    fd S = fd_sq(fd_add(p.X, p.Y));
-    fd cY = fd_carry(fd_add(YY, XX));
-    fd cZ = fd_carry(fd_sub(YY, XX));
-    fd cX = fd_sub(S, cY);
-    fd cT = fd_sub(ZZ2, cZ);
-    gd r; r.X = fd_mul(cT, cX); r.Y = fd_mul(cY, cZ); r.Z = fd_mul(cT, cZ); r.T = p.T;
-    return r;
-}
+    gd r; r.X = fd_mul(cT, cX); r.Y = fd_mul(cY, cZ); r.Z = fd_mul(cT, cZ);
+    if (with_t) r.T = fd_mul(cX, cY); else r.T = p.T;
+    return r;
+}
+HD gd gd_double_not(const gd &p) { return gd_double(p, false); }
 HDN inline niels gd_to_niels_zinv(const gd &p, const fd &zi) {
     fd x = fd_mul(p.X, zi), y = fd_mul(p.Y, zi);
     niels r;
diff --git a/rofl_project_code_amd/csrc/host_msm.hpp b/rofl_project_code_amd/csrc/host_msm.hpp
--- a/rofl_project_code_amd/csrc/host_msm.hpp
+++ b/rofl_project_code_amd/csrc/host_msm.hpp
@@ -30,6 +30,11 @@
     bool fb() const { return kind == MsmKind::FixedBase; }
 };
 static const u32 MSM_OVF_MAX = 4096;
+static inline uint64_t msm_acc_muls(uint64_t entries, uint64_t buckets) {
+    if (!entries || !buckets) return entries * 7;
+    const double nonempty = (double)buckets * (1.0 - std::exp(-(double)entries / (double)buckets));
+    return entries * 7 - (uint64_t)(6.0 * std::min(nonempty, (double)entries));
+}
 
 static inline u32 msm_bin_cap(size_t avg) {
     static const int sigmas = knob("ROFL_MSM_BIN_SIGMA") ? atoi(knob("ROFL_MSM_BIN_SIGMA")) : 8;
@@ -138,7 +143,7 @@
         size_t lds_red = G > 1 ? ((size_t)G * P.B * 3 / 4 + 1) * sizeof(ge)
                                : std::max(((size_t)(P.B / 8) * 4 + (size_t)(P.B / 16) * 5 + 1) * sizeof(ge), ((size_t)P.B + (size_t)P.B * 3 / 4 + 1) * sizeof(ge));
         uint64_t items = (uint64_t)np * n_side * P.W;
-        KSpan ks(C.tm, st, ROFL_TK_MSM_SMALL, items * 7 + (uint64_t)PW * P.B * 10, (uint64_t)np * n_side * (32 + 96));
+        KSpan ks(C.tm, st, ROFL_TK_MSM_SMALL, msm_acc_muls(items, (uint64_t)PW * P.B) + (uint64_t)PW * P.B * 10, (uint64_t)np * n_side * (32 + 96));
         static const bool small_tl = knob("ROFL_DBG_SMALL_TIMELINE") != nullptr;
         unsigned long long *tl_dev = nullptr;
         if (small_tl) { HIPCHK(hipMalloc(&tl_dev, PW * 32)); HIPCHK(hipMemsetAsync(tl_dev, 0, PW * 32, st)); }
@@ -199,7 +204,7 @@
         ROFL_LAUNCH(k_msm_scan, dim3((unsigned)PW), dim3(P.B >= 1024 ? 1024 : 256), 0, st, P.B, cnt, off, (u32 *)nullptr, perm);
         if (C.tm.enabled) { e0 = C.tm.get(); e1 = C.tm.get(); HIPCHK(hipEventRecord(e0, st)); }
         {
-            KSpan ks_acc(C.tm, st, ROFL_TK_MSM_ACCUMULATE_FB, terms * P.W * 7, terms * 32);
+            KSpan ks_acc(C.tm, st, ROFL_TK_MSM_ACCUMULATE_FB, msm_acc_muls(terms * P.W, (uint64_t)PW * P.B), terms * 32);
             static const char *timeline = knob("ROFL_DBG_ACC_TIMELINE");
             if (timeline) {
                 dim3 g = grid1((size_t)Wb * P.B, (u32)nq);
@@ -238,7 +243,7 @@
         if (C.tm.enabled) { e0 = C.tm.get(); e1 = C.tm.get(); HIPCHK(hipEventRecord(e0, st)); }
         {
             uint64_t acc_adds = terms * P.W;
-            KSpan ks_acc(C.tm, st, fb ? ROFL_TK_MSM_ACCUMULATE_FB : ROFL_TK_MSM_ACCUMULATE_GEN, acc_adds * 7, terms * 32);
+            KSpan ks_acc(C.tm, st, fb ? ROFL_TK_MSM_ACCUMULATE_FB : ROFL_TK_MSM_ACCUMULATE_GEN, msm_acc_muls(acc_adds, (uint64_t)PW * P.B), terms * 32);
             if (fb) ROFL_LAUNCH(k_msm_accumulate_fb, grid1((size_t)Wb * P.B, (u32)nq), dim3(TPB), 0, st, (u32)n, P.c, Wb, (u32)(np / nq), d_probs, cnt, off, slots, perm, buckets, cap, acc_balance);
             else ROFL_LAUNCH(k_msm_accumulate_gen, grid1((size_t)Wb * P.B, (u32)nq), dim3(TPB), 0, st, (u32)n, P.c, Wb, (u32)(np / nq), d_probs, cnt, off, slots, perm, buckets, cap, acc_balance);
         }
diff --git a/rofl_project_code_amd/csrc/host_prover.hpp b/rofl_project_code_amd/csrc/host_prover.hpp
--- a/rofl_project_code_amd/csrc/host_prover.hpp
+++ b/rofl_project_code_amd/csrc/host_prover.hpp
@@ -323,24 +323,13 @@
                 size_t thr = (size_t)2 * P * n_new;
                 while (K < FOLD_MAXSEG && thr * K < (size_t)C.fold_threads / (C.crowded() ? 2 : 1)) K *= 2;
                 if (C.fold_k > 0) K = (u32)C.fold_k;
-                FoldSeg seg{};
-                double eff = (double)(nsrc - 1);
-                double cst = 1.0 + (use_tab ? eff * fc.np / (fc.w + 1.0) : eff / 3.0), lo_t = 0, hi_t = (top + 1) * cst + top + 1;
-                int bounds[FOLD_MAXSEG + 1];
-                for (int it = 0; it < 60; it++) {
-                    double T = 0.5 * (lo_t + hi_t), pos = 0;
-                    for (u32 k = 0; k < K; k++) { double len = (T - pos) / cst; if (len < 0) len = 0; pos += len; }
-                    if (pos >= top + 1) hi_t = T; else lo_t = T;
-                }
-                { double pos = 0; bounds[0] = 0; for (u32 k = 0; k < K; k++) { double len = (hi_t - pos) / cst; if (len < 0) len = 0; pos += len; bounds[k + 1] = (int)(pos + 0.5); } }
-                bounds[K] = top + 1;
-                for (u32 k = 1; k <= K; k++) if (bounds[k] < bounds[k - 1]) bounds[k] = bounds[k - 1];
-                for (u32 k = 0; k <= FOLD_MAXSEG; k++) seg.lo[k] = bounds[k <= K ? k : K];
+                const double eff = (double)(nsrc - 1);
+                const FoldSeg seg = fold_segments(K, top, use_tab ? eff * fc.np / (fc.w + 1.0) : eff / 3.0);
                 dim3 grid((unsigned)((n_new + 63) / 64), (u32)(2 * P)), block(64, K);
                 if (knob("ROFL_TRACE")) fprintf(stderr, "[rofl] fold chunks=%zu n_g=%zu n_new=%zu nsrc=%u tab=%d pb=%u w=%u K=%u top=%d\n", P, n_g, n_new, nsrc, (int)use_tab, fc.pb, fc.w, K, top);
                 uint64_t nz = 0;
                 if (C.tm.enabled) { size_t tot_d = 2 * P * nsrc * dstride; for (size_t q = 0; q < tot_d; q++) nz += use_tab ? h_dig16[q] != 0 : h_dig[q] != 0; }
-                uint64_t fold_muls = (nz * 7 / (2 * P) + (uint64_t)(top + 1) * 8 + 7) * (uint64_t)(2 * P * n_new);
+                uint64_t fold_muls = (nz * 7 / (2 * P) + (uint64_t)(top + 1) * 7 + 1 + 7) * (uint64_t)(2 * P * n_new);
                 KSpan ks_fold(C.tm, C.stream, use_tab ? ROFL_TK_FOLD_TAB : ROFL_TK_FOLD, fold_muls, (uint64_t)2 * P * n_g * 32 + (uint64_t)2 * P * n_new * 32);
                 if (use_tab) {
                     const bool defer = 2 * P * n_new >= ((size_t)1 << 17);
diff --git a/rofl_project_code_amd/csrc/host_rt.hpp b/rofl_project_code_amd/csrc/host_rt.hpp
--- a/rofl_project_code_amd/csrc/host_rt.hpp
+++ b/rofl_project_code_amd/csrc/host_rt.hpp
@@ -110,6 +110,26 @@
         out[pos] = (int16_t)d; k >>= 1;
     }
     return top;
+}
+
+#define FOLD_MUL_COST 0.145
+FoldSeg fold_segments(u32 K, int top, double adds_per_pos) {
+    const double pos_cost = 1.0 + adds_per_pos - FOLD_MUL_COST, trail_cost = 1.0 - FOLD_MUL_COST;
+    double lo_t = 0, hi_t = (top + 1) * pos_cost + (top + 1) * trail_cost;
+    auto walk = [&](double T, int *bounds) {
+        double pos = 0;
+        if (bounds) bounds[0] = 0;
+        for (u32 k = 0; k < K; k++) { double len = (T - pos * trail_cost) / pos_cost; if (len < 0) len = 0; pos += len; if (bounds) bounds[k + 1] = (int)(pos + 0.5); }
+        return pos;
+    };
+    for (int it = 0; it < 60; it++) { const double T = 0.5 * (lo_t + hi_t); if (walk(T, nullptr) >= top + 1) hi_t = T; else lo_t = T; }
+    int bounds[FOLD_MAXSEG + 1];
+    walk(hi_t, bounds);
+    bounds[K] = top + 1;
+    for (u32 k = 1; k <= K; k++) if (bounds[k] < bounds[k - 1]) bounds[k] = bounds[k - 1];
+    FoldSeg seg{};
+    for (u32 k = 0; k <= FOLD_MAXSEG; k++) seg.lo[k] = bounds[k <= K ? k : K];
+    return seg;
 }
 
 using h51::ge5; using h51::niels5;
diff --git a/rofl_project_code_amd/csrc/kernels.hpp b/rofl_project_code_amd/csrc/kernels.hpp
--- a/rofl_project_code_amd/csrc/kernels.hpp
+++ b/rofl_project_code_amd/csrc/kernels.hpp
@@ -693,14 +693,18 @@
     gd acc = gd_identity();
     if (active) {
         int lo = seg.lo[k], hi = seg.lo[k + 1] - 1;
+        const u32 h0 = unit_first ? 1 : 0;
         for (int bit = hi; bit >= lo; bit--) {
-            acc = gd_double(acc);
-            for (u32 h = unit_first ? 1 : 0; h < nsrc; h++) {
+            const bool fin = bit == 0;
+            u32 last = 0; bool any = false;
+            for (u32 h = h0; h < nsrc; h++) if (dg[h * 256 + bit] != 0) { last = h; any = true; }
+            acc = gd_double(acc, any || fin);
+            for (u32 h = h0; h < nsrc; h++) {
                 int d = dg[h * 256 + bit];
-                if (d != 0) acc = gd_madd(acc, gload_nd(&src[(size_t)h * n_new + i]), d < 0);
+                if (d != 0) acc = gd_madd(acc, gload_nd(&src[(size_t)h * n_new + i]), d < 0, h != last || fin);
             }
         }
-        for (int t = 0; t < lo; t++) acc = gd_double(acc);
+        for (int t = 0; t < lo; t++) acc = gd_double(acc, t + 1 == lo);
     }
     if (K > 1) {
         if (k > 0) lds[(k - 1) * 64 + threadIdx.x] = gd_pack(acc);
@@ -730,13 +734,15 @@
         const nd s1 = gload_nd(&src[(size_t)1 * n_new + i]), s2 = gload_nd(&src[(size_t)2 * n_new + i]), s3 = gload_nd(&src[(size_t)3 * n_new + i]);
         int lo = seg.lo[k], hi = seg.lo[k + 1] - 1;
         for (int bit = hi; bit >= lo; bit--) {
-            acc = gd_double(acc);
-            int d1 = dg[256 + bit], d2 = dg[512 + bit], d3 = dg[768 + bit];
-            if (d1 != 0) acc = gd_madd(acc, s1, d1 < 0);
-            if (d2 != 0) acc = gd_madd(acc, s2, d2 < 0);
-            if (d3 != 0) acc = gd_madd(acc, s3, d3 < 0);
-        }
-        for (int t = 0; t < lo; t++) acc = gd_double(acc);
+            const int d1 = dg[256 + bit], d2 = dg[512 + bit], d3 = dg[768 + bit];
+            const bool fin = bit == 0;
+            const bool t3 = fin, t2 = t3 || d3 != 0, t1 = t2 || d2 != 0;
+            acc = gd_double(acc, t1 || d1 != 0);
+            if (d1 != 0) acc = gd_madd(acc, s1, d1 < 0, t1);
+            if (d2 != 0) acc = gd_madd(acc, s2, d2 < 0, t2);
+            if (d3 != 0) acc = gd_madd(acc, s3, d3 < 0, t3);
+        }
+        for (int t = 0; t < lo; t++) acc = gd_double(acc, t + 1 == lo);
     }
     if (K > 1) {
         if (k > 0) lds[(k - 1) * 64 + threadIdx.x] = gd_pack(acc);
@@ -770,7 +776,6 @@
         auto operand = [&](u32 w) { const u32 h = (w >> 9) & 63u, e = (w >> 15) & 4095u;
                                     const niels *p = e ? tb + (size_t)(e - 1) * tstride : src;
                                     return gload_nd(&p[(size_t)h * n_new + i]); };
-        const int lo = seg.lo[k];
         int pos = seg.lo[k + 1];
         u32 j = probs[q].seg_start[k];
         const u32 jend = k == 0 ? probs[q].n_ev : probs[q].seg_start[k - 1];
@@ -782,12 +787,11 @@
                 j++;
                 if (j < jend) { w = ev[j]; nxt = operand(w); }
                 const int b = (int)(wc & 511u);
-                for (; pos > b; pos--) acc = gd_double(acc);
-                acc = gd_madd(acc, cur, (wc >> 27) & 1u);
+                for (; pos > b; pos--) acc = gd_double(acc, pos == b + 1);
+                acc = gd_madd(acc, cur, (wc >> 27) & 1u, j < jend ? (int)(w & 511u) == b : b == 0);
             }
         }
-        for (; pos > lo; pos--) acc = gd_double(acc);
-        for (int t = 0; t < lo; t++) acc = gd_double(acc);
+        for (; pos > 0; pos--) acc = gd_double(acc, pos == 1);
     }
     if (K > 1) {
         if (k > 0) lds[(k - 1) * 64 + threadIdx.x] = gd_pack(acc);
@@ -1224,11 +1228,16 @@
     const niels *pts = probs[p * pstep].pts;
     gd acc = gd_identity();
     u32 vnext = num ? lst[0] : 0u;
-    for (u32 e = 0; e < num; e++) {
+    auto point = [&](u32 v) { const u32 idx = v & 0x7fffffffu; return FB ? gload_ndm(reinterpret_cast<const ndm *>(pts) + idx) : gload_nd(&pts[idx]); };
+    if (num) {
+        const u32 v = vnext;
+        if (1 < num) vnext = lst[1];
+        acc = gd_from_nd(point(v), (v >> 31) != 0);
+    }
+    for (u32 e = 1; e < num; e++) {
         u32 v = vnext;
         if (e + 1 < num) vnext = lst[e + 1];
-        u32 idx = v & 0x7fffffffu;
-        acc = gd_madd(acc, FB ? gload_ndm(reinterpret_cast<const ndm *>(pts) + idx) : gload_nd(&pts[idx]), (v >> 31) != 0);
+        acc = gd_madd(acc, point(v), (v >> 31) != 0);
     }
     store_gd(&buckets[bi], acc);
 }
@@ -1549,7 +1558,12 @@
         gd acc = gd_identity();
         u32 v = num ? lst[vb * cap] : 0u;
         nd nxt = fetch(v);
-        for (u32 e = 0; e < num; e++) {
+        if (num) {
+            const bool ng = (v & SIGN) != 0;
+            acc = gd_from_nd(nxt, ng);
+            if (1 < num) { v = lst[vb * cap + 1]; nxt = fetch(v); }
+        }
+        for (u32 e = 1; e < num; e++) {
             nd q = nxt; bool ng = (v & SIGN) != 0;
             if (e + 1 < num) { v = lst[vb * cap + e + 1]; nxt = fetch(v); }
             acc = gd_madd(acc, q, ng);
@@ -1673,6 +1687,10 @@
         gd_dbg_store(co, 0, R);
         gd_dbg_store(co, 4, op == FD_DBG_GQ_DOUBLE ? gd_double(P) : gd_add(P, Q));
     }
+}
+__global__ void __launch_bounds__(TPB) k_dbg_fd_ext(u32 op, u32 n, const u32 *in , u32 *out ) {
+    const u32 t = blockIdx.x * blockDim.x + threadIdx.x;
+    if (t < n) fd_dbg_apply_ext(op, in + (size_t)t * FD_DBG_IN, out + (size_t)t * FD_DBG_OUT);
 }
 __global__ void __launch_bounds__(TPB) k_dbg_sc(u32 op, u32 n, const u32 *in , u32 *out ) {
     const u32 t = blockIdx.x * blockDim.x + threadIdx.x;
diff --git a/rofl_project_code_amd/csrc/rofl_zk.hip b/rofl_project_code_amd/csrc/rofl_zk.hip
--- a/rofl_project_code_amd/csrc/rofl_zk.hip
+++ b/rofl_project_code_amd/csrc/rofl_zk.hip
@@ -2594,7 +2594,7 @@
 }
 static int dbg_ops_device(bool scalar_field, unsigned op, size_t n, const uint32_t *in, uint32_t *out) {
     const size_t in_words = scalar_field ? SC_DBG_IN : FD_DBG_IN, out_words = scalar_field ? SC_DBG_OUT : FD_DBG_OUT;
-    if (op >= (unsigned)(scalar_field ? SC_DBG_OPS : FD_DBG_OPS)) return fail(ROFL_BAD_PARAM, "bad parameter");
+    if (op >= (unsigned)(scalar_field ? SC_DBG_OPS : FD_DBG_OPS_EXT)) return fail(ROFL_BAD_PARAM, "bad parameter");
     return guarded([&]() -> int {
         LaneLock lane_lock = acquire_lane(); Ctx &C = *lane_lock.c;
         if (n == 0 || n > (1u << 20) || !in || !out) return fail(ROFL_BAD_PARAM, "bad parameter");
@@ -2603,13 +2603,58 @@
         C.up(din, in, n * in_words * 4, C.stream);
         C.up(dout, out, n * out_words * 4, C.stream);
         if (scalar_field) ROFL_LAUNCH(k_dbg_sc, grid1(n), dim3(TPB), 0, C.stream, (u32)op, (u32)n, (const u32 *)din, dout);
+        else if (op >= FD_DBG_OPS) ROFL_LAUNCH(k_dbg_fd_ext, grid1(n), dim3(TPB), 0, C.stream, (u32)op, (u32)n, (const u32 *)din, dout);
         else ROFL_LAUNCH(k_dbg_fd, grid1(op < FD_DBG_THREAD_OPS ? n : n * 4), dim3(TPB), 0, C.stream, (u32)op, (u32)n, (const u32 *)din, dout);
         C.down(out, dout, n * out_words * 4, C.stream);
         C.sync();
         return ROFL_OK;
     });
 }
-int rofl_dbg_fd_ops(unsigned op, size_t n, const uint32_t *in, uint32_t *out) { return dbg_ops_device(false, op, n, in, out); }
+int rofl_dbg_fd_ops(unsigned op, size_t n, const uint32_t *in, uint32_t *out) { if (op >= FD_DBG_OPS) return fail(ROFL_BAD_PARAM, "bad parameter"); return dbg_ops_device(false, op, n, in, out); }
+int rofl_dbg_fd_ops_ext(unsigned op, size_t n, const uint32_t *in, uint32_t *out) {
+    if (op < FD_DBG_OPS || op >= FD_DBG_OPS_EXT) return fail(ROFL_BAD_PARAM, "bad parameter");
+    return dbg_ops_device(false, op, n, in, out);
+}
+int rofl_dbg_fold(unsigned nsrc, unsigned K, const uint8_t *scalars32, const uint8_t *points32, size_t n_new, uint8_t *out32) {
+    return guarded([&]() -> int {
+        LaneLock lane_lock = acquire_lane(); Ctx &C = *lane_lock.c;
+        if (nsrc < 2 || nsrc > FOLD_MAXSRC || (K != 1 && K != 2 && K != 4) || !scalars32 || !points32 || !out32 || n_new == 0 || n_new > (1u << 16))
+            return fail(ROFL_BAD_PARAM, "bad parameter");
+        std::vector<sc> hs(nsrc);
+        for (unsigned h = 0; h < nsrc; h++) { hs[h] = sc_frombytes(scalars32 + 32 * h); if (sc_geq_l(hs[h].v)) return fail(ROFL_BAD_PARAM, "scalar is not canonical"); }
+        bool unit_first = hs[0].v[0] == 1; for (int i = 1; i < 8; i++) unit_first = unit_first && hs[0].v[i] == 0;
+        if (nsrc == 4 && !unit_first) return fail(ROFL_BAD_PARAM, "k_fold_gens4 takes source 0 with the scalar 1");
+        C.init();
+        const size_t n = (size_t)nsrc * n_new;
+        std::vector<int8_t> dig((size_t)nsrc * 256, 0);
+        int top = -1;
+        for (unsigned h = unit_first ? 1 : 0; h < nsrc; h++) top = std::max(top, sc_naf(dig.data() + (size_t)h * 256, hs[h]));
+        const FoldSeg seg = fold_segments(K, top, (double)(nsrc - 1) / 3.0);
+        uint8_t *dp = C.tmp_in.as<uint8_t>(n * 32); niels *src = C.aux_pts.as<niels>(n), *dst = C.gbuf[0].as<niels>(n_new);
+        int8_t *d_dig = C.naf.as<int8_t>(dig.size()); FoldProb *d_fp = C.foldprobs.as<FoldProb>(1);
+        u32 *status = C.status.as<u32>(4);
+        const FoldProb fp{src, dst};
+        HIPCHK(hipMemsetAsync(status, 0, 16, C.stream));
+        C.up(dp, points32, n * 32, C.stream);
+        C.up(d_dig, dig.data(), dig.size(), C.stream);
+        C.up(d_fp, &fp, sizeof fp, C.stream);
+        count_decodes(n);
+        ROFL_LAUNCH(k_decode, grid1(n), dim3(TPB), 0, C.stream, (u32)n, (u32)n, dp, (const niels *)nullptr, src, (uint8_t *)nullptr, status);
+        u32 st = 0;
+        HIPCHK(hipMemcpyAsync(&st, status, 4, hipMemcpyDeviceToHost, C.stream));
+        C.sync();
+        if (st & 4u) return fail(ROFL_FORMAT_ERROR, "invalid Ristretto encoding");
+        if (knob("ROFL_TRACE")) fprintf(stderr, "[rofl] fold chunks=%zu n_g=%zu n_new=%zu nsrc=%u tab=%d pb=%u w=%u K=%u top=%d\n", (size_t)1, n, n_new, nsrc, 0, 0u, 0u, K, top);
+        dim3 grid((unsigned)((n_new + 63) / 64), 1), block(64, K);
+        if (nsrc == 4) ROFL_LAUNCH(k_fold_gens4, grid, block, (K - 1) * 64 * sizeof(ge), C.stream, (u32)n_new, seg, (const FoldProb *)d_fp, (const int8_t *)d_dig);
+        else ROFL_LAUNCH(k_fold_gens, grid, block, (K - 1) * 64 * sizeof(ge), C.stream, (u32)n_new, (u32)nsrc, seg, (const FoldProb *)d_fp, (const int8_t *)d_dig, unit_first ? 1 : 0);
+        std::vector<niels> hn(n_new);
+        const niels *hp = static_cast<const niels *>(C.down(hn.data(), dst, n_new * sizeof(niels), C.stream));
+        C.sync();
+        for (size_t i = 0; i < n_new; i++) ristretto_encode(out32 + 32 * i, ge_from_niels(hp[i]));
+        return ROFL_OK;
+    });
+}
 int rofl_dbg_sc_ops(unsigned op, size_t n, const uint32_t *in, uint32_t *out) { return dbg_ops_device(true, op, n, in, out); }
 int rofl_dbg_quantize(unsigned site, size_t rows, size_t d, size_t dpad, size_t prove_range, unsigned fp_bits, unsigned fp_frac,
                       const float *values, const uint8_t *blindings32, void *out, float *terms_out, uint32_t *status_out) {
@@ -3405,6 +3450,11 @@
     for (size_t i = 0; i < n; i++) fd_dbg_apply(op, in + i * FD_DBG_IN, out + i * FD_DBG_OUT);
     return 0;
 }
+int rofl_dbg_host_fd_ops_ext(unsigned op, size_t n, const uint32_t *in, uint32_t *out) {
+    if (op < FD_DBG_OPS || op >= FD_DBG_OPS_EXT || !in || !out) return ROFL_BAD_PARAM;
+    for (size_t i = 0; i < n; i++) fd_dbg_apply_ext(op, in + i * FD_DBG_IN, out + i * FD_DBG_OUT);
+    return 0;
+}
 int rofl_dbg_host_sc_ops(unsigned op, size_t n, const uint32_t *in, uint32_t *out) {
     if (op >= SC_DBG_OPS || !in || !out) return ROFL_BAD_PARAM;
     for (size_t i = 0; i < n; i++) { const sc r = sc_dbg_apply(op, in + i * SC_DBG_IN); for (int k = 0; k < 8; k++) out[i * SC_DBG_OUT + k] = r.v[k]; }
```

Result: no change. 1.188 million (median of 6 runs) (+1.3%).
